# CMU-Quake/hercules

Hardware: AMD Instinct MI355X
Metric: element-updates/sec (whole node) + achieved HBM GB/s, 64M-elem box (higher is better)
Workload: dtype f64

## Files before the change

### hercules_amd/build.py

```python
import os
import subprocess
import sys

HERE = os.path.dirname(os.path.abspath(__file__))
ROOT = os.path.dirname(HERE)
CSRC = os.path.join(HERE, "csrc")
HIPCC = os.environ.get("HIPCC", "/opt/rocm/bin/hipcc")

SOLVER_LIB = os.path.join(CSRC, "libhq_solver.so")
HOST_LIB = os.path.join(CSRC, "libhq_host.so")


def _newer(target, sources):
    if not os.path.exists(target):
        return True
    t = os.path.getmtime(target)
    return any(os.path.getmtime(s) > t for s in sources)


def _build_solver(lib, defines, force):
    srcs = [os.path.join(CSRC, f) for f in ("hq_engine.hip", "hq_devmem.h", "hq_kernels.h", "hq_opts.h", "hq_patch.h",
                                           "hq_brick.h", "hq_prepare.h", "hq_plan_check.h", "hq_cadence.h", "hq_peak.h", "hq_cumul.h", "hq_sample.h", "hq_sdof.h",
                                           "hq_outputs.h")]
    srcs.append(os.path.join(ROOT, "include", "hq_solver.h"))
    if force or _newer(lib, srcs):
        cmd = [HIPCC, "-O3", "-std=c++17", "--offload-arch=gfx950", "-fPIC", "-shared"] + defines + \
              ["-fvisibility=hidden", "-fopenmp", "-Wno-unused-value"] + \
              os.environ.get("HQ_EXTRA_FLAGS", "").split() + \
              ["-o", lib, srcs[0], "-Wl,-rpath,/opt/rocm/lib", "-Wl,-Bsymbolic", "-ldl"]
        subprocess.check_call(cmd, cwd=CSRC)
    return lib


def build_solver(force=False):
    return _build_solver(SOLVER_LIB, [], force)


SOLVER_LIB_F32 = os.path.join(CSRC, "libhq_solver_f32.so")


def build_solver_f32(force=False):
    return _build_solver(SOLVER_LIB_F32, ["-DHQ_SINGLE_PRECISION_SOLVER"], force)


def build_host(force=False):
    src = os.path.join(CSRC, "hq_host.c")
    if not os.path.exists(src):
        return None
    deps = [src, os.path.join(CSRC, "hq_mesher.h"), os.path.join(CSRC, "hq_cadence.h"), os.path.join(CSRC, "hq_peak.h"), os.path.join(CSRC, "hq_cumul.h"),
            os.path.join(CSRC, "hq_sample.h"), os.path.join(CSRC, "hq_sdof.h"), os.path.join(ROOT, "include", "hq_host.h"),
            os.path.join(ROOT, "include", "hq_solver.h")]
    if force or _newer(HOST_LIB, deps):
        cmd = ["gcc", "-O2", "-std=gnu99", "-fPIC", "-shared", "-fvisibility=hidden", "-fopenmp",
               "-I", os.path.join(ROOT, "include"), "-o", HOST_LIB, src,
               "-L", CSRC, "-lhq_solver", "-Wl,-rpath,$ORIGIN", "-lm"]
        subprocess.check_call(cmd, cwd=CSRC)
    return HOST_LIB


EXAMPLE_BIN = os.path.join(ROOT, "examples", "hq_psolve_mini")


def build_example(force=False):
    src = os.path.join(ROOT, "examples", "hq_psolve_mini.c")
    if not os.path.exists(src):
        return None
    if force or _newer(EXAMPLE_BIN, [src, SOLVER_LIB, HOST_LIB]):
        cmd = ["gcc", "-O2", "-std=gnu99", "-I", os.path.join(ROOT, "include"), "-o", EXAMPLE_BIN, src,
               "-L", CSRC, "-lhq_host", "-lhq_solver", "-Wl,-rpath,$ORIGIN/../hercules_amd/csrc",
               "-Wl,-rpath,/opt/rocm/lib", "-lm"]
        subprocess.check_call(cmd)
    return EXAMPLE_BIN


def build(force=False):
    out = build_solver(force), build_host(force)
    build_solver_f32(force)
    build_example(force)
    return out


if __name__ == "__main__":
    print(build(force="--force" in sys.argv))
```

### hercules_amd/capi.py

```python
import ctypes
import os

import numpy as np

_HERE = os.path.dirname(os.path.abspath(__file__))
_LIBPATH = os.environ.get("HQ_SOLVER_LIB") or os.path.join(_HERE, "csrc", "libhq_solver.so")

HQ_VARIANT_AUTO, HQ_VARIANT_SCATTER, HQ_VARIANT_PATCH = 0, 1, 2
IPC_BLOB_BYTES = 4096

EXPORTS = ["hq_device_count", "hq_last_error", "hq_create", "hq_destroy", "hq_get_info", "hq_get_info_sized", "hq_abi_version", "hq_comm_init_ipc_n",
           "hq_options_init", "hq_create_opts", "hq_get_options", "hq_real_bytes",
           "hq_comm_unique_id", "hq_comm_init", "hq_comm_selftest", "hq_group_link", "hq_group_run", "hq_set_source", "hq_run", "hq_sync", "hq_gather", "hq_gather3",
           "hq_download", "hq_upload", "hq_phase_force", "hq_phase_update", "hq_download_force",
           "hq_run_timed", "hq_dominant_kernel", "hq_plan_check", "hq_stencil_plan_check", "hq_check_finite",
           "hq_stencil_coefficients", "hq_brick_plan_check", "hq_brick_plan_check_n", "hq_comm_init_host",
           "hq_comm_ipc_export", "hq_comm_init_ipc", "hq_comm_init_loopback",
           "hq_record_add", "hq_record_pending", "hq_record_fetch", "hq_record_clear",
           "hq_snapshot_add", "hq_snapshot_pending", "hq_snapshot_fetch", "hq_snapshot_clear",
           "hq_peak_add", "hq_peak_fetch", "hq_peak_load", "hq_peak_reset", "hq_peak_clear",
           "hq_spec_add", "hq_spec_coefficients", "hq_spec_fetch", "hq_spec_load", "hq_spec_reset", "hq_spec_clear",
           "hq_cum_add", "hq_cum_fetch", "hq_cum_load", "hq_cum_reset", "hq_cum_clear"]
HQ_SNAP_TM1, HQ_SNAP_TM2, HQ_SNAP_VEL = 1, 2, 4
HQ_PEAK_DISP, HQ_PEAK_VEL, HQ_PEAK_ACC = 1, 2, 4
HQ_SPEC_MAX_PERIODS, HQ_SPEC_NVAL = 32, 4


class HqError(RuntimeError):
    pass


HOST_EXCHANGE_FN = ctypes.CFUNCTYPE(ctypes.c_int, ctypes.c_void_p, ctypes.c_int32, ctypes.POINTER(ctypes.c_int32),
                                    ctypes.POINTER(ctypes.c_int64), ctypes.POINTER(ctypes.c_void_p), ctypes.c_int32,
                                    ctypes.POINTER(ctypes.c_int32), ctypes.POINTER(ctypes.c_int64),
                                    ctypes.POINTER(ctypes.c_void_p), ctypes.c_int32)


class _Messenger(ctypes.Structure):
    _fields_ = [("procid", ctypes.c_int32), ("nodecount", ctypes.c_int32),
                ("mapping", ctypes.c_void_p)]


class _Schedule(ctypes.Structure):
    _fields_ = [("c_count", ctypes.c_int32), ("first_c", ctypes.POINTER(_Messenger)),
                ("s_count", ctypes.c_int32), ("first_s", ctypes.POINTER(_Messenger))]


class _Desc(ctypes.Structure):
    _fields_ = [("lenum", ctypes.c_int32), ("nharbored", ctypes.c_int32), ("ldnnum", ctypes.c_int32),
                ("lnid", ctypes.c_void_p), ("node_xyz", ctypes.c_void_p),
                ("dn_ldnid", ctypes.c_void_p), ("dn_ptr", ctypes.c_void_p), ("dn_lanid", ctypes.c_void_p),
                ("eTable", ctypes.c_void_p), ("nTable", ctypes.c_void_p),
                ("tm1", ctypes.c_void_p), ("tm2", ctypes.c_void_p),
                ("an_sched", _Schedule), ("dn_sched", _Schedule),
                ("deltaT", ctypes.c_double), ("rank", ctypes.c_int32), ("nranks", ctypes.c_int32),
                ("variant", ctypes.c_int32), ("reserved", ctypes.c_int32), ("node_gnid", ctypes.c_void_p),
                ("edata", ctypes.c_void_p), ("mat_bbase", ctypes.c_double), ("mat_threshold_damping", ctypes.c_double),
                ("mat_threshold_vpvs", ctypes.c_double)]


class _RecorderDesc(ctypes.Structure):
    _fields_ = [("npoints", ctypes.c_int32), ("ids", ctypes.c_void_p), ("phi", ctypes.c_void_p),
                ("rate", ctypes.c_int32), ("derivs", ctypes.c_int32), ("capacity", ctypes.c_int32)]


class _SnapshotDesc(ctypes.Structure):
    _fields_ = [("first", ctypes.c_int32), ("count", ctypes.c_int32), ("rate", ctypes.c_int32),
                ("first_step", ctypes.c_int32), ("fields", ctypes.c_int32), ("slots", ctypes.c_int32)]


class _PeakDesc(ctypes.Structure):
    _fields_ = [("npoints", ctypes.c_int32), ("nodes_per_point", ctypes.c_int32), ("ids", ctypes.c_void_p),
                ("phi", ctypes.c_void_p), ("rate", ctypes.c_int32), ("first_step", ctypes.c_int32),
                ("quantities", ctypes.c_int32), ("reserved", ctypes.c_int32)]


class _SpecDesc(ctypes.Structure):
    _fields_ = [("npoints", ctypes.c_int32), ("nodes_per_point", ctypes.c_int32), ("ids", ctypes.c_void_p),
                ("phi", ctypes.c_void_p), ("rate", ctypes.c_int32), ("first_step", ctypes.c_int32),
                ("nperiods", ctypes.c_int32), ("reserved", ctypes.c_int32), ("periods", ctypes.c_void_p),
                ("damping", ctypes.c_double)]


class _CumDesc(ctypes.Structure):
    _fields_ = [("npoints", ctypes.c_int32), ("nodes_per_point", ctypes.c_int32), ("ids", ctypes.c_void_p),
                ("phi", ctypes.c_void_p), ("rate", ctypes.c_int32), ("first_step", ctypes.c_int32),
                ("quantities", ctypes.c_int32), ("husid_every", ctypes.c_int32), ("husid_slots", ctypes.c_int32),
                ("reserved", ctypes.c_int32), ("threshold", ctypes.c_double * 3)]


class _Info(ctypes.Structure):
    _fields_ = [("variant", ctypes.c_int32), ("npatches", ctypes.c_int32),
                ("patch_pairs", ctypes.c_int64), ("device_bytes", ctypes.c_int64),
                ("step", ctypes.c_int32), ("nranks", ctypes.c_int32),
                ("lattice_patches", ctypes.c_int32), ("stencil_patches", ctypes.c_int32),
                ("ragged_patches", ctypes.c_int32), ("brick_units", ctypes.c_int32),
                ("brick_nodes", ctypes.c_int64), ("brick_units_pernode", ctypes.c_int32),
                ("brick_units_het", ctypes.c_int32), ("pcie_h2d_bytes", ctypes.c_int64),
                ("pcie_d2h_bytes", ctypes.c_int64), ("transport", ctypes.c_int32), ("ipc_arena_coarse", ctypes.c_int32),
                ("ipc_arena_kind", ctypes.c_int32), ("debug_halo", ctypes.c_int32),
                ("brick_units_packed", ctypes.c_int32), ("brick_units_ragged", ctypes.c_int32),
                ("brick_stream", ctypes.c_int32), ("brick_units_ragged_het", ctypes.c_int32), ("timed_steps", ctypes.c_int64),
                ("t_step_us", ctypes.c_double), ("t_shell_us", ctypes.c_double), ("t_interior_us", ctypes.c_double),
                ("t_chain_us", ctypes.c_double), ("t_chain_exposed_us", ctypes.c_double)]


OPTION_FIELDS = ["no_bricks", "brick_cz", "brick_minz", "brick_minnodes", "brick_no_het", "brick_no_ntsame", "brick_by_component",
                 "brick_stream", "brick_no_faces", "brick_half_tiles", "brick_no_pack", "patch_pipe", "patch_threads", "patch_pmax", "patch_pmerge", "patch_psplit", "patch_nlmax",
                 "patch_vmax", "patch_ragged", "patch_no_lattice", "patch_no_stencil", "patch_no_uniform", "patch_no_iso",
                 "patch_no_ntsame", "patch_no_dedup", "patch_wform", "patch_merge_rounds", "overlap", "no_overlap", "reserve_cus",
                 "cu_mask", "no_fused_share", "group_copies", "debug_halo", "ipc_arena"]


class Options(ctypes.Structure):
    _fields_ = ([("size", ctypes.c_uint64)] + [(n, ctypes.c_int32) for n in OPTION_FIELDS] +
                [("ipc_timeout_ms", ctypes.c_double), ("loopback_delay_us", ctypes.c_double),
                 ("verbose", ctypes.c_int32), ("quiet", ctypes.c_int32),
                 ("brick_ragged", ctypes.c_int32), ("brick_ragged_minfill", ctypes.c_int32),
                 ("allow_env", ctypes.c_int32), ("brick_ragged_het", ctypes.c_int32), ("reserved0", ctypes.c_int32),
                 ("phase_timing", ctypes.c_int32)])

    def __init__(self, **kw):
        super().__init__()
        load_library().hq_options_init(ctypes.byref(self), ctypes.c_uint64(ctypes.sizeof(self)))
        for k, v in kw.items():
            if k not in dict(self._fields_):
                raise TypeError("hq_options has no field %r" % k)
            setattr(self, k, v)

    def as_dict(self):
        return {k: getattr(self, k) for k, _ in self._fields_ if k != "size"}


_lib = None
_lib_f32 = None
_LIBPATH_F32 = os.environ.get("HQ_SOLVER_LIB_F32") or os.path.join(_HERE, "csrc", "libhq_solver_f32.so")


def load_library(path=None, precision="f64"):
    global _lib, _lib_f32
    if precision == "f32" and path is None:
        if _lib_f32 is None:
            _lib_f32 = load_library(_LIBPATH_F32)
            if _lib_f32.hq_real_bytes() != 4:
                raise HqError("%s was not built with -DHQ_SINGLE_PRECISION_SOLVER" % _LIBPATH_F32)
        return _lib_f32
    if _lib is not None and path is None:
        return _lib
    p = path or _LIBPATH
    if not os.path.exists(p):
        raise HqError("native library %s is missing: run `python -m hercules_amd.build` "
                      "(there is no Python/CPU fallback)" % p)
    probe = ctypes.CDLL(p, mode=ctypes.RTLD_LOCAL)
    lib = probe if probe.hq_real_bytes() == 4 else ctypes.CDLL(p, mode=ctypes.RTLD_GLOBAL)
    lib.hq_last_error.restype = ctypes.c_char_p
    lib.hq_dominant_kernel.restype = ctypes.c_char_p
    lib.hq_dominant_kernel.argtypes = [ctypes.c_void_p]
    for name in EXPORTS:
        getattr(lib, name)
    if path is None:
        _lib = lib
    return lib


def device_count():
    return int(load_library().hq_device_count())


def _check(rc, lib=None):
    if rc != 0:
        raise HqError("hq error %d: %s" % (rc, (lib or load_library()).hq_last_error().decode()))


def _ptr(a):
    return None if a is None else a.ctypes.data_as(ctypes.c_void_p)


def _schedule(sched, keep):
    out = _Schedule()
    if not sched:
        return out
    for key, cnt, first in (("c", "c_count", "first_c"), ("s", "s_count", "first_s")):
        items = sched.get(key, [])
        arr = (_Messenger * max(len(items), 1))()
        for i, (procid, mapping) in enumerate(items):
            m = np.ascontiguousarray(mapping, np.int32)
            keep.append(m)
            arr[i].procid = int(procid)
            arr[i].nodecount = len(m)
            arr[i].mapping = m.ctypes.data
        keep.append(arr)
        setattr(out, cnt, len(items))
        setattr(out, first, ctypes.cast(arr, ctypes.POINTER(_Messenger)))
    return out


class Solver:

    def __init__(self, lnid, etable, ntable, dt, tm1=None, tm2=None, node_xyz=None,
                 dangling=None, an_sched=None, dn_sched=None, rank=0, nranks=1,
                 variant=HQ_VARIANT_AUTO, device=0, options=None, edata=None, material=None, precision="f64"):
        lib = load_library(precision=precision)
# ... 44 lines not shown
    def close(self):
        if getattr(self, "_h", None) and self._h.value:
            self._lib.hq_destroy(self._h)
            self._h = ctypes.c_void_p()

    __del__ = close

    def info(self):
        i = _Info()
        _check(self._lib.hq_get_info_sized(self._h, ctypes.byref(i), ctypes.c_uint64(ctypes.sizeof(i))), self._lib)
        return {k: getattr(i, k) for k, _ in _Info._fields_}

    def options(self):
        o = Options()
        _check(self._lib.hq_get_options(self._h, ctypes.byref(o), ctypes.c_uint64(ctypes.sizeof(o))), self._lib)
        return o.as_dict()

    def set_source(self, loaded_lnid, forces, step0=0):
        ids = np.ascontiguousarray(loaded_lnid, np.int32)
        F = np.ascontiguousarray(forces, np.float64)
        nsteps = F.shape[0] if len(ids) else 0
        _check(self._lib.hq_set_source(self._h, ctypes.c_int32(len(ids)), _ptr(ids),
                                       ctypes.c_int32(step0), ctypes.c_int32(nsteps), _ptr(F)))

    def comm_init(self, id128):
        buf = (ctypes.c_char * 128).from_buffer_copy(bytes(id128))
        _check(self._lib.hq_comm_init(self._h, buf), self._lib)

    def comm_init_host(self, exchange):
        import numpy as np

        def view(ptr, n):
            return np.ctypeslib.as_array(ctypes.cast(ctypes.c_void_p(ptr), ctypes.POINTER(ctypes.c_double)), shape=(int(n),))

        def trampoline(user, nrecv, rpeer, rcount, rbuf, nsend, speer, scount, sbuf, tag):
            try:
                exchange([(rpeer[i], view(rbuf[i], rcount[i])) for i in range(nrecv)],
                         [(speer[i], view(sbuf[i], scount[i])) for i in range(nsend)], tag)
                return 0
            except Exception:
                import traceback
                traceback.print_exc()
                return 1
        self._host_exchange = HOST_EXCHANGE_FN(trampoline)
        _check(self._lib.hq_comm_init_host(self._h, self._host_exchange, None), self._lib)

    def comm_ipc_export(self):
        buf = (ctypes.c_char * IPC_BLOB_BYTES)()
        _check(self._lib.hq_comm_ipc_export(self._h, buf), self._lib)
        return bytes(buf)

    def comm_init_ipc(self, blobs):
        raw = blobs if isinstance(blobs, (bytes, bytearray)) else b"".join(blobs)
        if len(raw) % IPC_BLOB_BYTES:
            raise HqError("comm_init_ipc: %d bytes is not a whole number of %d-byte blobs" % (len(raw), IPC_BLOB_BYTES))
        buf = (ctypes.c_char * len(raw)).from_buffer_copy(bytes(raw))
        _check(self._lib.hq_comm_init_ipc_n(self._h, buf, ctypes.c_int32(len(raw) // IPC_BLOB_BYTES)), self._lib)

    def comm_init_loopback(self):
        _check(self._lib.hq_comm_init_loopback(self._h), self._lib)

    def comm_selftest(self, count=1024):
        _check(self._lib.hq_comm_selftest(self._h, ctypes.c_int32(count)), self._lib)

    def run(self, nsteps):
        _check(self._lib.hq_run(self._h, ctypes.c_int32(nsteps)), self._lib)

    def sync(self):
        _check(self._lib.hq_sync(self._h), self._lib)

    def check_finite(self):
        n = ctypes.c_int64()
        _check(self._lib.hq_check_finite(self._h, ctypes.byref(n)), self._lib)
        return int(n.value)

    def run_timed(self, nsteps):
        tot, ker = ctypes.c_double(), ctypes.c_double()
        _check(self._lib.hq_run_timed(self._h, ctypes.c_int32(nsteps), ctypes.byref(tot), ctypes.byref(ker)), self._lib)
        return tot.value, ker.value

    def dominant_kernel(self):
        return self._lib.hq_dominant_kernel(self._h).decode()

    def download(self, want_tm2=True):
        tm1 = np.empty((self.N, 3), self.real)
        tm2 = np.empty((self.N, 3), self.real) if want_tm2 else None
        _check(self._lib.hq_download(self._h, _ptr(tm1), _ptr(tm2)), self._lib)
        return tm1, tm2

    def upload(self, tm1, tm2, step):
        a = np.ascontiguousarray(tm1, self.real)
        b = np.ascontiguousarray(tm2, self.real)
        _check(self._lib.hq_upload(self._h, _ptr(a), _ptr(b), ctypes.c_int32(step)), self._lib)

    def gather(self, lnid):
        ids = np.ascontiguousarray(np.asarray(lnid).reshape(-1), np.int32)
        o1 = np.empty((len(ids), 3), self.real)
        o2 = np.empty((len(ids), 3), self.real)
        _check(self._lib.hq_gather(self._h, ctypes.c_int32(len(ids)), _ptr(ids), _ptr(o1), _ptr(o2)), self._lib)
        return o1, o2

    def gather3(self, lnid):
        ids = np.ascontiguousarray(np.asarray(lnid).reshape(-1), np.int32)
        o = [np.empty((len(ids), 3), self.real) for _ in range(3)]
        _check(self._lib.hq_gather3(self._h, ctypes.c_int32(len(ids)), _ptr(ids), _ptr(o[0]), _ptr(o[1]), _ptr(o[2])), self._lib)
        return tuple(o)

    def record_add(self, ids, phi, rate, derivs=0, capacity=1024):
        ids = np.ascontiguousarray(np.asarray(ids).reshape(-1, 8), np.int32)
        phi = np.ascontiguousarray(np.asarray(phi).reshape(-1, 8), np.float64)
        if len(ids) != len(phi):
            raise HqError("record_add: %d rows of ids, %d of phi" % (len(ids), len(phi)))
        d = _RecorderDesc(len(ids), ids.ctypes.data, phi.ctypes.data, int(rate), int(derivs), int(capacity))
        h = ctypes.c_int32(-1)
        _check(self._lib.hq_record_add(self._h, ctypes.byref(d), ctypes.byref(h)), self._lib)
        if not hasattr(self, "_recorders"):
            self._recorders = {}
        self._recorders[h.value] = (len(ids), 3 * (1 + int(derivs)))
        return h.value

    def record_pending(self, handle):
        n, first = ctypes.c_int32(), ctypes.c_int32()
        _check(self._lib.hq_record_pending(self._h, ctypes.c_int32(handle), ctypes.byref(n), ctypes.byref(first)), self._lib)
        return n.value, first.value

    def record_fetch(self, handle, max_samples=None):
        pending, _ = self.record_pending(handle)
        npoints, ncomp = self._recorders[handle]
        want = pending if max_samples is None else min(int(max_samples), pending)
        steps = np.zeros(max(want, 1), np.int32)
        vals = np.zeros((max(want, 1), npoints, ncomp))
        got = ctypes.c_int32()
        _check(self._lib.hq_record_fetch(self._h, ctypes.c_int32(handle), ctypes.c_int32(want), _ptr(vals), _ptr(steps),
                                         ctypes.byref(got)), self._lib)
        return steps[:got.value].copy(), vals[:got.value].copy()

    def record_clear(self):
        _check(self._lib.hq_record_clear(self._h), self._lib)
        self._recorders = {}

    def snapshot_add(self, first=0, count=None, rate=1, first_step=0, fields=HQ_SNAP_TM1, slots=1):
        count = self.N - int(first) if count is None else int(count)
        d = _SnapshotDesc(int(first), count, int(rate), int(first_step), int(fields), int(slots))
        h = ctypes.c_int32(-1)
        _check(self._lib.hq_snapshot_add(self._h, ctypes.byref(d), ctypes.byref(h)), self._lib)
        if not hasattr(self, "_snapshots"):
            self._snapshots = {}
        self._snapshots[h.value] = (count, int(fields))
        return h.value

    def snapshot_pending(self, handle):
        n, ready, first = ctypes.c_int32(), ctypes.c_int32(), ctypes.c_int32()
        _check(self._lib.hq_snapshot_pending(self._h, ctypes.c_int32(handle), ctypes.byref(n), ctypes.byref(ready),
                                             ctypes.byref(first)), self._lib)
        return n.value, ready.value, first.value

    def snapshot_fetch(self, handle):
        self.snapshot_pending(handle)
        count, fields = self._snapshots[handle]
        tm1 = np.empty((count, 3), self.real) if fields & HQ_SNAP_TM1 else None
        tm2 = np.empty((count, 3), self.real) if fields & HQ_SNAP_TM2 else None
        vel = np.empty((count, 3), np.float64) if fields & HQ_SNAP_VEL else None
        step = ctypes.c_int32(-1)
        _check(self._lib.hq_snapshot_fetch(self._h, ctypes.c_int32(handle), _ptr(tm1), _ptr(tm2), _ptr(vel),
                                           ctypes.byref(step)), self._lib)
        if step.value < 0:
# ... 246 lines not shown
```

### hercules_amd/csrc/hq_brick.h

```cpp
#ifndef HQ_BRICK_H
#define HQ_BRICK_H

#include <chrono>
#include <map>

#include "hq_patch.h"

#define HQ_BK_TX 64
#ifndef HQ_BK_TY
#define HQ_BK_TY 8
#endif
#define HQ_BK_THREADS (HQ_BK_TX * HQ_BK_TY)
#define HQ_BK_PY (HQ_BK_TX + 2)
#define HQ_BK_PLANE ((HQ_BK_TX + 2) * (HQ_BK_TY + 2))
#ifndef HQ_BK_ATTR
#define HQ_BK_ATTR
#endif
#define HQ_BK_NTSAME 1
#define HQ_BK_HET 2
#define HQ_BK_TOPFACE 8
#define HQ_BK_BOTFACE 16
#define HQ_BK_RAGGED 32
#define HQ_BK_PACKED 4
#ifndef HQ_BH_WAVES
// ... 670 lines not shown
                            if (cx >= 0 && cy >= 0 && cz >= 0 && cx < L.D[0] && cy < L.D[1] && cz < L.D[2])
                                e = L.Eg[(size_t)((cz * L.D[1] + cy) * L.D[0] + cx)];
                            float* o = cq + (int64_t)l * (3 * HQ_BH_THREADS) + (j * 64 + i);
                            o[0] = o[HQ_BH_CS] = o[2 * HQ_BH_CS] = 0.0f;
                            if (e < 0) continue;
                            const float* ed = MS->edata + 4 * (int64_t)e;
                            if (ed[0] != hf || !(ed[3] > 0.0f)) { ok = false; break; }
                            bool hit = false;
                            for (int fixed = 0; fixed < 2 && !hit; fixed++) {
                                double k1, k2, kb;
                                hq_material_coef(fixed ? -ed[3] : ed[3], ed[2], ed[1], K, &k1, &k2, &kb);
                                if (k1 == c1[e] && k2 == c2[e] && kb == beta[e]) { o[0] = fixed ? -ed[3] : ed[3]; o[HQ_BH_CS] = ed[2]; o[2 * HQ_BH_CS] = ed[1]; hit = true; }
                            }
                            if (!hit) { ok = false; break; }
                        }
                const int32_t* own_ids = c.rag ? t + (int64_t)(np + 2) * nr + (int64_t)nx * ny : nullptr;
                for (int32_t z = 0; z < np && ok; z++)
                    for (int32_t y = 0; y < ny && ok; y++)
                        for (int32_t x = 0; x < nx; x++) {
                            if (own_ids && own_ids[((int64_t)z * ny + y) * nx + x] < 0) continue;
                            const int32_t n = L.Ng[(size_t)((((int64_t)za + z) * NY + (c.y0 + y)) * NX + (c.x0 + x))];
                            const double* q = ntab + 7 * (int64_t)n;
                            const double sdiff = q[0] - q[4];
                            if (q[0] - sdiff != q[4] || fabs((2.0 * q[0] - sdiff) - q[1]) > 1e-15 * fabs(q[1])) { ok = false; break; }
                            double* o2 = B->nt2.data() + 2 * (own_ids ? (int64_t)own_ids[((int64_t)z * ny + y) * nx + x] : U.base + ((int64_t)z * ny + y) * nx + x);
                            o2[0] = q[0]; o2[1] = sdiff;
                        }
                if (ok) { U.flags |= HQ_BK_PACKED; same[(size_t)u] = c.rag ? 6 : 3; U.c1 = K.A; U.c2 = K.h; }
            }
        }
    }
    lap("unit tables");
    if (fault) { g_patch_err = "brick plan: a neighbour of a simple node is missing"; return -1; }
    {
        std::vector<hq_brick_unit> a, r, b, h, hp, rh, rhp;
        for (size_t u = 0; u < us.size(); u++)
            (same[u] == 1 ? a : (same[u] == 4 ? r : (same[u] == 2 ? h : (same[u] == 3 ? hp : (same[u] == 5 ? rh : (same[u] == 6 ? rhp : b)))))).push_back(B->units[u]);
        B->nsame = (int32_t)(a.size() + r.size());
        B->nrag = (int32_t)r.size();
        B->nhet = (int32_t)(h.size() + hp.size());
        B->npacked = (int32_t)hp.size();
        B->nrhet = (int32_t)(rh.size() + rhp.size());
        B->nrpacked = (int32_t)rhp.size();
        a.insert(a.end(), r.begin(), r.end());
        a.insert(a.end(), b.begin(), b.end());
        a.insert(a.end(), h.begin(), h.end());
        a.insert(a.end(), hp.begin(), hp.end());
        a.insert(a.end(), rh.begin(), rh.end());
        a.insert(a.end(), rhp.begin(), rhp.end());
        B->units.swap(a);
        if (B->npacked + B->nrpacked == 0) { std::vector<float>().swap(B->coef32); std::vector<double>().swap(B->nt2); }
        if (verbose) fprintf(stderr, "  brick plan: %d units: %d with one n_t row of which %d ragged, %d per-element coefficients of which %d packed, %d ragged per-element of which %d packed\n",
                             (int)B->units.size(), B->nsame, B->nrag, B->nhet, B->npacked, B->nrhet, B->nrpacked);
        if (verbose && B->nrag) {
            int64_t pos = 0, own = 0, other = 0;
            for (const hq_brick_unit& U : B->units) {
                if (!(U.flags & HQ_BK_RAGGED)) continue;
                const int32_t* pl = B->tab.data() + U.tab + (int64_t)(U.np + 2) * (2 * (U.nx + 2) + 2 * U.ny);
                for (int64_t i = 0; i < (int64_t)U.nx * U.ny * (U.np + 2); i++) { pos++; own += pl[i] >= 0; other += pl[i] <= -2; }
            }
            fprintf(stderr, "  brick plan: ragged units: %lld positions, %lld owned, %lld loaded for their neighbours' sake\n", (long long)pos, (long long)own, (long long)other);
        }
    }
    return 0;
}


static __device__ __forceinline__ double hq_uniform(double v)
{
    const int lo = __builtin_amdgcn_readfirstlane(__double2loint(v)), hi = __builtin_amdgcn_readfirstlane(__double2hiint(v));
    return __hiloint2double(hi, lo);
}

template <bool PERNODE, bool BYCOMP, bool RAGGED = false>
__global__ void HQ_BK_ATTR __launch_bounds__(HQ_BK_THREADS, 4)
hq_k_brick(int32_t count, int32_t per_xcd, const hq_brick_unit* __restrict__ units, const int32_t* __restrict__ tab,
           const hq_real* __restrict__ u1g, const hq_real* __restrict__ u2g, hq_real* __restrict__ ung,
           const double* __restrict__ nt3, const int32_t* __restrict__ src_ptr, const int32_t* __restrict__ src_ent,
           const double* __restrict__ F, double dt2, hq_stencil_coef sc)
{
    __shared__ __align__(16) double s_w[2 * 3 * HQ_BK_PLANE];
    const int slot = (int)(blockIdx.x & 7) * per_xcd + (int)(blockIdx.x >> 3);
    if (slot >= count) return;
    const hq_brick_unit U = units[slot];
    const int nx = U.nx, ny = U.ny, np = U.np, nxy = nx * ny, nr = 2 * (nx + 2) + 2 * ny;
    const int t = threadIdx.x, lx = t & (HQ_BK_TX - 1), ly = t >> 6;
    const bool active = lx < nx && ly < ny;
    const int sidx = active ? ly * nx + lx : 0;
    const int myrow = (ly + 1) * HQ_BK_PY + lx + 1;
    const bool ring = t < nr;
    int rrow;
    {
        int rx, ry;
        if (t < nx + 2) { rx = t - 1; ry = -1; }
        else if (t < 2 * (nx + 2)) { rx = t - (nx + 2) - 1; ry = ny; }
        else if (t < 2 * (nx + 2) + ny) { rx = -1; ry = t - 2 * (nx + 2); }
        else { rx = nx; ry = t - 2 * (nx + 2) - ny; }
        rrow = (ry + 1) * HQ_BK_PY + rx + 1;
    }
    const int32_t* __restrict__ utab = tab + U.tab;
    const int rofs = ring ? t : 0;
    const int32_t* __restrict__ cap = utab + (int64_t)(np + 2) * nr;
    int32_t vOut = -1, vMid = RAGGED ? cap[sidx] : 0, vCur = RAGGED ? cap[nxy + sidx] : 0, vNext = 0;
    const int32_t id_lo = RAGGED ? (vMid >= 0 ? vMid : -vMid - 2) : cap[sidx];
    const double beta = U.beta;
    double P[6], Q[2];
#pragma unroll
    for (int i = 0; i < 6; i++) P[i] = hq_uniform(U.c1 * sc.p1[i] + U.c2 * sc.p2[i]);
#pragma unroll
    for (int i = 0; i < 2; i++) Q[i] = hq_uniform(U.c1 * sc.q1[i] + U.c2 * sc.q2[i]);
    const bool has_src = F && src_ptr[slot + 1] > src_ptr[slot];

    hq_real x1[3] = { 0, 0, 0 }, x2[3] = { 0, 0, 0 }, y1[3] = { 0, 0, 0 }, y2[3] = { 0, 0, 0 };
    double mn[3] = { U.m0, U.m2, U.m1 };
    double m0A = hq_uniform(1.0 / U.m0), m0B = m0A;
    double fA[3] = { 0.0, 0.0, 0.0 }, fB[3] = { 0.0, 0.0, 0.0 };
    int32_t rid = utab[rofs];

#define HQ_BK_LOAD(node_)                                                                             \
    {                                                                                                 \
        const int64_t a_ = (node_);                                                                   \
        if (active && (!RAGGED || a_ >= 0)) {                                                         \
            _Pragma("unroll") for (int d = 0; d < 3; d++) { x1[d] = u1g[3 * a_ + d]; x2[d] = u2g[3 * a_ + d]; } \
            if (PERNODE) { _Pragma("unroll") for (int d = 0; d < 3; d++) mn[d] = nt3[3 * a_ + d]; }    \
        }                                                                                             \
        if (ring && (!RAGGED || rid >= 0)) {                                                          \
            const int64_t b_ = (int64_t)rid;                                                          \
            _Pragma("unroll") for (int d = 0; d < 3; d++) { y1[d] = u1g[3 * b_ + d]; y2[d] = u2g[3 * b_ + d]; } \
        }                                                                                             \
    }
#define HQ_BK_PUT(s_, acc_, M2_, M1_)                                                                 \
    {                                                                                                 \
        hq_lds_double* img_ = (hq_lds_double*)s_w + 3 * HQ_BK_PLANE * (s_);                            \
        if (active) {                                                                                 \
            _Pragma("unroll") for (int d = 0; d < 3; d++) {                                           \
                const double a1_ = x1[d], a2_ = x2[d];                                                \
                img_[3 * myrow + d] = a1_ + beta * (a1_ - a2_);                                       \
                acc_[d] += (M2_) * a1_ - (M1_) * a2_;                                                 \
            }                                                                                         \
        }                                                                                             \
        if (ring) { _Pragma("unroll") for (int d = 0; d < 3; d++) { const double b1_ = y1[d], b2_ = y2[d]; img_[3 * rrow + d] = b1_ + beta * (b1_ - b2_); } } \
    }

    const bool topf = !PERNODE && !RAGGED && (U.flags & HQ_BK_TOPFACE) != 0, botf = !PERNODE && !RAGGED && (U.flags & HQ_BK_BOTFACE) != 0;
    const double rho = hq_uniform((U.c1 - U.c2) / (U.c1 + U.c2));

    HQ_BK_LOAD((int64_t)id_lo)
    rid = utab[nr + rofs];
    if (topf) HQ_BK_PUT(0, fB, U.ft[1 + d], U.ft[4 + d])
    else { double dummy[3] = { 0.0, 0.0, 0.0 }; HQ_BK_PUT(0, dummy, mn[1], mn[2]) }
    for (int k = 0; k <= np + 1; k++) {
        if (k <= np) {
            if (RAGGED) {
                HQ_BK_LOAD((int64_t)(vCur >= 0 ? vCur : -vCur - 2))
                if (k < np) vNext = cap[(k + 2) * nxy + sidx];
            } else HQ_BK_LOAD(k == np ? (int64_t)cap[nxy + sidx] : U.base + (int64_t)k * nxy + sidx)
            if (k < np) rid = utab[(k + 2) * nr + rofs];
        }
        __syncthreads();
        const hq_lds_double* __restrict__ q = (const hq_lds_double*)s_w + 3 * (HQ_BK_PLANE * (k & 1) + myrow);
        double m[3], g[3], Uo[3];
        if (BYCOMP) {
            double A_x, A_y;
            {
                const double C = q[2], XM = q[2 - 3], XP = q[2 + 3], YM = q[2 - 3 * HQ_BK_PY], YP = q[2 + 3 * HQ_BK_PY];
                const double MM = q[2 - 3 * HQ_BK_PY - 3], PM = q[2 - 3 * HQ_BK_PY + 3], MP = q[2 + 3 * HQ_BK_PY - 3], PP = q[2 + 3 * HQ_BK_PY + 3];
                const double sxy = (XM + XP) + (YM + YP), dg = (MM + PP) + (PM + MP);
                m[2] = fma(P[0], C, fma(P[2], sxy, P[4] * dg));
                g[2] = fma(P[1], C, fma(P[3], sxy, P[5] * dg));
                Uo[0] = fma(Q[0], XP - XM, Q[1] * ((PP - MP) + (PM - MM)));
                Uo[1] = fma(Q[0], YP - YM, Q[1] * ((PP - PM) + (MP - MM)));
            }
            __builtin_amdgcn_sched_barrier(0);
            {
                const double C = q[0], XM = q[0 - 3], XP = q[0 + 3], YM = q[0 - 3 * HQ_BK_PY], YP = q[0 + 3 * HQ_BK_PY];
                const double MM = q[0 - 3 * HQ_BK_PY - 3], PM = q[0 - 3 * HQ_BK_PY + 3], MP = q[0 + 3 * HQ_BK_PY - 3], PP = q[0 + 3 * HQ_BK_PY + 3];
                const double sx = XM + XP, sy = YM + YP, dg = (MM + PP) + (PM + MP);
                A_x = (PP + MM) - (PM + MP);
                m[0] = fma(P[0], C, fma(P[1], sx, fma(P[2], sy, P[3] * dg)));
                g[0] = fma(P[2], C, fma(P[3], sx, fma(P[4], sy, P[5] * dg)));
                Uo[2] = fma(Q[0], XP - XM, Q[1] * ((PP - MP) + (PM - MM)));
            }
            __builtin_amdgcn_sched_barrier(0);
            {
                const double C = q[1], XM = q[1 - 3], XP = q[1 + 3], YM = q[1 - 3 * HQ_BK_PY], YP = q[1 + 3 * HQ_BK_PY];
                const double MM = q[1 - 3 * HQ_BK_PY - 3], PM = q[1 - 3 * HQ_BK_PY + 3], MP = q[1 + 3 * HQ_BK_PY - 3], PP = q[1 + 3 * HQ_BK_PY + 3];
                const double sx = XM + XP, sy = YM + YP, dg = (MM + PP) + (PM + MP);
                A_y = (PP + MM) - (PM + MP);
                m[1] = fma(P[0], C, fma(P[1], sy, fma(P[2], sx, fma(P[3], dg, Q[0] * A_x))));
                g[1] = fma(P[2], C, fma(P[3], sy, fma(P[4], sx, fma(P[5], dg, Q[1] * A_x))));
                Uo[2] += fma(Q[0], YP - YM, Q[1] * ((PP - PM) + (MP - MM)));
            }
            m[0] = fma(Q[0], A_y, m[0]);
            g[0] = fma(Q[1], A_y, g[0]);
        } else {
            double C[3], XM[3], XP[3], YM[3], YP[3], MM[3], PM[3], MP[3], PP[3];
#pragma unroll
            for (int d = 0; d < 3; d++) {
                C[d] = q[d]; XM[d] = q[d - 3]; XP[d] = q[d + 3]; YM[d] = q[d - 3 * HQ_BK_PY]; YP[d] = q[d + 3 * HQ_BK_PY];
                MM[d] = q[d - 3 * HQ_BK_PY - 3]; PM[d] = q[d - 3 * HQ_BK_PY + 3];
                MP[d] = q[d + 3 * HQ_BK_PY - 3]; PP[d] = q[d + 3 * HQ_BK_PY + 3];
            }
            double sx[3], sy[3], dg[3];
#pragma unroll
            for (int d = 0; d < 3; d++) { sx[d] = XM[d] + XP[d]; sy[d] = YM[d] + YP[d]; dg[d] = (MM[d] + PP[d]) + (PM[d] + MP[d]); }
            const double A_x = (PP[0] + MM[0]) - (PM[0] + MP[0]), A_y = (PP[1] + MM[1]) - (PM[1] + MP[1]);
            const double Bx0_z = XP[2] - XM[2], Bx0_x = XP[0] - XM[0], By0_z = YP[2] - YM[2], By0_y = YP[1] - YM[1];
            const double Bx1_z = (PP[2] - MP[2]) + (PM[2] - MM[2]), Bx1_x = (PP[0] - MP[0]) + (PM[0] - MM[0]);
            const double By1_z = (PP[2] - PM[2]) + (MP[2] - MM[2]), By1_y = (PP[1] - PM[1]) + (MP[1] - MM[1]);
            const double sxy_z = sx[2] + sy[2];
            m[0] = fma(P[0], C[0], fma(P[1], sx[0], fma(P[2], sy[0], fma(P[3], dg[0], Q[0] * A_y))));
            m[1] = fma(P[0], C[1], fma(P[1], sy[1], fma(P[2], sx[1], fma(P[3], dg[1], Q[0] * A_x))));
            m[2] = fma(P[0], C[2], fma(P[2], sxy_z, P[4] * dg[2]));
            g[0] = fma(P[2], C[0], fma(P[3], sx[0], fma(P[4], sy[0], fma(P[5], dg[0], Q[1] * A_y))));
            g[1] = fma(P[2], C[1], fma(P[3], sy[1], fma(P[4], sx[1], fma(P[5], dg[1], Q[1] * A_x))));
            g[2] = fma(P[1], C[2], fma(P[3], sxy_z, P[5] * dg[2]));
            Uo[0] = fma(Q[0], Bx0_z, Q[1] * Bx1_z);
            Uo[1] = fma(Q[0], By0_z, Q[1] * By1_z);
            Uo[2] = fma(Q[0], Bx0_x, fma(Q[1], Bx1_x, fma(Q[0], By0_y, Q[1] * By1_y)));
        }
        if (k == 0 && topf) {
            m[0] = fma(rho, Uo[0], 0.5 * m[0]); m[1] = fma(rho, Uo[1], 0.5 * m[1]); m[2] = fma(-rho, Uo[2], 0.5 * m[2]);
        }
        if (k == np + 1 && botf && active) {
            double f[3];
            f[0] = fB[0] + fma(-rho, Uo[0], 0.5 * m[0]); f[1] = fB[1] + fma(-rho, Uo[1], 0.5 * m[1]); f[2] = fB[2] + fma(rho, Uo[2], 0.5 * m[2]);
            const int local = np * nxy + sidx;
            if (has_src) {
                for (int i = src_ptr[slot]; i < src_ptr[slot + 1]; i++)
                    if (src_ent[2 * i] == local) {
                        const int li = src_ent[2 * i + 1];
                        for (int d = 0; d < 3; d++) f[d] += F[3 * li + d] * dt2;
                    }
            }
            hq_real* out = ung + 3 * (int64_t)cap[nxy + sidx];
            const double rm = 1.0 / U.fb[0];
#pragma unroll
            for (int d = 0; d < 3; d++) out[d] = f[d] * rm;
        }
        const bool outface = k == 1 && topf;
        if ((k >= 2 || outface) && active && (!RAGGED || vOut >= 0)) {
            double f[3];
#pragma unroll
            for (int d = 0; d < 3; d++) f[d] = fA[d] + (g[d] + Uo[d]);
            const int local = RAGGED ? (int)(vOut - U.base) : (k - 2) * nxy + sidx;
            if (has_src) {
                for (int i = src_ptr[slot]; i < src_ptr[slot + 1]; i++)
                    if (src_ent[2 * i] == local) {
                        const int li = src_ent[2 * i + 1];
                        for (int d = 0; d < 3; d++) f[d] += F[3 * li + d] * dt2;
                    }
            }
            hq_real* out = ung + 3 * (RAGGED ? (int64_t)vOut : (outface ? (int64_t)cap[sidx] : U.base + (int64_t)local));
            const double rm = outface ? 1.0 / U.ft[0] : m0A;
#pragma unroll
            for (int d = 0; d < 3; d++) out[d] = f[d] * rm;
        }
#pragma unroll
        for (int d = 0; d < 3; d++) { fA[d] = fB[d] + m[d]; fB[d] = g[d] - Uo[d]; }
        if (RAGGED) { vOut = vMid; vMid = vCur; vCur = vNext; }
        if (PERNODE) { m0A = m0B; m0B = 1.0 / mn[0]; }
        if (k < np || (k == np && !botf)) HQ_BK_PUT((k + 1) & 1, fB, mn[1], mn[2])
        else if (k == np) HQ_BK_PUT((k + 1) & 1, fB, U.fb[1 + d], U.fb[4 + d])
    }
#undef HQ_BK_LOAD
#undef HQ_BK_PUT
}


#define HQ_BH_LDS (8 * (2 * 2 * 3 * HQ_BH_ROWS + 6 * HQ_BH_THREADS))
#ifndef HQ_BH_ABL
#define HQ_BH_ABL 0
#endif

static __device__ __forceinline__ double hq_dpp_from_next_lane(double v)
{
    int lo = __double2loint(v), hi = __double2hiint(v);
    lo = __builtin_amdgcn_update_dpp(0, lo, 0x130, 0xf, 0xf, true);
    hi = __builtin_amdgcn_update_dpp(0, hi, 0x130, 0xf, 0xf, true);
    return __hiloint2double(hi, lo);
}

static __device__ __forceinline__ int64_t hq_rag_node(int32_t v) { return v >= 0 ? (int64_t)v : (v <= -2 ? (int64_t)(-v - 2) : (int64_t)0); }

template <bool PACKED, bool RAGGED = false>
__global__ void __launch_bounds__(HQ_BH_THREADS, HQ_BH_WAVES == 12 ? 3 : 4)
hq_k_brick_het(int32_t count, int32_t per_xcd, const hq_brick_unit* __restrict__ units, const int32_t* __restrict__ tab,
               const void* __restrict__ coef_any, const hq_real* __restrict__ u1g, const hq_real* __restrict__ u2g,
               hq_real* __restrict__ ung, const double* __restrict__ nt3, const int32_t* __restrict__ src_ptr,
               const int32_t* __restrict__ src_ent, const double* __restrict__ F, double dt2, hq_mat_const mat)
{
    extern __shared__ __align__(16) double s_het[];
    hq_lds_double* const img = (hq_lds_double*)s_het;
    hq_lds_double* const xch = img + 2 * 2 * 3 * HQ_BH_ROWS;
    const int slot = (int)(blockIdx.x & 7) * per_xcd + (int)(blockIdx.x >> 3);
    if (slot >= count) return;
    const hq_brick_unit U = units[slot];
    const int nx = U.nx, ny = U.ny, np = U.np, nxy = nx * ny, nr = 2 * (nx + 2) + 2 * ny;
    const int t = threadIdx.x, lx = t & 63, ly = t >> 6;
    const bool owner = lx < nx && ly < ny;
    const int sidx = owner ? ly * nx + lx : 0;
    const int myrow = (ly + 1) * HQ_BH_PY + lx + 1;
    const int row0 = ly * HQ_BH_PY + lx;
    const int rq = ly == HQ_BH_WAVES - 1 ? lx : (lx >= 62 ? 64 + 2 * ly + (lx - 62) : -1);
    const bool ringA = rq >= 0 && rq < nr, ringB = rq >= 0 && rq + HQ_BH_NRT < nr;
    auto ring_row = [&](int r) {
        int rx, ry;
        if (r < nx + 2) { rx = r - 1; ry = -1; }
        else if (r < 2 * (nx + 2)) { rx = r - (nx + 2) - 1; ry = ny; }
        else if (r < 2 * (nx + 2) + ny) { rx = -1; ry = r - 2 * (nx + 2); }
        else { rx = nx; ry = r - 2 * (nx + 2) - ny; }
        return (ry + 1) * HQ_BH_PY + rx + 1;
    };
    const int rrowA = ringA ? ring_row(rq) : 0, rrowB = ringB ? ring_row(rq + HQ_BH_NRT) : 0;
    const int32_t* __restrict__ rtabA = tab + U.tab + (ringA ? rq : 0);
    const int32_t* __restrict__ rtabB = tab + U.tab + (ringB ? rq + HQ_BH_NRT : 0);
    const int32_t* __restrict__ cap = tab + U.tab + (int64_t)(np + 2) * nr;
    const int64_t id_lo = RAGGED ? 0 : cap[sidx], id_hi = RAGGED ? 0 : cap[nxy + sidx];
    int32_t vload = RAGGED ? cap[sidx] : 0, vnext = RAGGED ? cap[nxy + sidx] : 0, idA = -1, idB = -1;
    const double* __restrict__ cf = (const double*)coef_any + (PACKED ? 0 : U.coef + t);
    const float* __restrict__ cf32 = (const float*)coef_any + (PACKED ? U.coef + t : 0);
    hq_mat_const K = mat;
    if (PACKED) { K.A = hq_uniform(U.c1); K.h = hq_uniform(U.c2); }
    const int third = (PACKED && owner) ? 1 : 2;
    const bool has_src = F && src_ptr[slot + 1] > src_ptr[slot];

    hq_real x1[3] = { 0, 0, 0 }, x2[3] = { 0, 0, 0 }, rb1[3] = { 0, 0, 0 }, rb2[3] = { 0, 0, 0 };
    constexpr bool SAME = sizeof(hq_real) == sizeof(double);
    double mn[3] = { 1.0, 0.0, 0.0 };
    double accA[3] = { 0.0, 0.0, 0.0 }, accB[3] = { 0.0, 0.0, 0.0 }, m0A = 1.0, m0B = 1.0;
    int32_t ridA = rtabA[0], ridB = rtabB[0];
    if (RAGGED) { ridA = ridA < 0 ? 0 : ridA; ridB = ridB < 0 ? 0 : ridB; }

#define HQ_BH_LOAD(node_)                                                                             \
    {                                                                                                 \
        const int64_t a_ = owner ? (int64_t)(node_) : (int64_t)ridA;                                  \
        const double* __restrict__ pb_ = (owner || sizeof(hq_real) != sizeof(double)) ? nt3 + (PACKED ? 2 : 3) * a_ : (const double*)(const void*)(u1g + 3 * (int64_t)ridB); \
        _Pragma("unroll") for (int d = 0; d < 3; d++) { x1[d] = u1g[3 * a_ + d]; x2[d] = u2g[3 * a_ + d]; } \
        if (SAME || owner) {                                                                          \
            if (HQ_BH_ABL != 4) { mn[0] = pb_[0]; mn[1] = pb_[1]; mn[2] = pb_[third]; }                \
        } else {                      \
            const hq_real* __restrict__ pu_ = u1g + 3 * (int64_t)ridB;                                \
            rb1[0] = pu_[0]; rb1[1] = pu_[1]; rb1[2] = pu_[2];                                         \
        }                                                                                             \
    }
#define HQ_BH_LOAD_B()                                                                                \
    {                                                                                                 \
        if (ringB && HQ_BH_ABL != 1) {                                                                \
            const int64_t b_ = (int64_t)ridB;                                                         \
// ... 99 lines not shown
        __syncthreads();
    }
#undef HQ_BH_REQUEST
#undef HQ_BH_LOAD
#undef HQ_BH_LOAD_B
#undef HQ_BH_PUT
}


static void hq_brick_free(hq_brick_plan* P)
{
    *P = hq_brick_plan();
}

static int hq_brick_upload(hq_brick_plan* P, const hq_brick_host& B, int64_t* ledger, hipStream_t st)
{
    P->nb = B.nb;
    P->nunits = (int32_t)B.units.size();
    P->nsame = B.nsame;
    P->nrag = B.nrag;
    P->nhet = B.nhet;
    P->npacked = B.npacked;
    P->nrhet = B.nrhet;
    P->nrpacked = B.nrpacked;
    if (P->nunits == 0) return HQ_OK;
    if (P->nhet + P->nrhet > 0) {
        if (P->nhet > P->npacked || P->nrhet > P->nrpacked) HQ_TRY(P->d_coef.put(ledger, B.coef, st));
        if (P->npacked + P->nrpacked > 0) {
            HQ_TRY(P->d_coef32.put(ledger, B.coef32, st));
            HQ_TRY(P->d_nt2.put(ledger, B.nt2, st));
        }
        static bool attr_set = false;
        if (!attr_set) {
            if (hipFuncSetAttribute((const void*)hq_k_brick_het<false>, hipFuncAttributeMaxDynamicSharedMemorySize, HQ_BH_LDS) != hipSuccess ||
                hipFuncSetAttribute((const void*)hq_k_brick_het<true>, hipFuncAttributeMaxDynamicSharedMemorySize, HQ_BH_LDS) != hipSuccess ||
                hipFuncSetAttribute((const void*)hq_k_brick_het<false, true>, hipFuncAttributeMaxDynamicSharedMemorySize, HQ_BH_LDS) != hipSuccess ||
                hipFuncSetAttribute((const void*)hq_k_brick_het<true, true>, hipFuncAttributeMaxDynamicSharedMemorySize, HQ_BH_LDS) != hipSuccess) return hq_fail(HQ_ERR_DEVICE, "hq_k_brick_het: LDS attribute%s", "");
            attr_set = true;
        }
    }
    HQ_TRY(P->d_units.put(ledger, B.units, st));
    HQ_TRY(P->d_tab.put(ledger, B.tab, st));
    std::vector<std::pair<int64_t, int32_t>> by_base;
    for (int32_t u = 0; u < P->nunits; u++) by_base.push_back({ B.units[(size_t)u].base, u });
    std::sort(by_base.begin(), by_base.end());
    for (auto& pr : by_base) {
        const hq_brick_unit& U = B.units[(size_t)pr.second];
        const int64_t nxy = (int64_t)U.nx * U.ny;
        const int top = (U.flags & HQ_BK_TOPFACE) != 0, bot = (U.flags & HQ_BK_BOTFACE) != 0;
        int64_t size = nxy * (U.np + top + bot);
        if (U.flags & HQ_BK_RAGGED) {
            const int32_t* pl = B.tab.data() + U.tab + (int64_t)(U.np + 2) * (2 * (U.nx + 2) + 2 * U.ny);
            size = 0;
            for (int64_t i = nxy; i < nxy * (U.np + 1); i++) size += pl[i] >= 0;
        }
        P->h_base.push_back(pr.first - top * nxy); P->h_slot.push_back(pr.second); P->h_size.push_back(size);
        P->h_first.push_back(pr.first);
    }
    return HQ_OK;
}

static int hq_brick_set_source(hq_brick_plan* P, int32_t nloaded, const int32_t* loaded, int64_t* ledger, hipStream_t st)
{
    P->d_src_ptr.reset();
    P->d_src_ent.reset();
    if (nloaded <= 0 || P->nunits == 0) return HQ_OK;
    std::vector<std::array<int32_t, 3>> rec;
    for (int32_t i = 0; i < nloaded; i++) {
        if (loaded[i] >= P->nb) continue;
        const size_t k = (size_t)(std::upper_bound(P->h_base.begin(), P->h_base.end(), (int64_t)loaded[i]) - P->h_base.begin()) - 1;
        rec.push_back({ P->h_slot[k], (int32_t)(loaded[i] - P->h_first[k]), i });
    }
    if (rec.empty()) return HQ_OK;
    std::sort(rec.begin(), rec.end());
    std::vector<int32_t> ptr((size_t)P->nunits + 1, 0), ent(rec.size() * 2);
    for (auto& r : rec) ptr[(size_t)r[0] + 1]++;
    for (int32_t u = 0; u < P->nunits; u++) ptr[(size_t)u + 1] += ptr[(size_t)u];
    for (size_t k = 0; k < rec.size(); k++) { ent[2 * k] = rec[k][1]; ent[2 * k + 1] = rec[k][2]; }
    HQ_TRY(P->d_src_ptr.put(ledger, ptr, st));
    return P->d_src_ent.put(ledger, ent, st);
}

static void hq_brick_launch(const hq_brick_plan* P, const hq_real* u1, const hq_real* u2, hq_real* un, const double* nt3,
                            const double* F, double dt2, hipStream_t stream, bool light = false)
{
    const int32_t cnt[7] = { P->nsame - P->nrag, P->nunits - P->nsame - P->nhet - P->nrhet, P->nhet - P->npacked, P->npacked, P->nrag,
                             P->nrhet - P->nrpacked, P->nrpacked };
    int32_t first = 0;
    for (int k4 = 0; k4 < 7; k4++) {
        const int k = k4 == 0 ? 0 : (k4 == 1 ? 4 : (k4 < 5 ? k4 - 1 : k4));
        const int32_t count = cnt[k];
        if (count <= 0) continue;
        const int per_xcd = (count + 7) / 8;
        const int32_t* sp = P->d_src_ptr ? P->d_src_ptr + first : nullptr;
#define HQ_BK_ARGS count, per_xcd, P->d_units + first, P->d_tab, u1, u2, un, nt3, sp, P->d_src_ent, (sp ? F : nullptr), dt2, hq_stencil().c
#ifdef HQ_EXPERIMENT
        const unsigned xpad = getenv("HQ_X_BRICK_LDS_PAD") ? (unsigned)atoi(getenv("HQ_X_BRICK_LDS_PAD")) : 0u;
        if (xpad && k == 0) {
            static bool once = false;
            if (!once) {
                once = true;
                hipFuncSetAttribute((const void*)hq_k_brick<false, true>, hipFuncAttributeMaxDynamicSharedMemorySize, (int)xpad);
                hipFuncSetAttribute((const void*)hq_k_brick<false, false>, hipFuncAttributeMaxDynamicSharedMemorySize, (int)xpad);
            }
            if (light) hq_k_brick<false, true><<<per_xcd * 8, HQ_BK_THREADS, xpad, stream>>>(HQ_BK_ARGS);
            else hq_k_brick<false, false><<<per_xcd * 8, HQ_BK_THREADS, xpad, stream>>>(HQ_BK_ARGS);
        } else
#endif
        if (k == 0 && light) hq_k_brick<false, true><<<per_xcd * 8, HQ_BK_THREADS, 0, stream>>>(HQ_BK_ARGS);
        else if (k == 0) hq_k_brick<false, false><<<per_xcd * 8, HQ_BK_THREADS, 0, stream>>>(HQ_BK_ARGS);
        else if (k == 1 && light) hq_k_brick<true, true><<<per_xcd * 8, HQ_BK_THREADS, 0, stream>>>(HQ_BK_ARGS);
        else if (k == 1) hq_k_brick<true, false><<<per_xcd * 8, HQ_BK_THREADS, 0, stream>>>(HQ_BK_ARGS);
        else if (k == 4 && light) hq_k_brick<false, true, true><<<per_xcd * 8, HQ_BK_THREADS, 0, stream>>>(HQ_BK_ARGS);
        else if (k == 4) hq_k_brick<false, false, true><<<per_xcd * 8, HQ_BK_THREADS, 0, stream>>>(HQ_BK_ARGS);
        else if (k == 2) hq_k_brick_het<false><<<per_xcd * 8, HQ_BH_THREADS, HQ_BH_LDS, stream>>>(count, per_xcd, P->d_units + first, P->d_tab, P->d_coef, u1, u2, un, nt3, sp,
                                                                                               P->d_src_ent, (sp ? F : nullptr), dt2, P->mat);
        else if (k == 3) hq_k_brick_het<true><<<per_xcd * 8, HQ_BH_THREADS, HQ_BH_LDS, stream>>>(count, per_xcd, P->d_units + first, P->d_tab, P->d_coef32, u1, u2, un, P->d_nt2, sp,
                                                                                   P->d_src_ent, (sp ? F : nullptr), dt2, P->mat);
        else if (k == 5) hq_k_brick_het<false, true><<<per_xcd * 8, HQ_BH_THREADS, HQ_BH_LDS, stream>>>(count, per_xcd, P->d_units + first, P->d_tab, P->d_coef, u1, u2, un, nt3, sp,
                                                                                                     P->d_src_ent, (sp ? F : nullptr), dt2, P->mat);
        else hq_k_brick_het<true, true><<<per_xcd * 8, HQ_BH_THREADS, HQ_BH_LDS, stream>>>(count, per_xcd, P->d_units + first, P->d_tab, P->d_coef32, u1, u2, un, P->d_nt2, sp,
                                                                                          P->d_src_ent, (sp ? F : nullptr), dt2, P->mat);
#undef HQ_BK_ARGS
        first += count;
    }
}

#endif
```

### hercules_amd/csrc/hq_engine.hip

```cpp
#include <hip/hip_runtime.h>
#include <dlfcn.h>
#include <stdint.h>
#include <stdio.h>
#include <stdlib.h>
#include <string.h>
#include <unistd.h>

#include <algorithm>
#include <chrono>
#include <vector>

#define HQ_SOLVER_IMPLEMENTATION 1
#include "../../include/hq_solver.h"
#include "hq_devmem.h"
#include "hq_kernels.h"
#include "hq_opts.h"
#include "hq_cadence.h"
#include "hq_peak.h"
#include "hq_cumul.h"
#include "hq_sdof.h"
#define HQ_SAMPLE_REAL hq_real
#include "hq_sample.h"
#include "hq_patch.h"
#include "hq_brick.h"
// ... 44 lines not shown

#define HQ_NCCL(call)                                                                     \
    do {                                                                                  \
        ncclResult_t r_ = (call);                                                         \
        if (r_ != ncclSuccess) return hq_fail(HQ_ERR_COMM, "%s: %s", #call, g_rccl.GetErrorString(r_)); \
    } while (0)


struct hq_dev_messenger {
    int32_t procid, nodecount;
    int32_t offset;
};

struct hq_dev_schedule {
    std::vector<hq_dev_messenger> c, s;
    hq_dbuf<int32_t> d_cmap;
    hq_dbuf<int32_t> d_smap;
    int32_t* d_cmap_f = nullptr;
    int32_t* d_smap_f = nullptr;
    hq_dbuf<int32_t> d_cslot, d_sslot;
    hq_dbuf<double> d_c_out;
    hq_dbuf<double> d_s_out;
    double*  d_c_in = nullptr;
    double*  d_s_in = nullptr;
    hq_dbuf<double> c_in_mem, s_in_mem;
    int32_t  ctotal = 0, stotal = 0;
    hq_dbuf<int64_t> d_c_out_id, d_c_in_id, d_s_out_id, d_s_in_id;
    hq_dbuf<double*> d_c_dst, d_s_dst;
    double*  h_c_out = nullptr;
    double*  h_c_in = nullptr;
    double*  h_s_out = nullptr;
    double*  h_s_in = nullptr;
    int64_t* h_c_out_id = nullptr;
    int64_t* h_c_in_id = nullptr;
    int64_t* h_s_out_id = nullptr;
    int64_t* h_s_in_id = nullptr;
};

struct hq_ctx {
    hq_options opts;
    int device = 0;
    hipStream_t stream = nullptr;
    int32_t E = 0, N = 0, ldnnum = 0;
    int32_t variant = HQ_VARIANT_SCATTER;
    int32_t step = 0;
    int32_t rank = 0, nranks = 1;
    double dt = 0, dt2 = 0;
    int64_t bytes = 0;
    int64_t h2d_bytes = 0, d2h_bytes = 0;
    hq_dbuf<int32_t> d_gather_ids;
    hq_dbuf<hq_real> d_gather_out;
    int32_t gather_cap = 0;

    int32_t Epad = 0;
    hq_dbuf<int32_t> d_lnid;
    hq_dbuf<double> d_c1, d_c2, d_beta;
    double* d_nt = nullptr;
    hq_dbuf<double> d_nt_rows;
    hq_dbuf<hq_real> d_u[3];
    int now = 0, prev = 1, spare = 2;
    hq_dbuf<double> d_force;
    int32_t nloaded = 0, src_step0 = 0, src_nsteps = 0;
    hq_dbuf<int32_t> d_loaded;
    hq_dbuf<double> d_F;
    std::vector<int32_t> h_loaded;
    size_t F_capacity = 0;
    hq_dbuf<int32_t> d_dn_id, d_dn_ptr, d_dn_anchor;
    hq_dev_schedule an, dn;
    hq_nccl_comm comm = nullptr;
    hq_host_exchange_fn host_xchg = nullptr;
    void* host_user = nullptr;
    std::vector<hq_ctx*>* group = nullptr;
    bool group_owner = false;
    bool share_packed = false;
    struct hq_ipc_state* ipc = nullptr;
    hipEvent_t ev_sent = nullptr;
    hipStream_t cstream = nullptr;
    hipEvent_t ev_bnd = nullptr, ev_shared = nullptr, ev_an_shared = nullptr, ev_assigned = nullptr;
    hipStream_t bstream = nullptr;
    hipEvent_t ev_patches = nullptr, ev_bricks = nullptr;
    bool overlap = false;
    bool stream_masked = false;
    bool can_overlap = false;
    int reserve_cus = 8;
    int32_t nI = 0, nOI = 0;
    hq_dbuf<double> d_iforce;
    hq_dbuf<int32_t> d_oi_node;
    hq_dbuf<int32_t> d_oi_slot;
    hq_dbuf<int32_t> d_oi_ptr;
    hq_dbuf<int32_t> d_oi_pos;
    hq_dbuf<int32_t> d_oi_fc;
    int32_t  nSD = 0;
    hq_dbuf<int32_t> d_sd_dst;
    hq_dbuf<int32_t> d_sd_ptr;
    hq_dbuf<int32_t> d_sd_src;
    hq_dbuf<int32_t> d_sd_deps;
    hq_patch_plan plan;
    hq_brick_plan bricks;
    std::vector<int32_t> perm;
    bool debug_halo = false;
    unsigned long long dbg_send_epoch[4] = { 0, 0, 0, 0 }, dbg_recv_epoch[4] = { 0, 0, 0, 0 };
    hq_dbuf<int64_t> d_gkey;
    hq_dbuf<int32_t> d_halo_err;
    enum { HQ_CLK_STEP0 = 0, HQ_CLK_SHELL1, HQ_CLK_INT0, HQ_CLK_INT1, HQ_CLK_CHAIN0, HQ_CLK_CHAIN1, HQ_CLK_N, HQ_CLK_SLOTS = 64 };
    struct hq_clock_slot { hipEvent_t e[HQ_CLK_N] = {}; bool used[HQ_CLK_N] = {}; bool pending = false; };
    bool clock_skip = false;
    std::vector<hq_clock_slot> clock;
    size_t clock_at = 0;
    double clk_us[5] = { 0, 0, 0, 0, 0 };
    int64_t clk_steps = 0;
    struct hq_output; struct hq_recorder; struct hq_peak_tracker; struct hq_spec_tracker; struct hq_cum_tracker; struct hq_snapshot;
    std::vector<hq_recorder> recs;
    int32_t rec_next_id = 0;
    std::vector<hq_peak_tracker> peaks;
    int32_t peak_next_id = 0;
    std::vector<hq_spec_tracker> specs;
    int32_t spec_next_id = 0;
    std::vector<hq_cum_tracker> cums;
    int32_t cum_next_id = 0;
    std::vector<hq_snapshot> snaps;
    int32_t snap_next_id = 0;
    hipStream_t sstream = nullptr;
    hipEvent_t ev_output = nullptr;
    std::vector<hipEvent_t> ev;
    hipEvent_t ev_span[2] = { nullptr, nullptr };
    bool timing = false;
    size_t ev_used = 0;
};

enum { HQ_IPC_MAXNB = 64, HQ_IPC_MAGIC = 0x48514950  };
struct hq_ipc_blob {
    uint32_t magic, version;
    int32_t rank, nranks, device, pid;
    int32_t coarse, reserved;
    char busid[32];
    uint64_t arena_bytes, arena_addr;
    hipIpcMemHandle_t mem;
    uint64_t buf_off[4];
    uint64_t flag_off;
    uint64_t id_off[4];
    int32_t nrecv[4];
    struct { int32_t procid, offset, count; } recv[4][HQ_IPC_MAXNB];
};
static_assert(sizeof(hq_ipc_blob) <= HQ_IPC_BLOB_BYTES, "hq_ipc_blob must fit HQ_IPC_BLOB_BYTES");

struct hq_ipc_state {
    void* arena = nullptr;
    size_t arena_bytes = 0;
    bool coarse = false, ready = false, loopback = false;
    int arena_kind = 0;
    hq_ipc_blob mine;
    std::vector<void*> opened;
    unsigned long long* d_flags = nullptr;
    hq_dbuf<double*> d_dst[4];
    hq_dbuf<unsigned long long*> d_sig[4];
    hq_dbuf<int64_t*> d_dst_id[4];
    int64_t* d_in_id[4] = { nullptr, nullptr, nullptr, nullptr };
    int32_t nsig[4] = { 0, 0, 0, 0 };
    unsigned long long wait_mask[4] = { 0, 0, 0, 0 };
    unsigned long long send_epoch[4] = { 0, 0, 0, 0 }, recv_epoch[4] = { 0, 0, 0, 0 };
    hq_dbuf<uint32_t> d_done;
    unsigned long long timeout_ticks = 2000000000ull;
    unsigned long long delay_ticks = 0;
};


// ... 598 lines not shown
}

struct hq_ipc_args {
    const unsigned long long* wait_flags;
    unsigned long long wait_mask, wait_epoch, timeout_ticks;
    int32_t* err;
    uint32_t* done;
    int32_t nsig;
    unsigned long long* const* sig;
    unsigned long long sig_epoch;
    unsigned long long delay_ticks;
};

template <int IPC>
__global__ void __launch_bounds__(256)
hq_k_interface_update(int32_t n, const int32_t* __restrict__ node, const int32_t* __restrict__ slot,
                      const int32_t* __restrict__ ptr, const int32_t* __restrict__ pos, const int32_t* __restrict__ fcv,
                      const double* __restrict__ iforce, const double* rec,
                      const double* __restrict__ nt, const hq_real* __restrict__ u1,
                      const hq_real* __restrict__ u2, hq_real* __restrict__ un, double* __restrict__ s_out,
                      double* const* __restrict__ s_dst, hq_ipc_args ia)
{
    int t = blockIdx.x * blockDim.x + threadIdx.x;
    if (IPC) {
        const int j = threadIdx.x;
        if (j < 64 && ((ia.wait_mask >> j) & 1ull)) {
            const unsigned long long t0 = wall_clock64();
            while (__hip_atomic_load(&ia.wait_flags[j], __ATOMIC_RELAXED, __HIP_MEMORY_SCOPE_SYSTEM) < ia.wait_epoch) {
                __builtin_amdgcn_s_sleep(16);
                if (wall_clock64() - t0 > ia.timeout_ticks) { atomicAdd(ia.err, 1); break; }
            }
        }
        __syncthreads();
    }
    if (t < n * 3) {
        int i = t / 3, d = t - 3 * i;
        int64_t g = node[i];
        const int32_t fc = fcv[i];
        const int32_t first = fc & 0xffffff, cnt = (int32_t)((uint32_t)fc >> 24);
        const double* np = nt + 7 * g;
        double f = iforce[3 * (int64_t)slot[i] + d];
        double* p0 = (s_dst && cnt) ? s_dst[first] : nullptr;
        if (cnt)
            f += IPC ? __hip_atomic_load(rec + 3 * (int64_t)first + d, __ATOMIC_RELAXED, __HIP_MEMORY_SCOPE_SYSTEM)
                     : rec[3 * (int64_t)first + d];
        const int32_t k0 = cnt > 1 ? ptr[i] : 0;
        for (int32_t k = 1; k < cnt; k++)
            f += IPC ? __hip_atomic_load(rec + 3 * (int64_t)pos[k0 + k] + d, __ATOMIC_RELAXED, __HIP_MEMORY_SCOPE_SYSTEM)
                     : rec[3 * (int64_t)pos[k0 + k] + d];
        f += (np[1 + d] * (double)u1[3 * g + d] - np[4 + d] * (double)u2[3 * g + d]);
        const double v = (double)(hq_real)(f / np[0]);
        un[3 * g + d] = (hq_real)v;
        if (s_dst) {
            if (cnt) {
                if (IPC) __hip_atomic_store(p0 + d, v, __ATOMIC_RELAXED, __HIP_MEMORY_SCOPE_SYSTEM);
                else p0[d] = v;
            }
            for (int32_t k = 1; k < cnt; k++) {
                if (IPC) __hip_atomic_store(s_dst[pos[k0 + k]] + d, v, __ATOMIC_RELAXED, __HIP_MEMORY_SCOPE_SYSTEM);
                else s_dst[pos[k0 + k]][d] = v;
            }
        } else if (s_out) {
            if (cnt) s_out[3 * (int64_t)first + d] = v;
            for (int32_t k = 1; k < cnt; k++) s_out[3 * (int64_t)pos[k0 + k] + d] = v;
        }
    }
    if (IPC) {
        asm volatile("s_waitcnt vmcnt(0)" ::: "memory");
        __syncthreads();
        __shared__ int s_last;
        if (threadIdx.x == 0) s_last = __hip_atomic_fetch_add(ia.done, 1u, __ATOMIC_RELAXED, __HIP_MEMORY_SCOPE_AGENT) == gridDim.x - 1;
        __syncthreads();
        if (!s_last) return;
        if (threadIdx.x == 0) __hip_atomic_store(ia.done, 0u, __ATOMIC_RELAXED, __HIP_MEMORY_SCOPE_AGENT);
        if ((int)threadIdx.x < ia.nsig) {
            hq_ipc_delay(ia.delay_ticks);
            __hip_atomic_store(ia.sig[threadIdx.x], ia.sig_epoch, __ATOMIC_RELAXED, __HIP_MEMORY_SCOPE_SYSTEM);
        }
    }
}

enum { HQ_NPHASE = 9 };

static bool hq_use_brick_stream(hq_ctx* c)
{
    const bool solo = !hq_has_transport(c) && c->nranks == 1 && c->plan.npatches > 16 * c->plan.grid_cus;
    const bool want = hq_given(c->opts.brick_stream) ? c->opts.brick_stream != 0 : solo;
    if (!want || !(c->overlap || (!hq_has_transport(c) && c->nranks == 1)) || c->stream_masked || c->bricks.nunits <= 0 || c->plan.npatches <= 0) return false;
    if (!c->bstream) {
        int prio_lo = 0, prio_hi = 0;
        if (hipDeviceGetStreamPriorityRange(&prio_lo, &prio_hi) != hipSuccess) return false;
        int prio = prio_lo;
#ifdef HQ_EXPERIMENT
        if (getenv("HQ_X_BRICK_PRIO")) prio = !strcmp(getenv("HQ_X_BRICK_PRIO"), "high") ? prio_hi : (prio_lo + prio_hi) / 2;
#endif
        if (hipStreamCreateWithPriority(&c->bstream, hipStreamNonBlocking, prio) != hipSuccess) { c->bstream = nullptr; return false; }
        if (hipEventCreateWithFlags(&c->ev_patches, hipEventDisableTiming) != hipSuccess ||
            hipEventCreateWithFlags(&c->ev_bricks, hipEventDisableTiming) != hipSuccess) return false;
        hipEventRecord(c->ev_patches, c->stream);
        hipEventRecord(c->ev_bricks, c->stream);
    }
    return true;
}

#include "hq_outputs.h"

static int hq_phase(hq_ctx* c, int ph)
{
    const bool patch = (c->variant == HQ_VARIANT_PATCH);
    double* ftab = patch ? c->d_iforce : c->d_force;
    hq_real* unew = patch ? c->d_u[c->spare] : c->d_u[c->prev];
    switch (ph) {
    case 0:
        if (patch) {
            int32_t k = c->step - c->src_step0;
            const double* F = (c->nloaded > 0 && k >= 0 && k < c->src_nsteps)
                                  ? c->d_F + (int64_t)k * c->nloaded * 3 : nullptr;
            int32_t nb = c->plan.nb, ne = c->plan.ne;
            if (c->overlap && !hq_patch_uses_pers(&c->plan) && nb > 0 && nb + ne <= 2 * hq_value_or(c->opts.patch_merge_rounds, 2) * c->plan.grid_cus) { nb += ne; ne = 0; }
            const bool bs = hq_use_brick_stream(c);
            if (c->overlap) HQ_HIP(hipStreamWaitEvent(c->stream, c->ev_shared, 0));
            if (bs) {
                HQ_HIP(hipStreamWaitEvent(c->stream, c->ev_bricks, 0));
                if (c->ev_shared) HQ_HIP(hipStreamWaitEvent(c->bstream, c->ev_shared, 0));
                HQ_HIP(hipStreamWaitEvent(c->bstream, c->ev_patches, 0));
            }
            HQ_TRY(hq_outputs_enqueue(c, bs));
            auto launch_bricks = [&]() {
                if (c->bricks.nunits > 0)
                    hq_brick_launch(&c->bricks, c->d_u[c->now], c->d_u[c->prev], c->d_u[c->spare], c->plan.d_nt3, F, c->dt2,
                                    bs ? c->bstream : c->stream, hq_given(c->opts.brick_by_component) ? c->opts.brick_by_component != 0 : c->overlap);
                if (bs) hipEventRecord(c->ev_bricks, c->bstream);
            };
            hq_mark(c);
            hq_clock_begin(c);
            hq_clock(c, hq_ctx::HQ_CLK_STEP0, c->stream);
            if (bs) hq_clock(c, hq_ctx::HQ_CLK_INT0, c->bstream);
            bool chain_marked = false;
            auto chain_released = [&]() {
                if (!chain_marked && c->overlap) hq_clock(c, hq_ctx::HQ_CLK_CHAIN0, c->cstream);
                chain_marked = true;
            };
            if (c->plan.ns > 0 || c->plan.nr > 0) {
                const int32_t head = c->overlap ? nb : nb + ne;
                hq_patch_launch(&c->plan, 0, head, c->d_u[c->now], c->d_u[c->prev], c->d_u[c->spare], c->d_nt, F, c->dt2,
                                c->d_iforce, c->stream);
                hq_patch_launch_stencil(&c->plan, 0, c->d_u[c->now], c->d_u[c->prev], c->d_u[c->spare], c->d_nt, F, c->dt2,
                                        c->d_iforce, c->stream);
                if (c->overlap) {
                    HQ_HIP(hipEventRecord(c->ev_bnd, c->stream));
                    HQ_HIP(hipStreamWaitEvent(c->cstream, c->ev_bnd, 0));
                    chain_released();
                    hq_patch_launch(&c->plan, nb, ne, c->d_u[c->now], c->d_u[c->prev], c->d_u[c->spare], c->d_nt, F, c->dt2,
                                    c->d_iforce, c->stream, c->reserve_cus);
                }
                hq_patch_launch_stencil(&c->plan, 1, c->d_u[c->now], c->d_u[c->prev], c->d_u[c->spare], c->d_nt, F, c->dt2,
                                        c->d_iforce, c->stream);
            } else {
                if (c->overlap) {
                    hq_patch_launch(&c->plan, 0, nb, c->d_u[c->now], c->d_u[c->prev], c->d_u[c->spare], c->d_nt, F, c->dt2,
                                    c->d_iforce, c->stream);
                    HQ_HIP(hipEventRecord(c->ev_bnd, c->stream));
                    HQ_HIP(hipStreamWaitEvent(c->cstream, c->ev_bnd, 0));
                    chain_released();
                    hq_patch_launch(&c->plan, nb, ne, c->d_u[c->now], c->d_u[c->prev], c->d_u[c->spare], c->d_nt, F,
                                    c->dt2, c->d_iforce, c->stream, c->reserve_cus);
                } else {
                    hq_patch_launch(&c->plan, 0, nb + ne, c->d_u[c->now], c->d_u[c->prev], c->d_u[c->spare], c->d_nt, F,
                                    c->dt2, c->d_iforce, c->stream);
                }
            }
            if (bs) HQ_HIP(hipEventRecord(c->ev_patches, c->stream));
            hq_clock(c, hq_ctx::HQ_CLK_SHELL1, c->stream);
            if (!bs) hq_clock(c, hq_ctx::HQ_CLK_INT0, c->stream);
            launch_bricks();
            hq_clock(c, hq_ctx::HQ_CLK_INT1, bs ? c->bstream : c->stream);
            if (!c->overlap && hq_has_transport(c)) hq_clock(c, hq_ctx::HQ_CLK_CHAIN0, c->stream);
            hq_mark(c);
        } else {
            HQ_TRY(hq_outputs_enqueue(c, false));
            HQ_TRY(hq_launch_source(c));
            HQ_TRY(hq_launch_element_scatter(c));
        }
        return HQ_OK;
    case 1: return hq_xchg_send(c, &c->dn, ftab, true, true);
    case 2:
        HQ_TRY(hq_xchg_recv(c, &c->dn, ftab, true, true));
        if (patch) {
            if (c->nSD)
                hq_k_distribute<<<hq_blocks(c->nSD * 3, 256), 256, 0, c->overlap ? c->cstream : c->stream>>>(
                    c->nSD, c->d_sd_dst, c->d_sd_ptr, c->d_sd_src, c->d_sd_deps, c->d_iforce);
        } else if (c->nSD) {
            hq_k_distribute<<<hq_blocks(c->nSD * 3, 256), 256, 0, c->stream>>>(
                c->nSD, c->d_sd_dst, c->d_sd_ptr, c->d_sd_src, c->d_sd_deps, c->d_force);
        }
        return HQ_OK;
    case 3: return hq_xchg_send(c, &c->an, ftab, true, true);
    case 4:
        if (patch) {
            hipStream_t xs = c->overlap ? c->cstream : c->stream;
            if (c->group)
                for (auto& m : c->an.s)
                    if (m.nodecount) HQ_HIP(hipStreamWaitEvent(xs, (*c->group)[m.procid]->ev_sent, 0));
            const bool ipc_dbg = hq_ipc_ready(c) && c->debug_halo;
            if (ipc_dbg) hq_ipc_wait(c, &c->an, true, xs);
            hq_xchg_check(c, &c->an, true, xs);
            c->share_packed = false;
            if (c->nOI) {
                hq_ipc_args ia = {};
                const bool fuse = !hq_set(c->opts.no_fused_share) && !(c->debug_halo && (hq_ipc_ready(c) || c->host_xchg));
                double* s_out = fuse ? c->an.d_s_out : nullptr;
                double* const* s_dst = nullptr;
                if (fuse && c->group && c->an.d_s_dst && !c->debug_halo) s_dst = c->an.d_s_dst;
                if (hq_ipc_ready(c)) {
                    hq_ipc_state* I = c->ipc;
                    if (fuse) {
                        s_dst = I->d_dst[1];
                        ia.wait_flags = I->d_flags;
                        ia.wait_mask = I->wait_mask[0];
                        if (ia.wait_mask) ia.wait_epoch = ++I->recv_epoch[0];
                        ia.timeout_ticks = I->timeout_ticks;
                        ia.err = c->d_halo_err + 2;
                        ia.done = I->d_done + 1;
                        ia.nsig = I->nsig[1];
                        ia.sig = I->d_sig[1];
                        ia.sig_epoch = c->an.stotal ? ++I->send_epoch[1] : 0;
                        ia.delay_ticks = I->delay_ticks;
                        hq_k_interface_update<1><<<hq_blocks(c->nOI * 3, 256), 256, 0, xs>>>(
                            c->nOI, c->d_oi_node, c->d_oi_slot, c->d_oi_ptr, c->d_oi_pos, c->d_oi_fc, c->d_iforce, c->an.d_s_in,
                            c->d_nt, c->d_u[c->now], c->d_u[c->prev], unew, nullptr, s_dst, ia);
                        c->share_packed = true;
                        return HQ_OK;
                    }
                    if (!ipc_dbg) hq_ipc_wait(c, &c->an, true, xs);
                }
                hq_k_interface_update<0><<<hq_blocks(c->nOI * 3, 256), 256, 0, xs>>>(
                    c->nOI, c->d_oi_node, c->d_oi_slot, c->d_oi_ptr, c->d_oi_pos, c->d_oi_fc, c->d_iforce, c->an.d_s_in,
                    c->d_nt, c->d_u[c->now], c->d_u[c->prev], unew, s_dst ? nullptr : s_out, s_dst, ia);
                c->share_packed = fuse;
            } else if (hq_ipc_ready(c) && !ipc_dbg) {
                hq_ipc_wait(c, &c->an, true, xs);
            }
        } else {
            HQ_TRY(hq_xchg_recv(c, &c->an, ftab, true, true));
            HQ_TRY(hq_launch_update(c));
        }
        return HQ_OK;
    case 5: return hq_xchg_send(c, &c->an, unew, false, false);
    case 6:
        HQ_TRY(hq_xchg_recv(c, &c->an, unew, false, false));
        if (c->ldnnum) {
            if (c->overlap) {
                HQ_HIP(hipEventRecord(c->ev_an_shared, c->cstream));
                HQ_HIP(hipStreamWaitEvent(c->stream, c->ev_an_shared, 0));
            }
            hq_k_adjust_assign<<<hq_blocks(c->ldnnum * 3, 256), 256, 0, c->stream>>>(
                c->ldnnum, c->d_dn_id, c->d_dn_ptr, c->d_dn_anchor, unew);
// ... 140 lines not shown
        HQ_HIP(hipEventRecord(c->ev_shared, c->cstream));
        c->can_overlap = true;
        c->reserve_cus = hq_value_or(c->opts.reserve_cus, 8);
    }
    return HQ_OK;
}

extern "C" int hq_device_count(void)
{
    int n = 0;
    if (hipGetDeviceCount(&n) != hipSuccess) return 0;
    int ok = 0;
    for (int i = 0; i < n; i++) {
        hipDeviceProp_t p;
        if (hipGetDeviceProperties(&p, i) == hipSuccess && strncmp(p.gcnArchName, "gfx950", 6) == 0) ok++;
    }
    return ok;
}

static int hq_field_to_device(hq_ctx* c, const hq_real* host, hq_real* dev)
{
    const size_t bytes = sizeof(hq_real) * 3 * (size_t)c->N;
    c->h2d_bytes += (int64_t)bytes;
    if (c->perm.empty()) return hq_copy_wait(dev, host, bytes, hipMemcpyHostToDevice, c->stream);
    std::vector<hq_real> tmp;
    try { tmp.resize(3 * (size_t)c->N); } catch (...) { return hq_fail(HQ_ERR_NOMEM, "out of host memory%s", ""); }
    const int32_t* pm = c->perm.data();
#pragma omp parallel for schedule(static) if (c->N > 262144)
    for (int64_t n = 0; n < (int64_t)c->N; n++) {
        const int64_t q = pm[n];
        tmp[(size_t)(3 * q)] = host[3 * n]; tmp[(size_t)(3 * q + 1)] = host[3 * n + 1]; tmp[(size_t)(3 * q + 2)] = host[3 * n + 2];
    }
    return hq_copy_wait(dev, tmp.data(), bytes, hipMemcpyHostToDevice, c->stream);
}

static int hq_field_to_host(hq_ctx* c, const hq_real* dev, hq_real* host)
{
    const size_t bytes = sizeof(hq_real) * 3 * (size_t)c->N;
    c->d2h_bytes += (int64_t)bytes;
    if (c->perm.empty()) return hq_copy_wait(host, dev, bytes, hipMemcpyDeviceToHost, c->stream);
    std::vector<hq_real> tmp;
    try { tmp.resize(3 * (size_t)c->N); } catch (...) { return hq_fail(HQ_ERR_NOMEM, "out of host memory%s", ""); }
    HQ_TRY(hq_copy_wait(tmp.data(), dev, bytes, hipMemcpyDeviceToHost, c->stream));
    const int32_t* pm = c->perm.data();
#pragma omp parallel for schedule(static) if (c->N > 262144)
    for (int64_t n = 0; n < (int64_t)c->N; n++) {
        const int64_t q = pm[n];
        host[3 * n] = tmp[(size_t)(3 * q)]; host[3 * n + 1] = tmp[(size_t)(3 * q + 1)]; host[3 * n + 2] = tmp[(size_t)(3 * q + 2)];
    }
    return HQ_OK;
}

static int hq_create_impl(const hq_desc* d, int device, const hq_options& opts, hq_ctx** out);

#include "hq_prepare.h"

extern "C" void hq_options_init(hq_options* o, uint64_t size)
{
    if (!o || size < sizeof(uint64_t)) return;
    hq_options full;
    hq_options_defaults(&full);
    memcpy(o, &full, (size_t)std::min<uint64_t>(size, sizeof(full)));
    o->size = std::min<uint64_t>(size, sizeof(full));
}

extern "C" int hq_create_opts(const hq_desc* d, int device, const hq_options* opts, hq_ctx** out)
{
    if (opts && opts->size < sizeof(uint64_t)) return hq_fail(HQ_ERR_ARG, "hq_options.size is not set (hq_options_init)%s", "");
    hq_options full;
    hq_options_resolve(&full, opts);
    return hq_create_impl(d, device, full, out);
}

extern "C" int hq_create(const hq_desc* d, int device, hq_ctx** out) { return hq_create_opts(d, device, nullptr, out); }

extern "C" int hq_get_options(hq_ctx* c, hq_options* out, uint64_t size)
{
    if (!c || !out || size < sizeof(uint64_t)) return hq_fail(HQ_ERR_ARG, "null argument%s", "");
    memcpy(out, &c->opts, (size_t)std::min<uint64_t>(size, sizeof(c->opts)));
    out->size = std::min<uint64_t>(size, sizeof(c->opts));
    return HQ_OK;
}

static int hq_create_impl(const hq_desc* d, int device, const hq_options& opts, hq_ctx** out)
{
    if (!d || !out) return hq_fail(HQ_ERR_ARG, "null argument%s", "");
    *out = nullptr;
    int ndev = 0;
    if (hipGetDeviceCount(&ndev) != hipSuccess || ndev <= 0)
        return hq_fail(HQ_ERR_NODEVICE, "no HIP device: this engine has no CPU path%s", "");
    if (device < 0 || device >= ndev) return hq_fail(HQ_ERR_ARG, "device index out of range%s", "");
    hipDeviceProp_t prop;
    HQ_HIP(hipGetDeviceProperties(&prop, device));
    if (strncmp(prop.gcnArchName, "gfx950", 6) != 0)
        return hq_fail(HQ_ERR_NODEVICE, "device is %s, kernels are built for gfx950 only", prop.gcnArchName);
    HQ_HIP(hipSetDevice(device));
    const int variant = d->variant == HQ_VARIANT_AUTO ? HQ_VARIANT_PATCH : d->variant;
    if (variant != HQ_VARIANT_SCATTER && variant != HQ_VARIANT_PATCH) return hq_fail(HQ_ERR_ARG, "unknown variant%s", "");
    if (variant == HQ_VARIANT_PATCH && !d->node_xyz) {
        static bool warned = false;
        if (!warned && !hq_set(opts.quiet)) {
            warned = true;
            fprintf(stderr, "hq_create: hq_desc.node_xyz is NULL -- no bricks, no lattice / stencil patches (fixed runs of the node "
                            "order, element-form kernels only): expect about a third of the throughput; pass node_t.x/y/z\n");
        }
    }

    const hq_real *h_tm1 = d->tm1, *h_tm2 = d->tm2;
    hq_prep prep;
    HQ_TRY(hq_prepare(d, opts, HQ_PREP_COEF | HQ_PREP_NT | (variant == HQ_VARIANT_PATCH ? HQ_PREP_BRICKS : 0), &prep));
    d = &prep.desc;
    std::vector<char>().swap(prep.excl);
    const hq_brick_host& BH = prep.bricks;
    const double* ntab = prep.ntab;

    hq_ctx* c = new (std::nothrow) hq_ctx();
    if (!c) return hq_fail(HQ_ERR_NOMEM, "out of host memory%s", "");
    c->device = device;
    c->opts = opts;
    c->E = d->lenum; c->N = d->nharbored; c->ldnnum = d->ldnnum;
    c->dt = d->deltaT; c->dt2 = d->deltaT * d->deltaT;
    c->rank = d->rank; c->nranks = d->nranks > 0 ? d->nranks : 1;
    c->variant = variant;
    c->perm = std::move(prep.perm);
    int rc = HQ_OK;
    auto bail = [&](int r) { hq_destroy(c); return r; };
    if (hipStreamCreateWithFlags(&c->stream, hipStreamNonBlocking) != hipSuccess)
        return bail(hq_fail(HQ_ERR_DEVICE, "hipStreamCreate failed%s", ""));
    if (hipEventCreateWithFlags(&c->ev_sent, hipEventDisableTiming) != hipSuccess ||
        hipEventCreateWithFlags(&c->ev_output, hipEventDisableTiming) != hipSuccess)
        return bail(hq_fail(HQ_ERR_DEVICE, "hipEventCreate failed%s", ""));

    const bool verbose = hq_set(opts.verbose);
    auto t_last = std::chrono::steady_clock::now();
    auto lap = [&](const char* what, double s = -1.0) {
        const auto now = std::chrono::steady_clock::now();
        if (verbose) fprintf(stderr, "hq_create: %-34s %7.2f s\n", what, s >= 0.0 ? s : std::chrono::duration<double>(now - t_last).count());
        t_last = now;
    };
    if (prep.brick_plan_s > 0.0) lap("brick plan", prep.brick_plan_s);
    if (BH.nb > 0) lap("renumbering", prep.renumber_s);

    size_t n3 = (size_t)c->N * 3;
    int nbuf = (variant == HQ_VARIANT_PATCH) ? 3 : 2;
    for (int b = 0; b < nbuf; b++) {
        if ((rc = c->d_u[b].alloc(&c->bytes, n3)) != HQ_OK || (rc = c->d_u[b].fill(0, c->stream)) != HQ_OK) return bail(rc);
    }
    {
        const int64_t nt_first = (variant == HQ_VARIANT_PATCH) ? BH.nb : 0;
        const size_t rows = (size_t)std::max<int64_t>(c->N - nt_first, 1);
        if ((rc = c->d_nt_rows.alloc(&c->bytes, rows * 7)) != HQ_OK) return bail(rc);
        if (c->N > nt_first && (rc = c->d_nt_rows.upload(ntab + 7 * nt_first, 7 * (size_t)(c->N - nt_first), c->stream)) != HQ_OK) return bail(rc);
        c->d_nt = c->d_nt_rows - 7 * nt_first;
    }
    lap("state buffers, n_t rows");
    if (h_tm1 && (rc = hq_field_to_device(c, h_tm1, c->d_u[c->now])) != HQ_OK) return bail(rc);
    if (h_tm2 && (rc = hq_field_to_device(c, h_tm2, c->d_u[c->prev])) != HQ_OK) return bail(rc);
    lap("start fields");

    if (c->ldnnum) {
        int32_t na = d->dn_ptr[c->ldnnum];
        if ((rc = c->d_dn_id.put(&c->bytes, d->dn_ldnid, (size_t)c->ldnnum, c->stream)) != HQ_OK ||
            (rc = c->d_dn_ptr.put(&c->bytes, d->dn_ptr, (size_t)c->ldnnum + 1, c->stream)) != HQ_OK ||
            (rc = c->d_dn_anchor.put(&c->bytes, d->dn_lanid, (size_t)na, c->stream)) != HQ_OK)
            return bail(rc);
    }

    if ((rc = c->d_halo_err.alloc(&c->bytes, 4)) != HQ_OK || (rc = c->d_halo_err.fill(0, c->stream)) != HQ_OK) return bail(rc);
    if (hq_set(opts.debug_halo) && c->nranks > 1) {
        if (!d->node_gnid && !d->node_xyz)
            return bail(hq_fail(HQ_ERR_ARG, "HQ_DEBUG_HALO needs hq_desc.node_gnid or node_xyz%s", ""));
        std::vector<int64_t> key((size_t)c->N);
        for (int64_t n = 0; n < c->N; n++) {
            if (d->node_gnid) { key[(size_t)n] = d->node_gnid[n]; continue; }
            uint64_t h = 0x9E3779B97F4A7C15ull;
            for (int k = 0; k < 3; k++) {
                h ^= (uint64_t)(uint32_t)d->node_xyz[3 * n + k];
                h *= 0xBF58476D1CE4E5B9ull; h ^= h >> 29;
            }
            key[(size_t)n] = (int64_t)h;
        }
        if ((rc = c->d_gkey.put(&c->bytes, key, c->stream)) != HQ_OK) return bail(rc);
        c->debug_halo = true;
    }

    if (variant == HQ_VARIANT_SCATTER) {
        if ((rc = c->d_force.alloc(&c->bytes, n3)) != HQ_OK || (rc = c->d_force.fill(0, c->stream)) != HQ_OK) return bail(rc);
        c->Epad = (c->E + 63) & ~63;
        std::vector<int32_t> soa((size_t)8 * c->Epad, 0);
        for (int64_t e = 0; e < c->E; e++)
            for (int n = 0; n < 8; n++) soa[(size_t)n * c->Epad + e] = d->lnid[8 * e + n];
        if ((rc = c->d_lnid.put(&c->bytes, soa, c->stream)) != HQ_OK ||
            (rc = c->d_c1.put(&c->bytes, prep.c1.data(), (size_t)c->E, c->stream)) != HQ_OK ||
            (rc = c->d_c2.put(&c->bytes, prep.c2.data(), (size_t)c->E, c->stream)) != HQ_OK ||
            (rc = c->d_beta.put(&c->bytes, prep.beta.data(), (size_t)c->E, c->stream)) != HQ_OK)
            return bail(rc);
        if ((rc = hq_build_schedule(c, &d->an_sched, &c->an)) != HQ_OK) return bail(rc);
        if ((rc = hq_build_schedule(c, &d->dn_sched, &c->dn)) != HQ_OK) return bail(rc);
        if (c->ldnnum) {
            std::vector<int32_t> sd;
            for (int32_t k = 0; k < c->ldnnum; k++)
                for (int32_t a = d->dn_ptr[k]; a < d->dn_ptr[k + 1]; a++) {
// ... 591 lines not shown
            return hq_fail(HQ_ERR_COMM, "IPC transport: %s waits for a neighbour's halo records timed out (HQ_IPC_TIMEOUT_MS)", n);
        }
    }
    if (c->debug_halo) {
        int32_t bad = 0;
        HQ_TRY(hq_copy_wait(&bad, c->d_halo_err, sizeof bad, hipMemcpyDeviceToHost, c->stream));
        if (bad) {
            char n[32];
            snprintf(n, sizeof n, "%d", bad);
            HQ_HIP(hipMemsetAsync(c->d_halo_err, 0, sizeof(int32_t), c->stream));
            HQ_HIP(hipStreamSynchronize(c->stream));
            return hq_fail(HQ_ERR_COMM, "HQ_DEBUG_HALO: %s halo records arrived for another node than the schedule names "
                                        "(global node ids do not match, psolve.c:5058-5069)", n);
        }
    }
    return HQ_OK;
}

extern "C" int hq_check_finite(hq_ctx* c, int64_t* nonfinite)
{
    if (!c || !nonfinite) return hq_fail(HQ_ERR_ARG, "null argument%s", "");
    HQ_HIP(hipSetDevice(c->device));
    HQ_HIP(hq_quiesce(c));
    HQ_HIP(hipMemsetAsync(c->d_halo_err + 1, 0, sizeof(int32_t), c->stream));
    const int64_t n3 = 3 * (int64_t)c->N;
    const hq_real* arr[2] = { c->d_u[c->now], c->d_u[c->prev] };
    for (const hq_real* a : arr)
        if (a) hq_k_count_nonfinite<<<2048, 256, 0, c->stream>>>(n3, a, c->d_halo_err + 1);
    if (c->d_force) hq_k_count_nonfinite<<<2048, 256, 0, c->stream>>>(n3, (const double*)c->d_force, c->d_halo_err + 1);
    int32_t bad = 0;
    HQ_HIP(hipMemcpyAsync(&bad, c->d_halo_err + 1, sizeof bad, hipMemcpyDeviceToHost, c->stream));
    HQ_HIP(hipStreamSynchronize(c->stream));
    *nonfinite = bad;
    return HQ_OK;
}

extern "C" int hq_run_timed(hq_ctx* c, int32_t nsteps, double* total_ms, double* kernel_ms_avg)
{
    if (!c || nsteps <= 0) return hq_fail(HQ_ERR_ARG, "bad argument%s", "");
    HQ_TRY(hq_output_check_room(c, nsteps));
    HQ_HIP(hipSetDevice(c->device));
    size_t need = 2 * (size_t)nsteps;
    while (c->ev.size() < need) {
        hipEvent_t e;
        HQ_HIP(hipEventCreate(&e));
        c->ev.push_back(e);
    }
    for (int k = 0; k < 2; k++)
        if (!c->ev_span[k]) HQ_HIP(hipEventCreate(&c->ev_span[k]));
    HQ_HIP(hq_quiesce(c));
    hq_clock_harvest_all(c, true);
    const double clk_us0 = c->clk_us[0];
    const int64_t clk_n0 = c->clk_steps;
    c->ev_used = 0;
    HQ_HIP(hipEventRecord(c->ev_span[0], c->stream));
    c->timing = true;
    int rc = HQ_OK;
    for (int32_t s = 0; s < nsteps && rc == HQ_OK; s++) rc = hq_step(c);
    c->timing = false;
    if (c->overlap) hipStreamWaitEvent(c->stream, c->ev_shared, 0);
    if (c->bstream) hipStreamWaitEvent(c->stream, c->ev_bricks, 0);
    hipEventRecord(c->ev_span[1], c->stream);
    hipError_t he = hq_quiesce(c);
    if (he == hipSuccess) hq_clock_harvest_all(c, true);
    double tot = 0, ker = 0;
    if (rc == HQ_OK && he == hipSuccess) {
        float ms = 0;
        hipEventElapsedTime(&ms, c->ev_span[0], c->ev_span[1]);
        tot = ms;
        for (size_t i = 0; i + 1 < c->ev_used; i += 2) {
            hipEventElapsedTime(&ms, c->ev[i], c->ev[i + 1]);
            ker += ms;
        }
        if (c->ev_used >= 2) ker /= (double)(c->ev_used / 2);
        if (c->bstream && c->clk_steps > clk_n0) ker = (c->clk_us[0] - clk_us0) / (double)(c->clk_steps - clk_n0) * 1e-3;
    }
    if (rc != HQ_OK) return rc;
    if (he != hipSuccess) return hq_fail(HQ_ERR_DEVICE, "timed run failed: %s", hipGetErrorString(he));
    if (total_ms) *total_ms = tot;
    if (kernel_ms_avg) *kernel_ms_avg = ker;
    return HQ_OK;
}

extern "C" const char* hq_dominant_kernel(hq_ctx* c)
{
    if (!c || c->variant != HQ_VARIANT_PATCH) return "hq_k_element_scatter";
    if (2 * c->bricks.nb > (int64_t)c->N) return "hq_k_brick";
    if (2 * c->plan.nstencil > c->plan.npatches) return "hq_k_patch_stencil";
    if (!hq_patch_uses_pers(&c->plan)) return "hq_k_patch_step";
    return c->plan.seeded ? "hq_k_patch_seed" : "hq_k_patch_pers";
}

static int hq_gather_impl(hq_ctx* c, int32_t n, const int32_t* lnid, hq_real* o1, hq_real* o2, hq_real* o3);

extern "C" int hq_gather(hq_ctx* c, int32_t n, const int32_t* lnid, hq_real* o1, hq_real* o2)
{
    return hq_gather_impl(c, n, lnid, o1, o2, nullptr);
}

extern "C" int hq_gather3(hq_ctx* c, int32_t n, const int32_t* lnid, hq_real* o1, hq_real* o2, hq_real* o3)
{
    if (c && o3 && c->variant != HQ_VARIANT_PATCH)
        return hq_fail(HQ_ERR_STATE, "u(t - 2 dt) is kept by the patch variant only%s", "");
    return hq_gather_impl(c, n, lnid, o1, o2, o3);
}

static int hq_gather_impl(hq_ctx* c, int32_t n, const int32_t* lnid, hq_real* o1, hq_real* o2, hq_real* o3)
{
    if (!c || n < 0 || (n && !lnid)) return hq_fail(HQ_ERR_ARG, "bad argument%s", "");
    if (n == 0) return HQ_OK;
    HQ_HIP(hipSetDevice(c->device));
    HQ_HIP(hq_quiesce(c));
    for (int32_t i = 0; i < n; i++)
        if (lnid[i] < 0 || lnid[i] >= c->N) return hq_fail(HQ_ERR_ARG, "node id out of range%s", "");
    if (n > c->gather_cap) {
        c->gather_cap = 0;
        const int32_t cap = std::max(n, 1024);
        HQ_TRY(c->d_gather_ids.alloc(nullptr, (size_t)cap));
        HQ_TRY(c->d_gather_out.alloc(nullptr, 9 * (size_t)cap));
        c->gather_cap = cap;
    }
    int32_t* d_ids = c->d_gather_ids;
    hq_real* d_o = c->d_gather_out;
    hipError_t e;
    c->h2d_bytes += 4 * (int64_t)n;
    c->d2h_bytes += 3 * (int64_t)sizeof(hq_real) * (int64_t)n * ((o1 ? 1 : 0) + (o2 ? 1 : 0) + (o3 ? 1 : 0));
    std::vector<int32_t> dev_ids;
    if (!c->perm.empty()) {
        dev_ids.resize((size_t)n);
        for (int32_t i = 0; i < n; i++) dev_ids[(size_t)i] = c->perm[(size_t)lnid[i]];
        lnid = dev_ids.data();
    }
    hipMemcpyAsync(d_ids, lnid, sizeof(int32_t) * n, hipMemcpyHostToDevice, c->stream);
    hq_k_gather<<<hq_blocks((int64_t)n * 3, 256), 256, 0, c->stream>>>(n, d_ids, c->d_u[c->now], c->d_u[c->prev],
                                                                         d_o, d_o + 3 * (size_t)n);
    if (o1) hipMemcpyAsync(o1, d_o, sizeof(hq_real) * 3 * n, hipMemcpyDeviceToHost, c->stream);
    if (o2) hipMemcpyAsync(o2, d_o + 3 * (size_t)n, sizeof(hq_real) * 3 * n, hipMemcpyDeviceToHost, c->stream);
    if (o3) {
        hq_k_gather<<<hq_blocks((int64_t)n * 3, 256), 256, 0, c->stream>>>(n, d_ids, c->d_u[c->spare], c->d_u[c->spare],
                                                                             d_o + 6 * (size_t)n, d_o + 6 * (size_t)n);
        hipMemcpyAsync(o3, d_o + 6 * (size_t)n, sizeof(hq_real) * 3 * n, hipMemcpyDeviceToHost, c->stream);
    }
    e = hq_quiesce(c);
    if (e != hipSuccess) return hq_fail(HQ_ERR_DEVICE, "gather failed: %s", hipGetErrorString(e));
    return HQ_OK;
}

extern "C" int hq_download(hq_ctx* c, hq_real* tm1, hq_real* tm2)
{
    if (!c) return hq_fail(HQ_ERR_ARG, "null argument%s", "");
    HQ_HIP(hipSetDevice(c->device));
    HQ_HIP(hq_quiesce(c));
    if (tm1) HQ_TRY(hq_field_to_host(c, c->d_u[c->now], tm1));
    if (tm2) HQ_TRY(hq_field_to_host(c, c->d_u[c->prev], tm2));
    return HQ_OK;
}

extern "C" int hq_upload(hq_ctx* c, const hq_real* tm1, const hq_real* tm2, int32_t step)
{
    if (!c || !tm1 || !tm2) return hq_fail(HQ_ERR_ARG, "null argument%s", "");
    HQ_HIP(hipSetDevice(c->device));
    HQ_HIP(hq_quiesce(c));
    size_t bytes = sizeof(hq_real) * 3 * (size_t)c->N;
    HQ_TRY(hq_field_to_device(c, tm1, c->d_u[c->now]));
    HQ_TRY(hq_field_to_device(c, tm2, c->d_u[c->prev]));
    if (c->d_u[2]) {
// ... 39 lines not shown
```

### hercules_amd/csrc/hq_opts.h

```cpp
#ifndef HQ_OPTS_H
#define HQ_OPTS_H

#include <cstddef>
#include <cstdlib>
#include <cstring>

struct hq_opt_entry { const char* env; size_t off; int kind; };

#define HQ_OPT_I(env_, field_) { env_, offsetof(hq_options, field_), 0 }
#define HQ_OPT_D(env_, field_) { env_, offsetof(hq_options, field_), 1 }
static const hq_opt_entry g_opt_table[] = {
    HQ_OPT_I("HQ_NO_BRICKS", no_bricks), HQ_OPT_I("HQ_BRICK_CZ", brick_cz), HQ_OPT_I("HQ_BRICK_MINZ", brick_minz),
    HQ_OPT_I("HQ_BRICK_MINNODES", brick_minnodes), HQ_OPT_I("HQ_BRICK_NO_HET", brick_no_het),
    HQ_OPT_I("HQ_BRICK_NO_NTSAME", brick_no_ntsame), HQ_OPT_I("HQ_BRICK_BY_COMPONENT", brick_by_component),
    HQ_OPT_I("HQ_BRICK_STREAM", brick_stream), HQ_OPT_I("HQ_BRICK_NO_FACES", brick_no_faces), HQ_OPT_I("HQ_BRICK_HALF_TILES", brick_half_tiles), HQ_OPT_I("HQ_BRICK_NO_PACK", brick_no_pack), HQ_OPT_I("HQ_PATCH_PIPE", patch_pipe), HQ_OPT_I("HQ_PATCH_THREADS", patch_threads),
    HQ_OPT_I("HQ_PATCH_PMAX", patch_pmax), HQ_OPT_I("HQ_PATCH_PMERGE", patch_pmerge), HQ_OPT_I("HQ_PATCH_PSPLIT", patch_psplit),
    HQ_OPT_I("HQ_PATCH_NLMAX", patch_nlmax), HQ_OPT_I("HQ_PATCH_VMAX", patch_vmax), HQ_OPT_I("HQ_PATCH_RAGGED", patch_ragged),
    HQ_OPT_I("HQ_PATCH_NO_LATTICE", patch_no_lattice), HQ_OPT_I("HQ_PATCH_NO_STENCIL", patch_no_stencil),
    HQ_OPT_I("HQ_PATCH_NO_UNIFORM", patch_no_uniform), HQ_OPT_I("HQ_PATCH_NO_ISO", patch_no_iso),
    HQ_OPT_I("HQ_PATCH_NO_NTSAME", patch_no_ntsame), HQ_OPT_I("HQ_PATCH_NO_DEDUP", patch_no_dedup),
    HQ_OPT_I("HQ_PATCH_WFORM", patch_wform), HQ_OPT_I("HQ_PATCH_MERGE_ROUNDS", patch_merge_rounds),
    HQ_OPT_I("HQ_OVERLAP", overlap), HQ_OPT_I("HQ_NO_OVERLAP", no_overlap), HQ_OPT_I("HQ_RESERVE_CUS", reserve_cus),
    HQ_OPT_I("HQ_CU_MASK", cu_mask), HQ_OPT_I("HQ_NO_FUSED_SHARE", no_fused_share), HQ_OPT_I("HQ_GROUP_COPIES", group_copies),
    HQ_OPT_I("HQ_DEBUG_HALO", debug_halo), HQ_OPT_I("HQ_IPC_ARENA", ipc_arena), HQ_OPT_D("HQ_IPC_TIMEOUT_MS", ipc_timeout_ms),
    HQ_OPT_D("HQ_LOOPBACK_DELAY_US", loopback_delay_us), HQ_OPT_I("HQ_PATCH_VERBOSE", verbose), HQ_OPT_I("HQ_QUIET", quiet),
    HQ_OPT_I("HQ_BRICK_RAGGED", brick_ragged), HQ_OPT_I("HQ_BRICK_RAGGED_MINFILL", brick_ragged_minfill),
    HQ_OPT_I("HQ_PHASE_TIMING", phase_timing), HQ_OPT_I("HQ_BRICK_RAGGED_HET", brick_ragged_het),
};
#undef HQ_OPT_I
#undef HQ_OPT_D

static void hq_options_defaults(hq_options* o)
{
    o->size = sizeof(hq_options);
    for (const hq_opt_entry& e : g_opt_table) {
        if (e.kind == 0) *(int32_t*)((char*)o + e.off) = -1;
        else *(double*)((char*)o + e.off) = -1.0;
    }
    o->allow_env = -1;
    o->reserved0 = -1;
}

static void hq_options_adopt(hq_options* dst, const hq_options* src)
{
    hq_options_defaults(dst);
    if (!src) return;
    const size_t n = (size_t)(src->size < sizeof(hq_options) ? src->size : sizeof(hq_options));
    if (n > sizeof(uint64_t)) memcpy((char*)dst + sizeof(uint64_t), (const char*)src + sizeof(uint64_t), n - sizeof(uint64_t));
    dst->size = sizeof(hq_options);
}

static int hq_opt_env_int(const char* env, const char* v)
{
    if (!strcmp(env, "HQ_IPC_ARENA")) return !strcmp(v, "fine") ? 0 : (!strcmp(v, "uncached") ? 1 : (!strcmp(v, "coarse") ? 2 : atoi(v)));
    if (!*v) return 1;
    return atoi(v);
}

static void hq_options_resolve(hq_options* out, const hq_options* caller)
{
    hq_options_adopt(out, caller);
    const char* master = getenv("HQ_ALLOW_ENV");
    const bool allow = out->allow_env >= 0 ? out->allow_env != 0 : (master && *master && strcmp(master, "0") != 0);
    out->allow_env = allow ? 1 : 0;
    if (!allow) return;
    for (const hq_opt_entry& e : g_opt_table) {
        const char* v = getenv(e.env);
        if (!v) continue;
        if (e.kind == 0) *(int32_t*)((char*)out + e.off) = hq_opt_env_int(e.env, v);
        else if (*v) *(double*)((char*)out + e.off) = atof(v);
    }
}

template <typename T> static inline bool hq_given(T f) { return f >= 0; }
template <typename T> static inline T hq_value_or(T f, T def) { return f >= 0 ? f : def; }
template <typename T> static inline bool hq_set(T f) { return f > 0; }

static inline const char* hq_opt_env_only(const hq_options& o, const char* env)
{
    return o.allow_env == 1 ? getenv(env) : nullptr;
}

#endif
```

### hercules_amd/csrc/hq_patch.h

```cpp
#ifndef HQ_PATCH_H
#define HQ_PATCH_H

#ifdef _OPENMP
#include <omp.h>
#else
static inline int omp_get_num_threads(void) { return 1; }
static inline int omp_get_thread_num(void) { return 0; }
#endif
#include <hip/hip_runtime.h>
#include <stdint.h>

#include <algorithm>
#include <chrono>
#include <array>
#include <string>
#include <unordered_map>
#include <vector>
#include <cstring>

#include "hq_kernels.h"
#include "hq_opts.h"

#define HQ_PATCH_MAX_THREADS 512

// ... 739 lines not shown
                    ent[p].push_back(dn.anchor[a] - D.base);
                    ent[p].push_back(deps);
                }
            }
            H->ds_ptr.assign((size_t)P + 1, 0);
            for (int32_t p = 0; p < P; p++) {
                H->ds_ptr[p + 1] = H->ds_ptr[p] + (int32_t)(ent[p].size() / 3);
                H->ds_ent.insert(H->ds_ent.end(), ent[p].begin(), ent[p].end());
            }
        }
        return 0;
    }
    g_patch_err = "patch refinement did not converge";
    return -1;
}


#define HQ_PIDX_UNPACK(l, raw)                                                                  \
    l[0] = (raw).x & HQ_PIDX_ROW; l[1] = ((raw).x >> 16) & HQ_PIDX_ROW;                          \
    l[2] = (raw).y & HQ_PIDX_ROW; l[3] = ((raw).y >> 16) & HQ_PIDX_ROW;                          \
    l[4] = (raw).z & HQ_PIDX_ROW; l[5] = ((raw).z >> 16) & HQ_PIDX_ROW;                          \
    l[6] = (raw).w & HQ_PIDX_ROW; l[7] = ((raw).w >> 16) & HQ_PIDX_ROW;
#define HQ_PIDX_WORD(raw, n) ((n) < 2 ? (raw).x : (n) < 4 ? (raw).y : (n) < 6 ? (raw).z : (raw).w)
#define HQ_PIDX_HAS_ACC(raw, n) ((HQ_PIDX_WORD(raw, n) & (((n) & 1) ? (HQ_PIDX_ACC << 16) : HQ_PIDX_ACC)) != 0)

struct hq_pair_data {
    uint4 raw;
    double beta, c1, c2;
};

#ifdef HQ_PATCH_PROFILING
__device__ unsigned long long* g_hq_stamps = nullptr;
__device__ unsigned long long* g_hq_wg = nullptr;
#define HQ_WG_STAMP(k) do { if (threadIdx.x == 0 && g_hq_wg) g_hq_wg[2 * blockIdx.x + (k)] = __builtin_amdgcn_s_memrealtime(); } while (0)
static void hq_patch_report_stamps(const struct hq_patch_plan* P);
#define HQ_STAMP(k) do { if (DIAG == 6 && threadIdx.x == 0 && g_hq_stamps) g_hq_stamps[8 * (size_t)p + (k)] = __builtin_amdgcn_s_memtime(); } while (0)
#ifndef HQ_STAMP_TID
#define HQ_STAMP_TID 0
#endif
#define HQ_STAMPD(k) do { if (tid0 == HQ_STAMP_TID && p0 >= 0 && g_hq_stamps) g_hq_stamps[8 * (size_t)p0 + (k)] = __builtin_amdgcn_s_memtime(); } while (0)
#else
#define HQ_STAMP(k) do { } while (0)
#define HQ_STAMPD(k) do { } while (0)
#define HQ_WG_STAMP(k) do { } while (0)
#endif

typedef unsigned int hq_u32x4 __attribute__((ext_vector_type(4)));

__device__ __forceinline__ hq_pair_data hq_pair_load(const uint4* __restrict__ pidx, const double* __restrict__ pc1,
                                                     const double* __restrict__ pc2,
                                                     const double* __restrict__ pbeta, int64_t gi, int64_t gc)
{
    hq_pair_data d;
    hq_u32x4 r = reinterpret_cast<const hq_u32x4*>(pidx)[gi];
    d.raw.x = r.x; d.raw.y = r.y; d.raw.z = r.z; d.raw.w = r.w;
    d.beta = pbeta[gc];
    d.c1 = pc1[gc];
    d.c2 = pc2[gc];
    return d;
}

template <int DIAG>
__global__ void __launch_bounds__(HQ_PATCH_MAX_THREADS, 4)
hq_k_patch_step(int32_t npatches, int32_t per_xcd, const int32_t* __restrict__ order, int32_t nlmax,
                const hq_patch_desc* __restrict__ desc,
                const uint4* __restrict__ pidx, const double* __restrict__ pc1,
                const double* __restrict__ pc2, const double* __restrict__ pbeta,
                const int32_t* __restrict__ halo, const hq_real* __restrict__ u1g,
                const hq_real* __restrict__ u2g, hq_real* __restrict__ ung,
                const double* __restrict__ nt, const double* __restrict__ nt3,
                const int32_t* __restrict__ src_ptr,
                const int32_t* __restrict__ src_ent, const double* __restrict__ F, double dt2,
                const int32_t* __restrict__ if_ptr, const int32_t* __restrict__ if_ent,
                double* __restrict__ iforce, const int32_t* __restrict__ ds_ptr,
                const int32_t* __restrict__ ds_ent, int32_t hstride)
{
    extern __shared__ __align__(16) double s_mem[];
    double* __restrict__ s_u1 = s_mem;
    double* __restrict__ s_u2 = s_mem + 3 * nlmax;
    double* __restrict__ s_f = s_mem + 6 * nlmax;

    const int slot = (int)(blockIdx.x & 7) * per_xcd + (int)(blockIdx.x >> 3);
    if (slot >= npatches) return;
    const int p = order ? order[slot] : slot;
    const int tid = threadIdx.x, T = blockDim.x;
    HQ_STAMP(0);
    const int32_t* __restrict__ hl = halo + (int64_t)p * hstride;
    int32_t hid[4];
#pragma unroll
    for (int k = 0; k < 4; k++) hid[k] = hl[(k * T + tid) / 3];
    const hq_patch_desc D = desc[p];
    const int own3 = D.nown * 3, halo3 = D.nhalo * 3;
    for (int i = own3 + tid; i < 3 * D.nacc; i += T) s_f[i] = 0.0;
    if (DIAG == 6 && D.nown > 0) HQ_STAMP(1);

    const bool wf = (D.flags & HQ_PATCH_WFORM) != 0;
    const double wbeta = wf ? pbeta[D.pair_off] : 0.0;
    const int o2off = 3 * (nlmax / 2);
    hq_pair_data cur;
    const int cstep = (D.flags & HQ_PATCH_UNIFORM) ? 0 : 1;
    if (tid < D.npairs) cur = hq_pair_load(pidx, pc1, pc2, pbeta, D.pidx_off + tid, D.pair_off + cstep * tid);

    {
        const hq_real* g1 = u1g + 3 * (int64_t)D.base;
        const hq_real* g2 = u2g + 3 * (int64_t)D.base;
        for (int i0 = 0; i0 < own3 || i0 < halo3; i0 += 4 * T) {
            double a1[4], a2[4], b1[4], b2[4];
#pragma unroll
            for (int k = 0; k < 4; k++) {
                int i = i0 + k * T + tid;
                if (DIAG == 2) { a1[k] = a2[k] = b1[k] = b2[k] = 1e-3 * i; continue; }
                if (i < own3) { a1[k] = g1[i]; a2[k] = g2[i]; }
                if (i < halo3) {
                    int h = i / 3, d = i - 3 * h;
                    int32_t id = hid[k];
                    if (i0 > 0) id = hl[h];
                    int64_t g = 3 * (int64_t)id + d;
                    b1[k] = u1g[g]; b2[k] = u2g[g];
                }
            }
#pragma unroll
            for (int k = 0; k < 4; k++) {
                int i = i0 + k * T + tid;
                if (wf) {
                    if (i < own3) { s_u1[i] = a1[k] + wbeta * (a1[k] - a2[k]); s_u2[i] = a1[k]; s_u2[o2off + i] = a2[k]; s_f[i] = 0.0; }
                    if (i < halo3) s_u1[own3 + i] = b1[k] + wbeta * (b1[k] - b2[k]);
                } else {
                    if (i < own3) { s_u1[i] = a1[k]; s_u2[i] = a2[k]; s_f[i] = 0.0; }
                    if (i < halo3) { s_u1[own3 + i] = b1[k]; s_u2[own3 + i] = b2[k]; }
                }
            }
        }
    }
    HQ_STAMP(2);
    __syncthreads();
    HQ_STAMP(3);

    const bool iso = (D.flags & HQ_PATCH_ISO) != 0;
    double np[7];
    if (tid < D.nown) {
        if (iso) {
            const double* q = nt3 + 3 * ((int64_t)D.base + ((D.flags & HQ_PATCH_NTSAME) ? 0 : tid));
            np[0] = q[0];
            np[1] = q[1];
            np[4] = q[2];
        } else {
            const double* q = nt + 7 * ((int64_t)D.base + tid);
#pragma unroll
            for (int k = 0; k < 7; k++) np[k] = q[k];
        }
    }

    for (int q = tid; q < (DIAG == 1 ? 0 : D.npairs); q += T) {
        hq_pair_data nxt;
        if (q + T < D.npairs)
            nxt = hq_pair_load(pidx, pc1, pc2, pbeta, D.pidx_off + q + T, D.pair_off + cstep * (q + T));
        const uint4 raw = cur.raw;
        const double beta = cur.beta;
        int l[8];
        HQ_PIDX_UNPACK(l, raw)
        double X[8], Y[8], Z[8];
        if (wf) {
#pragma unroll
            for (int n = 0; n < 8; n++) {
                const double* a = &s_u1[3 * (DIAG == 5 ? (tid & 7) : l[n])];
                X[n] = a[0]; Y[n] = a[1]; Z[n] = a[2];
            }
        } else {
#pragma unroll
            for (int n = 0; n < 8; n++) {
                const double* a = &s_u1[3 * (DIAG == 5 ? (tid & 7) : l[n])];
                const double* b = &s_u2[3 * (DIAG == 5 ? (tid & 7) : l[n])];
                double a0 = a[0], a1 = a[1], a2 = a[2];
                X[n] = a0 + beta * (a0 - b[0]);
                Y[n] = a1 + beta * (a1 - b[1]);
                Z[n] = a2 + beta * (a2 - b[2]);
            }
        }
        hq_element_force(X, Y, Z, cur.c1, cur.c2);
#pragma unroll
        for (int n = 0; n < 8; n++) {
            if (DIAG == 4) { if (X[n] + Y[n] + Z[n] == 1.2345e-300) s_f[n] = 1.0; continue; }
            if (HQ_PIDX_HAS_ACC(raw, n)) {
                atomicAdd(&s_f[3 * l[n] + 0], X[n]);
                atomicAdd(&s_f[3 * l[n] + 1], Y[n]);
                atomicAdd(&s_f[3 * l[n] + 2], Z[n]);
            }
        }
        cur = nxt;
    }
    HQ_STAMP(4);
    if (F) {
        for (int k = src_ptr[p] + tid; k < src_ptr[p + 1]; k += T) {
            int ln = src_ent[2 * k], li = src_ent[2 * k + 1];
            for (int d = 0; d < 3; d++) atomicAdd(&s_f[3 * ln + d], F[3 * li + d] * dt2);
        }
    }
    if (ds_ptr && ds_ptr[p + 1] > ds_ptr[p]) {
        __syncthreads();
        for (int k = ds_ptr[p] + tid; k < ds_ptr[p + 1]; k += T) {
            const int src = ds_ent[3 * k], dst = ds_ent[3 * k + 1];
            const double deps = (double)(unsigned)ds_ent[3 * k + 2];
            for (int d = 0; d < 3; d++) atomicAdd(&s_f[3 * dst + d], s_f[3 * src + d] / deps);
        }
    }
    __syncthreads();
    HQ_STAMP(5);

    for (int n = tid; n < (DIAG == 3 ? (tid == 0 ? 1 : 0) : D.nown); n += T) {
        if (n != tid) {
            if (iso) {
                const double* q = nt3 + 3 * ((int64_t)D.base + ((D.flags & HQ_PATCH_NTSAME) ? 0 : n));
                np[0] = q[0]; np[1] = q[1]; np[4] = q[2];
            } else {
                const double* q = nt + 7 * ((int64_t)D.base + n);
#pragma unroll
                for (int k = 0; k < 7; k++) np[k] = q[k];
            }
        }
        hq_real* out = ung + 3 * ((int64_t)D.base + n);
#pragma unroll
        for (int d = 0; d < 3; d++) {
            const double m2 = iso ? np[1] : np[1 + d], m1 = iso ? np[4] : np[4 + d];
            const double x1 = wf ? s_u2[3 * n + d] : s_u1[3 * n + d], x2 = wf ? s_u2[o2off + 3 * n + d] : s_u2[3 * n + d];
            double f = s_f[3 * n + d] + (m2 * x1 - m1 * x2);
            out[d] = f / np[0];
        }
    }
    if (if_ptr) {
        for (int k = if_ptr[p] + tid; k < if_ptr[p + 1]; k += T) {
            int ln = if_ent[2 * k];
            double* o = iforce + 3 * (int64_t)if_ent[2 * k + 1];
            o[0] = s_f[3 * ln]; o[1] = s_f[3 * ln + 1]; o[2] = s_f[3 * ln + 2];
        }
    }
    HQ_STAMP(6);
}

__device__ __forceinline__ hq_patch_desc hq_patch_desc_or_empty(const hq_patch_desc* __restrict__ desc, int p)
{
    hq_patch_desc D = desc[p < 0 ? 0 : p];
    if (p < 0) { D.nown = 0; D.nhalo = 0; D.npairs = 0; D.nacc = 0; D.flags = 0; }
    return D;
}

#define HQ_PERS_THREADS 1024
#ifndef HQ_TICKET_STRIDE
#define HQ_TICKET_STRIDE 64
#endif
typedef __attribute__((address_space(3))) double hq_lds_double;
#define HQ_LDS_ADD(p, v) __hip_atomic_fetch_add((p), (v), __ATOMIC_RELAXED, __HIP_MEMORY_SCOPE_WORKGROUP)
static __device__ __forceinline__ hq_lds_double* hq_lds_row3(hq_lds_double* base, int i) {
    unsigned b = (unsigned)(__SIZE_TYPE__)base, o;
    asm("v_mad_u32_u24 %0, %1, 24, %2" : "=v"(o) : "v"(i), "v"(b));
    return (hq_lds_double*)(__SIZE_TYPE__)o;
}

__global__ void __launch_bounds__(HQ_PERS_THREADS)
hq_k_patch_pers(int32_t count, int32_t per_xcd, const int32_t* __restrict__ order, int32_t nrows,
                int32_t nfacc, const hq_patch_desc* __restrict__ desc,
                const uint4* __restrict__ pidx, const double* __restrict__ pc1,
                const double* __restrict__ pc2, const double* __restrict__ pbeta,
                const int32_t* __restrict__ halo, const hq_real* __restrict__ u1g,
                const hq_real* __restrict__ u2g, hq_real* __restrict__ ung,
                const double* __restrict__ nt, const double* __restrict__ nt3,
                const int32_t* __restrict__ src_ptr, const int32_t* __restrict__ src_ent,
                const double* __restrict__ F, double dt2, const int32_t* __restrict__ if_ptr,
                const int32_t* __restrict__ if_ent, double* __restrict__ iforce,
                const int32_t* __restrict__ ds_ptr, const int32_t* __restrict__ ds_ent, int32_t hstride,
                int32_t* __restrict__ tickets, const uint16_t* __restrict__ lat_row)
{
    extern __shared__ __align__(16) double s_mem[];
    double* __restrict__ s_fg = s_mem + 12 * nrows;
    int32_t* __restrict__ s_tick = reinterpret_cast<int32_t*>(s_fg + nfacc);
    const int tid0 = threadIdx.x, T = HQ_PERS_THREADS;
    const int W = (int)(gridDim.x >> 3), xcd = (int)(blockIdx.x & 7);
    const int end = min((xcd + 1) * per_xcd, count);
    HQ_WG_STAMP(0);
#define HQ_SLOT_PATCH(s) ((s) < end ? (order ? order[(s)] : (s)) : -1)
#define HQ_DRAW() (xcd * per_xcd + atomicAdd(&tickets[HQ_TICKET_STRIDE * xcd], 1))
#define HQ_PERS_ID(P_, DD) \
    ((tid >= (DD).nown && tid < (DD).nown + (DD).nhalo) ? halo[(int64_t)(P_) * hstride + (tid - (DD).nown)] : 0)

    if (tid0 == 0) { for (int i = 0; i < 5; i++) s_tick[i] = HQ_DRAW(); }
    int lrow0 = lat_row ? (int)lat_row[tid0] : tid0;
    __syncthreads();
    const int sl0 = __builtin_amdgcn_readfirstlane(s_tick[0]), sl1 = __builtin_amdgcn_readfirstlane(s_tick[1]),
              sl2 = __builtin_amdgcn_readfirstlane(s_tick[2]);
    int p0 = HQ_SLOT_PATCH(sl0), p1 = HQ_SLOT_PATCH(sl1), p2 = HQ_SLOT_PATCH(sl2);
#define HQ_PERS_EXIT()                                                                          \
    {                                                                                           \
        if (tid0 == 0 && atomicAdd(&tickets[HQ_TICKET_STRIDE * xcd + 1], 1) == W - 1) {    \
            tickets[HQ_TICKET_STRIDE * xcd] = 0;                                                \
            tickets[HQ_TICKET_STRIDE * xcd + 1] = 0;                                            \
        }                                                                                       \
        HQ_WG_STAMP(1);                                                                         \
    }
    if (p0 < 0) {
        HQ_PERS_EXIT()
        return;
    }
    hq_patch_desc D0 = hq_patch_desc_or_empty(desc, p0);
    hq_patch_desc D1 = hq_patch_desc_or_empty(desc, p1);
    hq_patch_desc D2 = hq_patch_desc_or_empty(desc, p2);
    hq_u32x4 c_raw = { 0, 0, 0, 0 };
    double c_beta = 0.0, c_c1 = 0.0, c_c2 = 0.0;
    int32_t idn;
#define HQ_PERS_ROW(DD)                                                                         \
    {                                                                                           \
        const int q_ = tid < (DD).npairs ? tid : 0;                                             \
        const int64_t gc_ = (DD).pair_off + (((DD).flags & HQ_PATCH_UNIFORM) ? 0 : q_);         \
        c_raw = *(reinterpret_cast<const hq_u32x4*>(pidx) + ((DD).pidx_off + q_));              \
        c_beta = pbeta[gc_]; c_c1 = pc1[gc_]; c_c2 = pc2[gc_];                                  \
    }
    {
        const int tid = tid0;
        for (int i = tid; i < nfacc; i += T) s_fg[i] = 0.0;
        HQ_PERS_ROW(D0)
        const int32_t id0 = HQ_PERS_ID(p0, D0);
// ... 973 lines not shown
static int hq_patch_set_interface(const hq_options& o, hq_patch_plan* P, const int32_t* slot, int64_t nnodes, int64_t* ledger, hipStream_t st)
{
    std::vector<int32_t> ptr((size_t)P->npatches + 1, 0), ent;
    for (int32_t p = 0; p < P->npatches; p++) {
        for (int32_t n = 0; n < P->patch_nown[p]; n++) {
            int32_t sl = slot[P->patch_base[p] + n];
            if (sl >= 0) { ent.push_back(P->patch_lat[p] ? (int32_t)hq_lattice().row_of_local[n] : n); ent.push_back(sl); }
        }
        ptr[p + 1] = (int32_t)(ent.size() / 2);
    }
    if (ent.empty()) return HQ_OK;
    bool any_st_if = false;
    for (int32_t p = 0; p < P->npatches; p++)
        if (ptr[p + 1] > ptr[p] && (P->h_flags[p] & HQ_PATCH_STENCIL)) {
            if (o.patch_ragged == 2) { P->h_flags[p] &= ~(HQ_PATCH_STENCIL | HQ_PATCH_RAGGED); continue; }
            P->h_flags[p] |= HQ_PATCH_RAGGED;
            any_st_if = true;
        }
    P->d_if_slot.reset();
    if (any_st_if) HQ_TRY(P->d_if_slot.put(ledger, slot, (size_t)nnodes, st));
    HQ_TRY(hq_patch_build_order(P, ptr.data(), ledger, st));
    HQ_TRY(P->d_if_ptr.put(ledger, ptr, st));
    return P->d_if_ent.put(ledger, ent, st);
}

#ifdef HQ_PATCH_PROFILING
static unsigned long long* g_hq_stamp_buf = nullptr;
static unsigned long long* g_hq_wg_buf = nullptr;
static int32_t g_hq_stamp_n = 0;
static void hq_patch_report_stamps(const hq_patch_plan* P)
{
    if (!g_hq_stamp_buf) return;
    std::vector<unsigned long long> h((size_t)g_hq_stamp_n * 8);
    hipDeviceSynchronize();
    hipMemcpy(h.data(), g_hq_stamp_buf, 64 * (size_t)g_hq_stamp_n, hipMemcpyDeviceToHost);
    const int pipe_ = P->pipe == 0 ? 0 : (P->pipe == 6 ? 6 : 4);
    const char* name0[6] = { "descriptor", "issue+wait staging, LDS write", "barrier 1", "element loop", "src/ds + barrier 2", "update + stores issued" };
    const char* name4[6] = { "row wait + node loads issued", "element section", "row/n_t loads, src/ds, barrier", "wait node data, LDS write", "update + stores issued", "barrier" };
    const char* name6[6] = { "node requests issued, descriptor", "gather + arithmetic", "row/n_t requests, atomics, image + seeds", "barrier", "update + stores issued", "-" };
    const char** name = pipe_ == 4 ? name4 : (pipe_ == 6 ? name6 : name0);
    double sum[6] = { 0, 0, 0, 0, 0, 0 };
    long cnt = 0;
    for (int32_t p = 0; p < g_hq_stamp_n; p++) {
        const unsigned long long* s = &h[8 * (size_t)p];
        if (!s[6] || !s[0]) continue;
        for (int k = 0; k < 6; k++) sum[k] += (double)(s[k + 1] - s[k]);
        cnt++;
    }
    if ((pipe_ == 4 || pipe_ == 6) && g_hq_wg_buf) {
        unsigned long long w[512];
        hipMemcpy(w, g_hq_wg_buf, sizeof w, hipMemcpyDeviceToHost);
        unsigned long long t0 = ~0ull, t1 = 0; double me = 0; int c = 0;
        for (int i = 0; i < 256; i++) if (w[2 * i] && w[2 * i + 1]) { if (w[2 * i] < t0) t0 = w[2 * i]; if (w[2 * i + 1] > t1) t1 = w[2 * i + 1]; c++; }
        for (int i = 0; i < 256; i++) if (w[2 * i] && w[2 * i + 1]) me += (double)(w[2 * i + 1] - t0);
        if (c) fprintf(stderr, "  workgroups of the last launch: %d; first start -> last exit %.1f us, mean exit at %.1f us "
                       "(the mean workgroup idles %.1f %% at the end)\n", c, (double)(t1 - t0) / 100.0, me / c / 100.0,
                       100.0 * ((double)(t1 - t0) - me / c) / (double)(t1 - t0));
    }
    if (pipe_ == 4 || pipe_ == 6) {
        double pre = 0; long c7 = 0;
        for (int32_t p = 0; p < g_hq_stamp_n; p++) {
            const unsigned long long* s = &h[8 * (size_t)p];
            if (!s[6] || !s[0] || !s[7]) continue;
            pre += (double)(s[7] - s[0]); c7++;
        }
        fprintf(stderr, "  (of the first phase, up to and including the issue of the node loads: %.0f)\n", pre / (c7 ? c7 : 1));
    }
    fprintf(stderr, "hq patch stamps (mean shader cycles per workgroup over %ld patches, last step):\n", cnt);
    double tot = 0;
    for (int k = 0; k < 6; k++) tot += sum[k] / (cnt ? cnt : 1);
    for (int k = 0; k < 6; k++) fprintf(stderr, "  %-34s %9.0f  (%4.1f %%)\n", name[k], sum[k] / (cnt ? cnt : 1), 100.0 * sum[k] / (cnt ? cnt : 1) / tot);
    fprintf(stderr, "  %-34s %9.0f\n", "total", tot);
}
#endif


static bool hq_patch_uses_pers(const hq_patch_plan* P)
{
    if (P->pipe != 4 && P->pipe != 6) return false;
    if (P->cfg.nlmax > HQ_PERS_THREADS || P->max_npairs > HQ_PERS_THREADS) return false;
    return (12 * (size_t)P->nrows + 3 * (size_t)(P->cfg.pmax + P->cfg.vmax) + 36) * sizeof(double) <= 160 * 1024;
}

static void hq_patch_launch(const hq_patch_plan* P, int32_t first, int32_t count, const hq_real* u1,
                            const hq_real* u2, hq_real* un, const double* nt, const double* F, double dt2,
                            double* iforce, hipStream_t stream, int reserve_cus = 0)
{
    if (count <= 0) return;
#ifdef HQ_EXPERIMENT
    if (getenv("HQ_X_NO_SHELL")) return;
#endif
    int per_xcd = (count + 7) / 8;
    const int32_t step_nl = P->step_nl > 0 ? P->step_nl : P->cfg.nlmax;
    const int32_t step_na = P->step_nl > 0 && P->max_nacc > 0 ? P->max_nacc : P->cfg.pmax + P->cfg.vmax;
    size_t lds = (6 * (size_t)step_nl + 3 * (size_t)step_na) * sizeof(double);
#ifdef HQ_PATCH_PROFILING
    const int diag = getenv("HQ_PATCH_DIAG") ? atoi(getenv("HQ_PATCH_DIAG")) : 0;
    if (diag == 6) {
        static unsigned long long* d_st = nullptr;
        if (!d_st) {
            hipMalloc((void**)&d_st, 64 * (size_t)P->npatches);
            hipMemset(d_st, 0, 64 * (size_t)P->npatches);
            hipMemcpyToSymbol(HIP_SYMBOL(g_hq_stamps), &d_st, sizeof d_st);
            g_hq_stamp_buf = d_st; g_hq_stamp_n = P->npatches;
            hipMalloc((void**)&g_hq_wg_buf, 16 * 256);
            hipMemset(g_hq_wg_buf, 0, 16 * 256);
            hipMemcpyToSymbol(HIP_SYMBOL(g_hq_wg), &g_hq_wg_buf, sizeof g_hq_wg_buf);
        }
    }
#endif
    if (hq_patch_uses_pers(P)) {
        const int32_t nfacc = 3 * (P->cfg.pmax + P->cfg.vmax);
        size_t lds4 = (12 * (size_t)P->nrows + (size_t)nfacc + 4) * sizeof(double);
        {
            int grid = std::max(8, P->grid_cus - (reserve_cus & ~7));
            while (grid > 8 && (grid >> 3) > per_xcd) grid -= 8;
            if (P->seeded) {
                const int32_t nfa = 3 * P->max_nacc;
                const size_t ldss = (12 * (size_t)P->nrows + 3 * (size_t)nfa + 4) * sizeof(double);
                hq_k_patch_seed<<<grid, HQ_PERS_THREADS, ldss, stream>>>(
                    count, per_xcd, P->d_order ? P->d_order + first : nullptr, P->nrows, nfa, P->d_desc, P->d_pidx,
                    P->d_pc1, P->d_pc2, P->d_pbeta, P->d_halo, u1, u2, un, nt, P->d_nt3, P->d_src_ptr, P->d_src_ent,
                    (P->d_src_ptr ? F : nullptr), dt2, P->d_if_ptr, P->d_if_ent, iforce, P->d_ds_ptr, P->d_ds_ent,
                    P->hstride, P->d_tickets, P->d_lat_row);
                return;
            }
            hq_k_patch_pers<<<grid, HQ_PERS_THREADS, lds4, stream>>>(
                count, per_xcd, P->d_order ? P->d_order + first : nullptr, P->nrows, nfacc, P->d_desc, P->d_pidx,
                P->d_pc1, P->d_pc2, P->d_pbeta, P->d_halo, u1, u2, un, nt, P->d_nt3, P->d_src_ptr, P->d_src_ent,
                (P->d_src_ptr ? F : nullptr), dt2, P->d_if_ptr, P->d_if_ent, iforce, P->d_ds_ptr, P->d_ds_ent,
                P->hstride, P->d_tickets, P->d_lat_row);
            return;
        }
    }
    auto kern = hq_k_patch_step<0>;
#ifdef HQ_PATCH_PROFILING
    if (diag == 1) kern = hq_k_patch_step<1>;
    if (diag == 2) kern = hq_k_patch_step<2>;
    if (diag == 3) kern = hq_k_patch_step<3>;
    if (diag == 4) kern = hq_k_patch_step<4>;
    if (diag == 5) kern = hq_k_patch_step<5>;
    if (diag == 6) kern = hq_k_patch_step<6>;
#endif
    kern<<<per_xcd * 8, P->cfg.threads, lds, stream>>>(
        count, per_xcd, P->d_order ? P->d_order + first : nullptr, step_nl, P->d_desc, P->d_pidx, P->d_pc1,
        P->d_pc2, P->d_pbeta, P->d_halo, u1, u2, un, nt, P->d_nt3, P->d_src_ptr, P->d_src_ent,
        (P->d_src_ptr ? F : nullptr), dt2, P->d_if_ptr, P->d_if_ent, iforce, P->d_ds_ptr, P->d_ds_ent,
        P->hstride);
}

static void hq_patch_launch_stencil(const hq_patch_plan* P, int part, const hq_real* u1, const hq_real* u2, hq_real* un,
                                    const double* nt, const double* F, double dt2, double* iforce, hipStream_t stream)
{
    const int32_t total = part == 0 ? P->nr : P->ns, nbig = part == 0 ? P->nr_big : P->ns_big;
    const int32_t nrg = part == 0 ? total - nbig : P->ns_rg;
    const int64_t first = part == 0 ? 0 : P->nr;
    const int32_t cnt[3] = { total - nbig - nrg, nrg, nbig };
    int64_t e0 = first;
    for (int k = 0; k < 3; k++) {
        const int32_t count = cnt[k];
        if (count <= 0) continue;
        const int per_xcd = (count + 7) / 8;
        const size_t lds = k == 0 ? 0 : HQ_ST_LDS_RAGGED;
#define HQ_ST_ARGS count, per_xcd, P->d_st_desc + e0, P->d_st_halo + e0 * HQ_ST_HSTRIDE, u1, u2, un, nt, P->d_nt3, P->d_src_ptr,  \
        P->d_src_ent, (P->d_src_ptr ? F : nullptr), dt2, P->d_rg_tab, P->d_E1, P->d_E2,                                             \
        part == 0 ? P->d_if_slot : nullptr, iforce, P->d_lat_row, hq_stencil().c
        if (k < 2) hq_k_patch_stencil<HQ_ST_THREADS><<<per_xcd * 8, HQ_ST_THREADS, lds, stream>>>(HQ_ST_ARGS);
        else hq_k_patch_stencil<768><<<per_xcd * 8, 768, lds, stream>>>(HQ_ST_ARGS);
#undef HQ_ST_ARGS
        e0 += count;
    }
}

#endif
```

### include/hq_solver.h

```cpp
#ifndef HQ_SOLVER_H
#define HQ_SOLVER_H

#include <stdint.h>

#ifdef __cplusplus
extern "C" {
#endif

#define HQ_API __attribute__((visibility("default")))

typedef struct hq_ctx hq_ctx;

typedef enum {
    HQ_OK            =  0,
    HQ_ERR_ARG       = -1,
    HQ_ERR_NOMEM     = -2,
    HQ_ERR_DEVICE    = -3,
    HQ_ERR_NODEVICE  = -4,
    HQ_ERR_COMM      = -5,
    HQ_ERR_STATE     = -6
} hq_status;

enum {
    HQ_VARIANT_AUTO    = 0,
// ... 49 lines not shown
typedef struct {
    int32_t variant;
    int32_t npatches;
    int64_t patch_pairs;
    int64_t device_bytes;
    int32_t step;
    int32_t nranks;
    int32_t lattice_patches;
    int32_t stencil_patches;
    int32_t ragged_patches;
    int32_t brick_units;
    int64_t brick_nodes;
    int32_t brick_units_pernode;
    int32_t brick_units_het;
    int64_t pcie_h2d_bytes;
    int64_t pcie_d2h_bytes;
    int32_t transport;
    int32_t ipc_arena_coarse;
    int32_t ipc_arena_kind;
    int32_t debug_halo;
    int32_t brick_units_packed;
    int32_t brick_units_ragged;
    int32_t brick_stream;
    int32_t brick_units_ragged_het;
    int64_t timed_steps;
    double  t_step_us;
    double  t_shell_us;
    double  t_interior_us;
    double  t_chain_us;
    double  t_chain_exposed_us;
} hq_info;

HQ_API int hq_device_count(void);

HQ_API const char* hq_last_error(void);

HQ_API int hq_create(const hq_desc* desc, int device, hq_ctx** out);

typedef struct {
    uint64_t size;
    int32_t no_bricks;
    int32_t brick_cz;
    int32_t brick_minz;
    int32_t brick_minnodes;
    int32_t brick_no_het;
    int32_t brick_no_ntsame;
    int32_t brick_by_component;
    int32_t brick_stream;
    int32_t brick_no_faces;
    int32_t brick_half_tiles;
    int32_t brick_no_pack;
    int32_t patch_pipe;
    int32_t patch_threads;
    int32_t patch_pmax;
    int32_t patch_pmerge;
    int32_t patch_psplit;
    int32_t patch_nlmax;
    int32_t patch_vmax;
    int32_t patch_ragged;
    int32_t patch_no_lattice;
    int32_t patch_no_stencil;
    int32_t patch_no_uniform;
    int32_t patch_no_iso;
    int32_t patch_no_ntsame;
    int32_t patch_no_dedup;
    int32_t patch_wform;
    int32_t patch_merge_rounds;
    int32_t overlap;
    int32_t no_overlap;
    int32_t reserve_cus;
    int32_t cu_mask;
    int32_t no_fused_share;
    int32_t group_copies;
    int32_t debug_halo;
    int32_t ipc_arena;
    double  ipc_timeout_ms;
    double  loopback_delay_us;
    int32_t verbose;
    int32_t quiet;
    int32_t brick_ragged;
    int32_t brick_ragged_minfill;
    int32_t allow_env;
    int32_t brick_ragged_het;
    int32_t reserved0;
    int32_t phase_timing;
} hq_options;

HQ_API void hq_options_init(hq_options* opts, uint64_t size);
HQ_API int  hq_create_opts(const hq_desc* desc, int device, const hq_options* opts, hq_ctx** out);
HQ_API int  hq_get_options(hq_ctx* ctx, hq_options* out, uint64_t size);

HQ_API int hq_destroy(hq_ctx* ctx);

#define HQ_ABI_VERSION 6
HQ_API int hq_abi_version(void);
HQ_API int hq_real_bytes(void);
HQ_API int hq_get_info_sized(hq_ctx* ctx, hq_info* info, uint64_t size);
HQ_API int hq_get_info(hq_ctx* ctx, hq_info* info);
#ifndef HQ_SOLVER_IMPLEMENTATION
#define hq_get_info(ctx, info) hq_get_info_sized((ctx), (info), (uint64_t)sizeof(hq_info))
#endif

HQ_API int hq_comm_unique_id(void* id128);
HQ_API int hq_comm_init(hq_ctx* ctx, const void* id128);
HQ_API int hq_comm_selftest(hq_ctx* ctx, int32_t count);

typedef int (*hq_host_exchange_fn)(void* user, int32_t nrecv, const int32_t* recv_peer, const int64_t* recv_count,
                                   double* const* recv_buf, int32_t nsend, const int32_t* send_peer,
                                   const int64_t* send_count, const double* const* send_buf, int32_t tag);
HQ_API int hq_comm_init_host(hq_ctx* ctx, hq_host_exchange_fn fn, void* user);

#define HQ_IPC_BLOB_BYTES 4096
HQ_API int hq_comm_ipc_export(hq_ctx* ctx, void* blob);
HQ_API int hq_comm_init_ipc(hq_ctx* ctx, const void* all_blobs);
HQ_API int hq_comm_init_ipc_n(hq_ctx* ctx, const void* all_blobs, int32_t nblobs);
HQ_API int hq_comm_init_loopback(hq_ctx* ctx);

HQ_API int hq_group_link(hq_ctx** ctxs, int32_t n);
HQ_API int hq_group_run(hq_ctx** ctxs, int32_t n, int32_t nsteps);

HQ_API int hq_set_source(hq_ctx* ctx, int32_t nloaded, const int32_t* loaded_lnid,
                         int32_t step0, int32_t nsteps, const double* F);

HQ_API int hq_run(hq_ctx* ctx, int32_t nsteps);

HQ_API int hq_sync(hq_ctx* ctx);

HQ_API int hq_check_finite(hq_ctx* ctx, int64_t* nonfinite);

HQ_API int hq_gather(hq_ctx* ctx, int32_t n, const int32_t* lnid, hq_real* tm1_out, hq_real* tm2_out);
HQ_API int hq_gather3(hq_ctx* ctx, int32_t n, const int32_t* lnid, hq_real* tm1_out, hq_real* tm2_out,
                      hq_real* tm3_out);
HQ_API int hq_download(hq_ctx* ctx, hq_real* tm1, hq_real* tm2);
HQ_API int hq_upload(hq_ctx* ctx, const hq_real* tm1, const hq_real* tm2, int32_t step);

typedef struct {
    int32_t        npoints;
    const int32_t* ids;
    const double*  phi;
    int32_t        rate;
    int32_t        derivs;
    int32_t        capacity;
} hq_recorder_desc;
HQ_API int hq_record_add(hq_ctx* ctx, const hq_recorder_desc* desc, int32_t* handle);
HQ_API int hq_record_pending(hq_ctx* ctx, int32_t handle, int32_t* nsamples, int32_t* first_step);
HQ_API int hq_record_fetch(hq_ctx* ctx, int32_t handle, int32_t max_samples, double* out, int32_t* steps,
                           int32_t* nfetched);
HQ_API int hq_record_clear(hq_ctx* ctx);

enum { HQ_SNAP_TM1 = 1, HQ_SNAP_TM2 = 2, HQ_SNAP_VEL = 4 };
typedef struct {
    int32_t first, count;
    int32_t rate;
    int32_t first_step;
    int32_t fields;
    int32_t slots;
} hq_snapshot_desc;
HQ_API int hq_snapshot_add(hq_ctx* ctx, const hq_snapshot_desc* desc, int32_t* handle);
HQ_API int hq_snapshot_pending(hq_ctx* ctx, int32_t handle, int32_t* npending, int32_t* nready, int32_t* first_step);
HQ_API int hq_snapshot_fetch(hq_ctx* ctx, int32_t handle, hq_real* tm1, hq_real* tm2, double* vel, int32_t* step);
HQ_API int hq_snapshot_clear(hq_ctx* ctx);

enum { HQ_PEAK_DISP = 1, HQ_PEAK_VEL = 2, HQ_PEAK_ACC = 4 };
typedef struct {
    int32_t        npoints;
    int32_t        nodes_per_point;
    const int32_t* ids;
    const double*  phi;
    int32_t        rate, first_step;
    int32_t        quantities;
    int32_t        reserved;
} hq_peak_desc;
HQ_API int hq_peak_add(hq_ctx* ctx, const hq_peak_desc* desc, int32_t* handle);
HQ_API int hq_peak_fetch(hq_ctx* ctx, int32_t handle, double* peaks, int32_t* when, int64_t* nsamples);
HQ_API int hq_peak_load(hq_ctx* ctx, int32_t handle, const double* peaks, const int32_t* when, int64_t nsamples);
HQ_API int hq_peak_reset(hq_ctx* ctx, int32_t handle);
HQ_API int hq_peak_clear(hq_ctx* ctx);

enum { HQ_SPEC_MAX_PERIODS = 32, HQ_SPEC_NVAL = 4 };
typedef struct {
    int32_t        npoints;
    int32_t        nodes_per_point;
    const int32_t* ids;
    const double*  phi;
    int32_t        rate, first_step;
    int32_t        nperiods;
    int32_t        reserved;
    const double*  periods;
    double         damping;
} hq_spec_desc;
HQ_API int hq_spec_add(hq_ctx* ctx, const hq_spec_desc* desc, int32_t* handle);
HQ_API int hq_spec_coefficients(hq_ctx* ctx, int32_t handle, double* coef);
HQ_API int hq_spec_fetch(hq_ctx* ctx, int32_t handle, double* sd, double* osc, double* aprev, int64_t* nsamples);
HQ_API int hq_spec_load(hq_ctx* ctx, int32_t handle, const double* sd, const double* osc, const double* aprev, int64_t nsamples);
HQ_API int hq_spec_reset(hq_ctx* ctx, int32_t handle);
HQ_API int hq_spec_clear(hq_ctx* ctx);

typedef struct {
    int32_t        npoints;
    int32_t        nodes_per_point;
    const int32_t* ids;
    const double*  phi;
    int32_t        rate, first_step;
    int32_t        quantities;
    int32_t        husid_every, husid_slots;
    int32_t        reserved;
    double         threshold[3];
} hq_cum_desc;
HQ_API int hq_cum_add(hq_ctx* ctx, const hq_cum_desc* desc, int32_t* handle);
HQ_API int hq_cum_fetch(hq_ctx* ctx, int32_t handle, double* sums, int32_t* span, double* curve, int32_t* curve_steps,
                        int32_t* nfilled, int64_t* nsamples);
HQ_API int hq_cum_load(hq_ctx* ctx, int32_t handle, const double* sums, const int32_t* span, const double* curve,
                       const int32_t* curve_steps, int32_t nfilled, int64_t nsamples);
HQ_API int hq_cum_reset(hq_ctx* ctx, int32_t handle);
HQ_API int hq_cum_clear(hq_ctx* ctx);

HQ_API int hq_phase_force(hq_ctx* ctx);
HQ_API int hq_phase_update(hq_ctx* ctx);
HQ_API int hq_download_force(hq_ctx* ctx, double* force);

HQ_API int hq_run_timed(hq_ctx* ctx, int32_t nsteps, double* total_ms, double* kernel_ms_avg);

HQ_API int hq_plan_check(const hq_desc* desc, int64_t report[8]);

HQ_API int hq_stencil_plan_check(const hq_desc* desc, int64_t report[6]);

HQ_API int hq_brick_plan_check(const hq_desc* desc, int64_t report[8]);
HQ_API int hq_brick_plan_check_n(const hq_desc* desc, int64_t* report, int32_t n);

HQ_API int hq_stencil_coefficients(double out[16]);

HQ_API const char* hq_dominant_kernel(hq_ctx* ctx);

#ifdef __cplusplus
}
#endif
#endif
```

Before: 68.50 billion.

## Fuse brick interior march and patch shell step into one kernel launch

Moves the brick march body and the patch step body into shared include files so one kernel, hq_k_brick_shell, can run either body per workgroup. Workgroups are assigned to brick units or shell patches according to a placement mode (first, last or spread). The aim is to remove a separate launch and let the shell and interior work run concurrently on the CUs. It adds a fused_step option and query, uses dynamic LDS sized for the larger of the two bodies, and may lower occupancy or unbalance the load across workgroups.

After: 66.53 billion. 0.971x the previous value.

```diff
diff --git a/hercules_amd/build.py b/hercules_amd/build.py
--- a/hercules_amd/build.py
+++ b/hercules_amd/build.py
@@ -20,7 +20,7 @@
 
 def _build_solver(lib, defines, force):
     srcs = [os.path.join(CSRC, f) for f in ("hq_engine.hip", "hq_devmem.h", "hq_kernels.h", "hq_opts.h", "hq_patch.h",
-                                           "hq_brick.h", "hq_prepare.h", "hq_plan_check.h", "hq_cadence.h", "hq_peak.h", "hq_cumul.h", "hq_sample.h", "hq_sdof.h",
+                                           "hq_patch_step.inc", "hq_brick.h", "hq_brick_march.inc", "hq_prepare.h", "hq_plan_check.h", "hq_cadence.h", "hq_peak.h", "hq_cumul.h", "hq_sample.h", "hq_sdof.h",
                                            "hq_outputs.h")]
     srcs.append(os.path.join(ROOT, "include", "hq_solver.h"))
     if force or _newer(lib, srcs):
diff --git a/hercules_amd/capi.py b/hercules_amd/capi.py
--- a/hercules_amd/capi.py
+++ b/hercules_amd/capi.py
@@ -13,7 +13,7 @@
            "hq_options_init", "hq_create_opts", "hq_get_options", "hq_real_bytes",
            "hq_comm_unique_id", "hq_comm_init", "hq_comm_selftest", "hq_group_link", "hq_group_run", "hq_set_source", "hq_run", "hq_sync", "hq_gather", "hq_gather3",
            "hq_download", "hq_upload", "hq_phase_force", "hq_phase_update", "hq_download_force",
-           "hq_run_timed", "hq_dominant_kernel", "hq_plan_check", "hq_stencil_plan_check", "hq_check_finite",
+           "hq_run_timed", "hq_dominant_kernel", "hq_fused_step", "hq_plan_check", "hq_stencil_plan_check", "hq_check_finite",
            "hq_stencil_coefficients", "hq_brick_plan_check", "hq_brick_plan_check_n", "hq_comm_init_host",
            "hq_comm_ipc_export", "hq_comm_init_ipc", "hq_comm_init_loopback",
            "hq_record_add", "hq_record_pending", "hq_record_fetch", "hq_record_clear",
@@ -117,7 +117,7 @@
                 [("ipc_timeout_ms", ctypes.c_double), ("loopback_delay_us", ctypes.c_double),
                  ("verbose", ctypes.c_int32), ("quiet", ctypes.c_int32),
                  ("brick_ragged", ctypes.c_int32), ("brick_ragged_minfill", ctypes.c_int32),
-                 ("allow_env", ctypes.c_int32), ("brick_ragged_het", ctypes.c_int32), ("reserved0", ctypes.c_int32),
+                 ("allow_env", ctypes.c_int32), ("brick_ragged_het", ctypes.c_int32), ("fused_step", ctypes.c_int32),
                  ("phase_timing", ctypes.c_int32)])
 
     def __init__(self, **kw):
@@ -328,6 +328,9 @@
     def dominant_kernel(self):
         return self._lib.hq_dominant_kernel(self._h).decode()
 
+    def fused_step(self):
+        return int(self._lib.hq_fused_step(self._h))
+
     def download(self, want_tm2=True):
         tm1 = np.empty((self.N, 3), self.real)
         tm2 = np.empty((self.N, 3), self.real) if want_tm2 else None
diff --git a/hercules_amd/csrc/hq_brick.h b/hercules_amd/csrc/hq_brick.h
--- a/hercules_amd/csrc/hq_brick.h
+++ b/hercules_amd/csrc/hq_brick.h
@@ -776,189 +776,70 @@
     __shared__ __align__(16) double s_w[2 * 3 * HQ_BK_PLANE];
     const int slot = (int)(blockIdx.x & 7) * per_xcd + (int)(blockIdx.x >> 3);
     if (slot >= count) return;
-    const hq_brick_unit U = units[slot];
-    const int nx = U.nx, ny = U.ny, np = U.np, nxy = nx * ny, nr = 2 * (nx + 2) + 2 * ny;
-    const int t = threadIdx.x, lx = t & (HQ_BK_TX - 1), ly = t >> 6;
-    const bool active = lx < nx && ly < ny;
-    const int sidx = active ? ly * nx + lx : 0;
-    const int myrow = (ly + 1) * HQ_BK_PY + lx + 1;
-    const bool ring = t < nr;
-    int rrow;
-    {
-        int rx, ry;
-        if (t < nx + 2) { rx = t - 1; ry = -1; }
-        else if (t < 2 * (nx + 2)) { rx = t - (nx + 2) - 1; ry = ny; }
-        else if (t < 2 * (nx + 2) + ny) { rx = -1; ry = t - 2 * (nx + 2); }
-        else { rx = nx; ry = t - 2 * (nx + 2) - ny; }
-        rrow = (ry + 1) * HQ_BK_PY + rx + 1;
-    }
-    const int32_t* __restrict__ utab = tab + U.tab;
-    const int rofs = ring ? t : 0;
-    const int32_t* __restrict__ cap = utab + (int64_t)(np + 2) * nr;
-    int32_t vOut = -1, vMid = RAGGED ? cap[sidx] : 0, vCur = RAGGED ? cap[nxy + sidx] : 0, vNext = 0;
-    const int32_t id_lo = RAGGED ? (vMid >= 0 ? vMid : -vMid - 2) : cap[sidx];
-    const double beta = U.beta;
-    double P[6], Q[2];
-#pragma unroll
-    for (int i = 0; i < 6; i++) P[i] = hq_uniform(U.c1 * sc.p1[i] + U.c2 * sc.p2[i]);
-#pragma unroll
-    for (int i = 0; i < 2; i++) Q[i] = hq_uniform(U.c1 * sc.q1[i] + U.c2 * sc.q2[i]);
-    const bool has_src = F && src_ptr[slot + 1] > src_ptr[slot];
-
-    hq_real x1[3] = { 0, 0, 0 }, x2[3] = { 0, 0, 0 }, y1[3] = { 0, 0, 0 }, y2[3] = { 0, 0, 0 };
-    double mn[3] = { U.m0, U.m2, U.m1 };
-    double m0A = hq_uniform(1.0 / U.m0), m0B = m0A;
-    double fA[3] = { 0.0, 0.0, 0.0 }, fB[3] = { 0.0, 0.0, 0.0 };
-    int32_t rid = utab[rofs];
-
-#define HQ_BK_LOAD(node_)                                                                             \
-    {                                                                                                 \
-        const int64_t a_ = (node_);                                                                   \
-        if (active && (!RAGGED || a_ >= 0)) {                                                         \
-            _Pragma("unroll") for (int d = 0; d < 3; d++) { x1[d] = u1g[3 * a_ + d]; x2[d] = u2g[3 * a_ + d]; } \
-            if (PERNODE) { _Pragma("unroll") for (int d = 0; d < 3; d++) mn[d] = nt3[3 * a_ + d]; }    \
-        }                                                                                             \
-        if (ring && (!RAGGED || rid >= 0)) {                                                          \
-            const int64_t b_ = (int64_t)rid;                                                          \
-            _Pragma("unroll") for (int d = 0; d < 3; d++) { y1[d] = u1g[3 * b_ + d]; y2[d] = u2g[3 * b_ + d]; } \
-        }                                                                                             \
-    }
-#define HQ_BK_PUT(s_, acc_, M2_, M1_)                                                                 \
-    {                                                                                                 \
-        hq_lds_double* img_ = (hq_lds_double*)s_w + 3 * HQ_BK_PLANE * (s_);                            \
-        if (active) {                                                                                 \
-            _Pragma("unroll") for (int d = 0; d < 3; d++) {                                           \
-                const double a1_ = x1[d], a2_ = x2[d];                                                \
-                img_[3 * myrow + d] = a1_ + beta * (a1_ - a2_);                                       \
-                acc_[d] += (M2_) * a1_ - (M1_) * a2_;                                                 \
-            }                                                                                         \
-        }                                                                                             \
-        if (ring) { _Pragma("unroll") for (int d = 0; d < 3; d++) { const double b1_ = y1[d], b2_ = y2[d]; img_[3 * rrow + d] = b1_ + beta * (b1_ - b2_); } } \
-    }
-
-    const bool topf = !PERNODE && !RAGGED && (U.flags & HQ_BK_TOPFACE) != 0, botf = !PERNODE && !RAGGED && (U.flags & HQ_BK_BOTFACE) != 0;
-    const double rho = hq_uniform((U.c1 - U.c2) / (U.c1 + U.c2));
-
-    HQ_BK_LOAD((int64_t)id_lo)
-    rid = utab[nr + rofs];
-    if (topf) HQ_BK_PUT(0, fB, U.ft[1 + d], U.ft[4 + d])
-    else { double dummy[3] = { 0.0, 0.0, 0.0 }; HQ_BK_PUT(0, dummy, mn[1], mn[2]) }
-    for (int k = 0; k <= np + 1; k++) {
-        if (k <= np) {
-            if (RAGGED) {
-                HQ_BK_LOAD((int64_t)(vCur >= 0 ? vCur : -vCur - 2))
-                if (k < np) vNext = cap[(k + 2) * nxy + sidx];
-            } else HQ_BK_LOAD(k == np ? (int64_t)cap[nxy + sidx] : U.base + (int64_t)k * nxy + sidx)
-            if (k < np) rid = utab[(k + 2) * nr + rofs];
-        }
-        __syncthreads();
-        const hq_lds_double* __restrict__ q = (const hq_lds_double*)s_w + 3 * (HQ_BK_PLANE * (k & 1) + myrow);
-        double m[3], g[3], Uo[3];
-        if (BYCOMP) {
-            double A_x, A_y;
-            {
-                const double C = q[2], XM = q[2 - 3], XP = q[2 + 3], YM = q[2 - 3 * HQ_BK_PY], YP = q[2 + 3 * HQ_BK_PY];
-                const double MM = q[2 - 3 * HQ_BK_PY - 3], PM = q[2 - 3 * HQ_BK_PY + 3], MP = q[2 + 3 * HQ_BK_PY - 3], PP = q[2 + 3 * HQ_BK_PY + 3];
-                const double sxy = (XM + XP) + (YM + YP), dg = (MM + PP) + (PM + MP);
-                m[2] = fma(P[0], C, fma(P[2], sxy, P[4] * dg));
-                g[2] = fma(P[1], C, fma(P[3], sxy, P[5] * dg));
-                Uo[0] = fma(Q[0], XP - XM, Q[1] * ((PP - MP) + (PM - MM)));
-                Uo[1] = fma(Q[0], YP - YM, Q[1] * ((PP - PM) + (MP - MM)));
-            }
-            __builtin_amdgcn_sched_barrier(0);
-            {
-                const double C = q[0], XM = q[0 - 3], XP = q[0 + 3], YM = q[0 - 3 * HQ_BK_PY], YP = q[0 + 3 * HQ_BK_PY];
-                const double MM = q[0 - 3 * HQ_BK_PY - 3], PM = q[0 - 3 * HQ_BK_PY + 3], MP = q[0 + 3 * HQ_BK_PY - 3], PP = q[0 + 3 * HQ_BK_PY + 3];
-                const double sx = XM + XP, sy = YM + YP, dg = (MM + PP) + (PM + MP);
-                A_x = (PP + MM) - (PM + MP);
-                m[0] = fma(P[0], C, fma(P[1], sx, fma(P[2], sy, P[3] * dg)));
-                g[0] = fma(P[2], C, fma(P[3], sx, fma(P[4], sy, P[5] * dg)));
-                Uo[2] = fma(Q[0], XP - XM, Q[1] * ((PP - MP) + (PM - MM)));
-            }
-            __builtin_amdgcn_sched_barrier(0);
-            {
-                const double C = q[1], XM = q[1 - 3], XP = q[1 + 3], YM = q[1 - 3 * HQ_BK_PY], YP = q[1 + 3 * HQ_BK_PY];
-                const double MM = q[1 - 3 * HQ_BK_PY - 3], PM = q[1 - 3 * HQ_BK_PY + 3], MP = q[1 + 3 * HQ_BK_PY - 3], PP = q[1 + 3 * HQ_BK_PY + 3];
-                const double sx = XM + XP, sy = YM + YP, dg = (MM + PP) + (PM + MP);
-                A_y = (PP + MM) - (PM + MP);
-                m[1] = fma(P[0], C, fma(P[1], sy, fma(P[2], sx, fma(P[3], dg, Q[0] * A_x))));
-                g[1] = fma(P[2], C, fma(P[3], sy, fma(P[4], sx, fma(P[5], dg, Q[1] * A_x))));
-                Uo[2] += fma(Q[0], YP - YM, Q[1] * ((PP - PM) + (MP - MM)));
-            }
-            m[0] = fma(Q[0], A_y, m[0]);
-            g[0] = fma(Q[1], A_y, g[0]);
-        } else {
-            double C[3], XM[3], XP[3], YM[3], YP[3], MM[3], PM[3], MP[3], PP[3];
-#pragma unroll
-            for (int d = 0; d < 3; d++) {
-                C[d] = q[d]; XM[d] = q[d - 3]; XP[d] = q[d + 3]; YM[d] = q[d - 3 * HQ_BK_PY]; YP[d] = q[d + 3 * HQ_BK_PY];
-                MM[d] = q[d - 3 * HQ_BK_PY - 3]; PM[d] = q[d - 3 * HQ_BK_PY + 3];
-                MP[d] = q[d + 3 * HQ_BK_PY - 3]; PP[d] = q[d + 3 * HQ_BK_PY + 3];
-            }
-            double sx[3], sy[3], dg[3];
-#pragma unroll
-            for (int d = 0; d < 3; d++) { sx[d] = XM[d] + XP[d]; sy[d] = YM[d] + YP[d]; dg[d] = (MM[d] + PP[d]) + (PM[d] + MP[d]); }
-            const double A_x = (PP[0] + MM[0]) - (PM[0] + MP[0]), A_y = (PP[1] + MM[1]) - (PM[1] + MP[1]);
-            const double Bx0_z = XP[2] - XM[2], Bx0_x = XP[0] - XM[0], By0_z = YP[2] - YM[2], By0_y = YP[1] - YM[1];
-            const double Bx1_z = (PP[2] - MP[2]) + (PM[2] - MM[2]), Bx1_x = (PP[0] - MP[0]) + (PM[0] - MM[0]);
-            const double By1_z = (PP[2] - PM[2]) + (MP[2] - MM[2]), By1_y = (PP[1] - PM[1]) + (MP[1] - MM[1]);
-            const double sxy_z = sx[2] + sy[2];
-            m[0] = fma(P[0], C[0], fma(P[1], sx[0], fma(P[2], sy[0], fma(P[3], dg[0], Q[0] * A_y))));
-            m[1] = fma(P[0], C[1], fma(P[1], sy[1], fma(P[2], sx[1], fma(P[3], dg[1], Q[0] * A_x))));
-            m[2] = fma(P[0], C[2], fma(P[2], sxy_z, P[4] * dg[2]));
-            g[0] = fma(P[2], C[0], fma(P[3], sx[0], fma(P[4], sy[0], fma(P[5], dg[0], Q[1] * A_y))));
-            g[1] = fma(P[2], C[1], fma(P[3], sy[1], fma(P[4], sx[1], fma(P[5], dg[1], Q[1] * A_x))));
-            g[2] = fma(P[1], C[2], fma(P[3], sxy_z, P[5] * dg[2]));
-            Uo[0] = fma(Q[0], Bx0_z, Q[1] * Bx1_z);
-            Uo[1] = fma(Q[0], By0_z, Q[1] * By1_z);
-            Uo[2] = fma(Q[0], Bx0_x, fma(Q[1], Bx1_x, fma(Q[0], By0_y, Q[1] * By1_y)));
-        }
-        if (k == 0 && topf) {
-            m[0] = fma(rho, Uo[0], 0.5 * m[0]); m[1] = fma(rho, Uo[1], 0.5 * m[1]); m[2] = fma(-rho, Uo[2], 0.5 * m[2]);
-        }
-        if (k == np + 1 && botf && active) {
-            double f[3];
-            f[0] = fB[0] + fma(-rho, Uo[0], 0.5 * m[0]); f[1] = fB[1] + fma(-rho, Uo[1], 0.5 * m[1]); f[2] = fB[2] + fma(rho, Uo[2], 0.5 * m[2]);
-            const int local = np * nxy + sidx;
-            if (has_src) {
-                for (int i = src_ptr[slot]; i < src_ptr[slot + 1]; i++)
-                    if (src_ent[2 * i] == local) {
-                        const int li = src_ent[2 * i + 1];
-                        for (int d = 0; d < 3; d++) f[d] += F[3 * li + d] * dt2;
-                    }
-            }
-            hq_real* out = ung + 3 * (int64_t)cap[nxy + sidx];
-            const double rm = 1.0 / U.fb[0];
-#pragma unroll
-            for (int d = 0; d < 3; d++) out[d] = f[d] * rm;
-        }
-        const bool outface = k == 1 && topf;
-        if ((k >= 2 || outface) && active && (!RAGGED || vOut >= 0)) {
-            double f[3];
-#pragma unroll
-            for (int d = 0; d < 3; d++) f[d] = fA[d] + (g[d] + Uo[d]);
-            const int local = RAGGED ? (int)(vOut - U.base) : (k - 2) * nxy + sidx;
-            if (has_src) {
-                for (int i = src_ptr[slot]; i < src_ptr[slot + 1]; i++)
-                    if (src_ent[2 * i] == local) {
-                        const int li = src_ent[2 * i + 1];
-                        for (int d = 0; d < 3; d++) f[d] += F[3 * li + d] * dt2;
-                    }
-            }
-            hq_real* out = ung + 3 * (RAGGED ? (int64_t)vOut : (outface ? (int64_t)cap[sidx] : U.base + (int64_t)local));
-            const double rm = outface ? 1.0 / U.ft[0] : m0A;
-#pragma unroll
-            for (int d = 0; d < 3; d++) out[d] = f[d] * rm;
-        }
-#pragma unroll
-        for (int d = 0; d < 3; d++) { fA[d] = fB[d] + m[d]; fB[d] = g[d] - Uo[d]; }
-        if (RAGGED) { vOut = vMid; vMid = vCur; vCur = vNext; }
-        if (PERNODE) { m0A = m0B; m0B = 1.0 / mn[0]; }
-        if (k < np || (k == np && !botf)) HQ_BK_PUT((k + 1) & 1, fB, mn[1], mn[2])
-        else if (k == np) HQ_BK_PUT((k + 1) & 1, fB, U.fb[1 + d], U.fb[4 + d])
-    }
-#undef HQ_BK_LOAD
-#undef HQ_BK_PUT
+#include "hq_brick_march.inc"
+}
+
+enum { HQ_FUSE_FIRST = 0, HQ_FUSE_SPREAD = 1, HQ_FUSE_LAST = 2 };
+#define HQ_FUSE_LDS_MAX (80 * 1024)
+#define HQ_BK_LDS_BYTES (2 * 3 * HQ_BK_PLANE * 8)
+
+struct hq_shell_args {
+    int32_t npatches, per_xcd, nlmax, hstride;
+    const int32_t* order;
+    const hq_patch_desc* desc;
+    const uint4* pidx;
+    const double *pc1, *pc2, *pbeta;
+    const int32_t* halo;
+    const double* nt;
+    const int32_t *src_ptr, *src_ent;
+    const double* F;
+    const int32_t *ds_ptr, *ds_ent;
+};
+
+__global__ void __launch_bounds__(HQ_BK_THREADS, 4)
+hq_k_brick_shell(int32_t count, int32_t per_xcd, const hq_brick_unit* __restrict__ units, const int32_t* __restrict__ tab,
+                 const hq_real* __restrict__ u1g, const hq_real* __restrict__ u2g, hq_real* __restrict__ ung,
+                 const double* __restrict__ nt3, const int32_t* __restrict__ src_ptr, const int32_t* __restrict__ src_ent,
+                 const double* __restrict__ F, double dt2, hq_stencil_coef sc, int32_t place, hq_shell_args S)
+{
+    extern __shared__ __align__(16) double s_dyn[];
+    const uint32_t grp = blockIdx.x >> 3, xcd = blockIdx.x & 7, nbg = (uint32_t)per_xcd, npg = (uint32_t)S.per_xcd;
+    uint32_t before, upto;
+    if (place == HQ_FUSE_FIRST) { before = min(grp, npg); upto = min(grp + 1, npg); }
+    else if (place == HQ_FUSE_LAST) { before = grp > nbg ? grp - nbg : 0u; upto = grp + 1 > nbg ? grp + 1 - nbg : 0u; }
+    else { before = grp * npg / (nbg + npg); upto = (grp + 1) * npg / (nbg + npg); }
+    if (upto == before) {
+        const int slot = (int)(xcd * nbg + (grp - before));
+        if (slot >= count) return;
+        constexpr bool PERNODE = false, BYCOMP = false, RAGGED = false;
+        double* const s_w = s_dyn;
+#include "hq_brick_march.inc"
+    } else {
+        const int slot = (int)(xcd * npg + before);
+        if (slot >= S.npatches) return;
+        constexpr int DIAG = 0;
+        const int32_t nlmax = S.nlmax, hstride = S.hstride;
+        double* __restrict__ s_u1 = s_dyn;
+        double* __restrict__ s_u2 = s_dyn + 3 * nlmax;
+        double* __restrict__ s_f = s_dyn + 6 * nlmax;
+        const int32_t* __restrict__ order = S.order;
+        const hq_patch_desc* __restrict__ desc = S.desc;
+        const uint4* __restrict__ pidx = S.pidx;
+        const double* __restrict__ pc1 = S.pc1;
+        const double* __restrict__ pc2 = S.pc2;
+        const double* __restrict__ pbeta = S.pbeta;
+        const int32_t* __restrict__ halo = S.halo;
+        const double* __restrict__ nt = S.nt;
+        const int32_t* __restrict__ src_ptr = S.src_ptr;
+        const int32_t* __restrict__ src_ent = S.src_ent;
+        const double* __restrict__ F = S.F;
+        const int32_t* __restrict__ ds_ptr = S.ds_ptr;
+        const int32_t* __restrict__ ds_ent = S.ds_ent;
+        const int32_t* const if_ptr = nullptr;
+        const int32_t* const if_ent = nullptr;
+        double* const iforce = nullptr;
+#include "hq_patch_step.inc"
+    }
 }
 
 
@@ -1224,7 +1105,7 @@
 }
 
 static void hq_brick_launch(const hq_brick_plan* P, const hq_real* u1, const hq_real* u2, hq_real* un, const double* nt3,
-                            const double* F, double dt2, hipStream_t stream, bool light = false)
+                            const double* F, double dt2, hipStream_t stream, bool light = false, bool skip_first = false)
 {
     const int32_t cnt[7] = { P->nsame - P->nrag, P->nunits - P->nsame - P->nhet - P->nrhet, P->nhet - P->npacked, P->npacked, P->nrag,
                              P->nrhet - P->nrpacked, P->nrpacked };
@@ -1233,6 +1114,7 @@
         const int k = k4 == 0 ? 0 : (k4 == 1 ? 4 : (k4 < 5 ? k4 - 1 : k4));
         const int32_t count = cnt[k];
         if (count <= 0) continue;
+        if (k == 0 && skip_first) { first += count; continue; }
         const int per_xcd = (count + 7) / 8;
         const int32_t* sp = P->d_src_ptr ? P->d_src_ptr + first : nullptr;
 #define HQ_BK_ARGS count, per_xcd, P->d_units + first, P->d_tab, u1, u2, un, nt3, sp, P->d_src_ent, (sp ? F : nullptr), dt2, hq_stencil().c
@@ -1268,4 +1150,44 @@
     }
 }
 
+static bool hq_brick_shell_fits(const hq_brick_plan* P, const hq_patch_plan* S, int32_t npatch)
+{
+    const int32_t count = P->nsame - P->nrag;
+    if (count <= 0 || npatch <= 0 || npatch > S->npatches) return false;
+    if (S->cfg.threads != HQ_BK_THREADS || hq_patch_uses_pers(S) || S->d_if_ptr) return false;
+    int32_t rows = 0;
+    if (std::max(hq_patch_step_lds(S, &rows), (size_t)HQ_BK_LDS_BYTES) > (size_t)HQ_FUSE_LDS_MAX) return false;
+    const int64_t nbg = (count + 7) / 8, npg = (npatch + 7) / 8;
+    return (nbg + npg) * npg < 0x7fffffffLL && (nbg + npg) * 8 < 0x7fffffffLL;
+}
+
+static int hq_brick_shell_launch(const hq_brick_plan* P, const hq_patch_plan* S, int32_t npatch, int place, const hq_real* u1,
+                                 const hq_real* u2, hq_real* un, const double* nt, const double* F, double dt2, hipStream_t stream)
+{
+    const int32_t count = P->nsame - P->nrag;
+    const int per_xcd = (count + 7) / 8;
+    hq_shell_args A;
+    A.npatches = npatch;
+    A.per_xcd = (npatch + 7) / 8;
+    const size_t lds = std::max(hq_patch_step_lds(S, &A.nlmax), (size_t)HQ_BK_LDS_BYTES);
+    A.hstride = S->hstride;
+    A.order = S->d_order;
+    A.desc = S->d_desc; A.pidx = S->d_pidx; A.pc1 = S->d_pc1; A.pc2 = S->d_pc2; A.pbeta = S->d_pbeta; A.halo = S->d_halo;
+    A.nt = nt;
+    A.src_ptr = S->d_src_ptr; A.src_ent = S->d_src_ent;
+    A.F = S->d_src_ptr ? F : nullptr;
+    A.ds_ptr = S->d_ds_ptr; A.ds_ent = S->d_ds_ent;
+    static bool attr_set = false;
+    if (!attr_set) {
+        if (hipFuncSetAttribute((const void*)hq_k_brick_shell, hipFuncAttributeMaxDynamicSharedMemorySize, HQ_FUSE_LDS_MAX) != hipSuccess)
+            return hq_fail(HQ_ERR_DEVICE, "hq_k_brick_shell: LDS attribute%s", "");
+        attr_set = true;
+    }
+    const int32_t* sp = P->d_src_ptr ? (const int32_t*)P->d_src_ptr : nullptr;
+    hq_k_brick_shell<<<(per_xcd + A.per_xcd) * 8, HQ_BK_THREADS, lds, stream>>>(
+        count, per_xcd, P->d_units, P->d_tab, u1, u2, un, S->d_nt3, sp, P->d_src_ent, (sp ? F : nullptr), dt2, hq_stencil().c,
+        place, A);
+    return HQ_OK;
+}
+
 #endif
diff --git a/hercules_amd/csrc/hq_brick_march.inc b/hercules_amd/csrc/hq_brick_march.inc
--- /dev/null
+++ b/hercules_amd/csrc/hq_brick_march.inc
@@ -0,0 +1,183 @@
+    const hq_brick_unit U = units[slot];
+    const int nx = U.nx, ny = U.ny, np = U.np, nxy = nx * ny, nr = 2 * (nx + 2) + 2 * ny;
+    const int t = threadIdx.x, lx = t & (HQ_BK_TX - 1), ly = t >> 6;
+    const bool active = lx < nx && ly < ny;
+    const int sidx = active ? ly * nx + lx : 0;
+    const int myrow = (ly + 1) * HQ_BK_PY + lx + 1;
+    const bool ring = t < nr;
+    int rrow;
+    {
+        int rx, ry;
+        if (t < nx + 2) { rx = t - 1; ry = -1; }
+        else if (t < 2 * (nx + 2)) { rx = t - (nx + 2) - 1; ry = ny; }
+        else if (t < 2 * (nx + 2) + ny) { rx = -1; ry = t - 2 * (nx + 2); }
+        else { rx = nx; ry = t - 2 * (nx + 2) - ny; }
+        rrow = (ry + 1) * HQ_BK_PY + rx + 1;
+    }
+    const int32_t* __restrict__ utab = tab + U.tab;
+    const int rofs = ring ? t : 0;
+    const int32_t* __restrict__ cap = utab + (int64_t)(np + 2) * nr;
+    int32_t vOut = -1, vMid = RAGGED ? cap[sidx] : 0, vCur = RAGGED ? cap[nxy + sidx] : 0, vNext = 0;
+    const int32_t id_lo = RAGGED ? (vMid >= 0 ? vMid : -vMid - 2) : cap[sidx];
+    const double beta = U.beta;
+    double P[6], Q[2];
+#pragma unroll
+    for (int i = 0; i < 6; i++) P[i] = hq_uniform(U.c1 * sc.p1[i] + U.c2 * sc.p2[i]);
+#pragma unroll
+    for (int i = 0; i < 2; i++) Q[i] = hq_uniform(U.c1 * sc.q1[i] + U.c2 * sc.q2[i]);
+    const bool has_src = F && src_ptr[slot + 1] > src_ptr[slot];
+
+    hq_real x1[3] = { 0, 0, 0 }, x2[3] = { 0, 0, 0 }, y1[3] = { 0, 0, 0 }, y2[3] = { 0, 0, 0 };
+    double mn[3] = { U.m0, U.m2, U.m1 };
+    double m0A = hq_uniform(1.0 / U.m0), m0B = m0A;
+    double fA[3] = { 0.0, 0.0, 0.0 }, fB[3] = { 0.0, 0.0, 0.0 };
+    int32_t rid = utab[rofs];
+
+#define HQ_BK_LOAD(node_)                                                                             \
+    {                                                                                                 \
+        const int64_t a_ = (node_);                                                                   \
+        if (active && (!RAGGED || a_ >= 0)) {                                                         \
+            _Pragma("unroll") for (int d = 0; d < 3; d++) { x1[d] = u1g[3 * a_ + d]; x2[d] = u2g[3 * a_ + d]; } \
+            if (PERNODE) { _Pragma("unroll") for (int d = 0; d < 3; d++) mn[d] = nt3[3 * a_ + d]; }    \
+        }                                                                                             \
+        if (ring && (!RAGGED || rid >= 0)) {                                                          \
+            const int64_t b_ = (int64_t)rid;                                                          \
+            _Pragma("unroll") for (int d = 0; d < 3; d++) { y1[d] = u1g[3 * b_ + d]; y2[d] = u2g[3 * b_ + d]; } \
+        }                                                                                             \
+    }
+#define HQ_BK_PUT(s_, acc_, M2_, M1_)                                                                 \
+    {                                                                                                 \
+        hq_lds_double* img_ = (hq_lds_double*)s_w + 3 * HQ_BK_PLANE * (s_);                            \
+        if (active) {                                                                                 \
+            _Pragma("unroll") for (int d = 0; d < 3; d++) {                                           \
+                const double a1_ = x1[d], a2_ = x2[d];                                                \
+                img_[3 * myrow + d] = a1_ + beta * (a1_ - a2_);                                       \
+                acc_[d] += (M2_) * a1_ - (M1_) * a2_;                                                 \
+            }                                                                                         \
+        }                                                                                             \
+        if (ring) { _Pragma("unroll") for (int d = 0; d < 3; d++) { const double b1_ = y1[d], b2_ = y2[d]; img_[3 * rrow + d] = b1_ + beta * (b1_ - b2_); } } \
+    }
+
+    const bool topf = !PERNODE && !RAGGED && (U.flags & HQ_BK_TOPFACE) != 0, botf = !PERNODE && !RAGGED && (U.flags & HQ_BK_BOTFACE) != 0;
+    const double rho = hq_uniform((U.c1 - U.c2) / (U.c1 + U.c2));
+
+    HQ_BK_LOAD((int64_t)id_lo)
+    rid = utab[nr + rofs];
+    if (topf) HQ_BK_PUT(0, fB, U.ft[1 + d], U.ft[4 + d])
+    else { double dummy[3] = { 0.0, 0.0, 0.0 }; HQ_BK_PUT(0, dummy, mn[1], mn[2]) }
+    for (int k = 0; k <= np + 1; k++) {
+        if (k <= np) {
+            if (RAGGED) {
+                HQ_BK_LOAD((int64_t)(vCur >= 0 ? vCur : -vCur - 2))
+                if (k < np) vNext = cap[(k + 2) * nxy + sidx];
+            } else HQ_BK_LOAD(k == np ? (int64_t)cap[nxy + sidx] : U.base + (int64_t)k * nxy + sidx)
+            if (k < np) rid = utab[(k + 2) * nr + rofs];
+        }
+        __syncthreads();
+        const hq_lds_double* __restrict__ q = (const hq_lds_double*)s_w + 3 * (HQ_BK_PLANE * (k & 1) + myrow);
+        double m[3], g[3], Uo[3];
+        if (BYCOMP) {
+            double A_x, A_y;
+            {
+                const double C = q[2], XM = q[2 - 3], XP = q[2 + 3], YM = q[2 - 3 * HQ_BK_PY], YP = q[2 + 3 * HQ_BK_PY];
+                const double MM = q[2 - 3 * HQ_BK_PY - 3], PM = q[2 - 3 * HQ_BK_PY + 3], MP = q[2 + 3 * HQ_BK_PY - 3], PP = q[2 + 3 * HQ_BK_PY + 3];
+                const double sxy = (XM + XP) + (YM + YP), dg = (MM + PP) + (PM + MP);
+                m[2] = fma(P[0], C, fma(P[2], sxy, P[4] * dg));
+                g[2] = fma(P[1], C, fma(P[3], sxy, P[5] * dg));
+                Uo[0] = fma(Q[0], XP - XM, Q[1] * ((PP - MP) + (PM - MM)));
+                Uo[1] = fma(Q[0], YP - YM, Q[1] * ((PP - PM) + (MP - MM)));
+            }
+            __builtin_amdgcn_sched_barrier(0);
+            {
+                const double C = q[0], XM = q[0 - 3], XP = q[0 + 3], YM = q[0 - 3 * HQ_BK_PY], YP = q[0 + 3 * HQ_BK_PY];
+                const double MM = q[0 - 3 * HQ_BK_PY - 3], PM = q[0 - 3 * HQ_BK_PY + 3], MP = q[0 + 3 * HQ_BK_PY - 3], PP = q[0 + 3 * HQ_BK_PY + 3];
+                const double sx = XM + XP, sy = YM + YP, dg = (MM + PP) + (PM + MP);
+                A_x = (PP + MM) - (PM + MP);
+                m[0] = fma(P[0], C, fma(P[1], sx, fma(P[2], sy, P[3] * dg)));
+                g[0] = fma(P[2], C, fma(P[3], sx, fma(P[4], sy, P[5] * dg)));
+                Uo[2] = fma(Q[0], XP - XM, Q[1] * ((PP - MP) + (PM - MM)));
+            }
+            __builtin_amdgcn_sched_barrier(0);
+            {
+                const double C = q[1], XM = q[1 - 3], XP = q[1 + 3], YM = q[1 - 3 * HQ_BK_PY], YP = q[1 + 3 * HQ_BK_PY];
+                const double MM = q[1 - 3 * HQ_BK_PY - 3], PM = q[1 - 3 * HQ_BK_PY + 3], MP = q[1 + 3 * HQ_BK_PY - 3], PP = q[1 + 3 * HQ_BK_PY + 3];
+                const double sx = XM + XP, sy = YM + YP, dg = (MM + PP) + (PM + MP);
+                A_y = (PP + MM) - (PM + MP);
+                m[1] = fma(P[0], C, fma(P[1], sy, fma(P[2], sx, fma(P[3], dg, Q[0] * A_x))));
+                g[1] = fma(P[2], C, fma(P[3], sy, fma(P[4], sx, fma(P[5], dg, Q[1] * A_x))));
+                Uo[2] += fma(Q[0], YP - YM, Q[1] * ((PP - PM) + (MP - MM)));
+            }
+            m[0] = fma(Q[0], A_y, m[0]);
+            g[0] = fma(Q[1], A_y, g[0]);
+        } else {
+            double C[3], XM[3], XP[3], YM[3], YP[3], MM[3], PM[3], MP[3], PP[3];
+#pragma unroll
+            for (int d = 0; d < 3; d++) {
+                C[d] = q[d]; XM[d] = q[d - 3]; XP[d] = q[d + 3]; YM[d] = q[d - 3 * HQ_BK_PY]; YP[d] = q[d + 3 * HQ_BK_PY];
+                MM[d] = q[d - 3 * HQ_BK_PY - 3]; PM[d] = q[d - 3 * HQ_BK_PY + 3];
+                MP[d] = q[d + 3 * HQ_BK_PY - 3]; PP[d] = q[d + 3 * HQ_BK_PY + 3];
+            }
+            double sx[3], sy[3], dg[3];
+#pragma unroll
+            for (int d = 0; d < 3; d++) { sx[d] = XM[d] + XP[d]; sy[d] = YM[d] + YP[d]; dg[d] = (MM[d] + PP[d]) + (PM[d] + MP[d]); }
+            const double A_x = (PP[0] + MM[0]) - (PM[0] + MP[0]), A_y = (PP[1] + MM[1]) - (PM[1] + MP[1]);
+            const double Bx0_z = XP[2] - XM[2], Bx0_x = XP[0] - XM[0], By0_z = YP[2] - YM[2], By0_y = YP[1] - YM[1];
+            const double Bx1_z = (PP[2] - MP[2]) + (PM[2] - MM[2]), Bx1_x = (PP[0] - MP[0]) + (PM[0] - MM[0]);
+            const double By1_z = (PP[2] - PM[2]) + (MP[2] - MM[2]), By1_y = (PP[1] - PM[1]) + (MP[1] - MM[1]);
+            const double sxy_z = sx[2] + sy[2];
+            m[0] = fma(P[0], C[0], fma(P[1], sx[0], fma(P[2], sy[0], fma(P[3], dg[0], Q[0] * A_y))));
+            m[1] = fma(P[0], C[1], fma(P[1], sy[1], fma(P[2], sx[1], fma(P[3], dg[1], Q[0] * A_x))));
+            m[2] = fma(P[0], C[2], fma(P[2], sxy_z, P[4] * dg[2]));
+            g[0] = fma(P[2], C[0], fma(P[3], sx[0], fma(P[4], sy[0], fma(P[5], dg[0], Q[1] * A_y))));
+            g[1] = fma(P[2], C[1], fma(P[3], sy[1], fma(P[4], sx[1], fma(P[5], dg[1], Q[1] * A_x))));
+            g[2] = fma(P[1], C[2], fma(P[3], sxy_z, P[5] * dg[2]));
+            Uo[0] = fma(Q[0], Bx0_z, Q[1] * Bx1_z);
+            Uo[1] = fma(Q[0], By0_z, Q[1] * By1_z);
+            Uo[2] = fma(Q[0], Bx0_x, fma(Q[1], Bx1_x, fma(Q[0], By0_y, Q[1] * By1_y)));
+        }
+        if (k == 0 && topf) {
+            m[0] = fma(rho, Uo[0], 0.5 * m[0]); m[1] = fma(rho, Uo[1], 0.5 * m[1]); m[2] = fma(-rho, Uo[2], 0.5 * m[2]);
+        }
+        if (k == np + 1 && botf && active) {
+            double f[3];
+            f[0] = fB[0] + fma(-rho, Uo[0], 0.5 * m[0]); f[1] = fB[1] + fma(-rho, Uo[1], 0.5 * m[1]); f[2] = fB[2] + fma(rho, Uo[2], 0.5 * m[2]);
+            const int local = np * nxy + sidx;
+            if (has_src) {
+                for (int i = src_ptr[slot]; i < src_ptr[slot + 1]; i++)
+                    if (src_ent[2 * i] == local) {
+                        const int li = src_ent[2 * i + 1];
+                        for (int d = 0; d < 3; d++) f[d] += F[3 * li + d] * dt2;
+                    }
+            }
+            hq_real* out = ung + 3 * (int64_t)cap[nxy + sidx];
+            const double rm = 1.0 / U.fb[0];
+#pragma unroll
+            for (int d = 0; d < 3; d++) out[d] = f[d] * rm;
+        }
+        const bool outface = k == 1 && topf;
+        if ((k >= 2 || outface) && active && (!RAGGED || vOut >= 0)) {
+            double f[3];
+#pragma unroll
+            for (int d = 0; d < 3; d++) f[d] = fA[d] + (g[d] + Uo[d]);
+            const int local = RAGGED ? (int)(vOut - U.base) : (k - 2) * nxy + sidx;
+            if (has_src) {
+                for (int i = src_ptr[slot]; i < src_ptr[slot + 1]; i++)
+                    if (src_ent[2 * i] == local) {
+                        const int li = src_ent[2 * i + 1];
+                        for (int d = 0; d < 3; d++) f[d] += F[3 * li + d] * dt2;
+                    }
+            }
+            hq_real* out = ung + 3 * (RAGGED ? (int64_t)vOut : (outface ? (int64_t)cap[sidx] : U.base + (int64_t)local));
+            const double rm = outface ? 1.0 / U.ft[0] : m0A;
+#pragma unroll
+            for (int d = 0; d < 3; d++) out[d] = f[d] * rm;
+        }
+#pragma unroll
+        for (int d = 0; d < 3; d++) { fA[d] = fB[d] + m[d]; fB[d] = g[d] - Uo[d]; }
+        if (RAGGED) { vOut = vMid; vMid = vCur; vCur = vNext; }
+        if (PERNODE) { m0A = m0B; m0B = 1.0 / mn[0]; }
+        if (k < np || (k == np && !botf)) HQ_BK_PUT((k + 1) & 1, fB, mn[1], mn[2])
+        else if (k == np) HQ_BK_PUT((k + 1) & 1, fB, U.fb[1 + d], U.fb[4 + d])
+    }
+#undef HQ_BK_LOAD
+#undef HQ_BK_PUT
diff --git a/hercules_amd/csrc/hq_engine.hip b/hercules_amd/csrc/hq_engine.hip
--- a/hercules_amd/csrc/hq_engine.hip
+++ b/hercules_amd/csrc/hq_engine.hip
@@ -150,6 +150,7 @@
     bool overlap = false;
     bool stream_masked = false;
     bool can_overlap = false;
+    int fused_place = 2;
     int reserve_cus = 8;
     int32_t nI = 0, nOI = 0;
     hq_dbuf<double> d_iforce;
@@ -914,11 +915,11 @@
 
 enum { HQ_NPHASE = 9 };
 
+static bool hq_want_brick_stream(const hq_ctx* c);
+
 static bool hq_use_brick_stream(hq_ctx* c)
 {
-    const bool solo = !hq_has_transport(c) && c->nranks == 1 && c->plan.npatches > 16 * c->plan.grid_cus;
-    const bool want = hq_given(c->opts.brick_stream) ? c->opts.brick_stream != 0 : solo;
-    if (!want || !(c->overlap || (!hq_has_transport(c) && c->nranks == 1)) || c->stream_masked || c->bricks.nunits <= 0 || c->plan.npatches <= 0) return false;
+    if (!hq_want_brick_stream(c)) return false;
     if (!c->bstream) {
         int prio_lo = 0, prio_hi = 0;
         if (hipDeviceGetStreamPriorityRange(&prio_lo, &prio_hi) != hipSuccess) return false;
@@ -935,6 +936,22 @@
     return true;
 }
 
+static bool hq_want_brick_stream(const hq_ctx* c)
+{
+    const bool solo = !hq_has_transport(c) && c->nranks == 1 && c->plan.npatches > 16 * c->plan.grid_cus;
+    const bool want = hq_given(c->opts.brick_stream) ? c->opts.brick_stream != 0 : solo;
+    return want && (c->overlap || (!hq_has_transport(c) && c->nranks == 1)) && !c->stream_masked && c->bricks.nunits > 0 && c->plan.npatches > 0;
+}
+
+static bool hq_use_fused_step(const hq_ctx* c)
+{
+    if (c->variant != HQ_VARIANT_PATCH || !hq_value_or(c->opts.fused_step, 0)) return false;
+    if (hq_has_transport(c) || c->nranks != 1 || c->group || c->overlap || hq_want_brick_stream(c)) return false;
+    if (hq_given(c->opts.brick_by_component) && c->opts.brick_by_component != 0) return false;
+    if (c->plan.ns > 0 || c->plan.nr > 0 || c->plan.nstencil > 0 || c->plan.nlattice > 0) return false;
+    return hq_brick_shell_fits(&c->bricks, &c->plan, c->plan.nb + c->plan.ne);
+}
+
 #include "hq_outputs.h"
 
 static int hq_phase(hq_ctx* c, int ph)
@@ -951,6 +968,7 @@
             int32_t nb = c->plan.nb, ne = c->plan.ne;
             if (c->overlap && !hq_patch_uses_pers(&c->plan) && nb > 0 && nb + ne <= 2 * hq_value_or(c->opts.patch_merge_rounds, 2) * c->plan.grid_cus) { nb += ne; ne = 0; }
             const bool bs = hq_use_brick_stream(c);
+            const bool fused = !bs && hq_use_fused_step(c);
             if (c->overlap) HQ_HIP(hipStreamWaitEvent(c->stream, c->ev_shared, 0));
             if (bs) {
                 HQ_HIP(hipStreamWaitEvent(c->stream, c->ev_bricks, 0));
@@ -961,13 +979,14 @@
             auto launch_bricks = [&]() {
                 if (c->bricks.nunits > 0)
                     hq_brick_launch(&c->bricks, c->d_u[c->now], c->d_u[c->prev], c->d_u[c->spare], c->plan.d_nt3, F, c->dt2,
-                                    bs ? c->bstream : c->stream, hq_given(c->opts.brick_by_component) ? c->opts.brick_by_component != 0 : c->overlap);
+                                    bs ? c->bstream : c->stream, hq_given(c->opts.brick_by_component) ? c->opts.brick_by_component != 0 : c->overlap, fused);
                 if (bs) hipEventRecord(c->ev_bricks, c->bstream);
             };
             hq_mark(c);
             hq_clock_begin(c);
             hq_clock(c, hq_ctx::HQ_CLK_STEP0, c->stream);
             if (bs) hq_clock(c, hq_ctx::HQ_CLK_INT0, c->bstream);
+            if (fused) hq_clock(c, hq_ctx::HQ_CLK_INT0, c->stream);
             bool chain_marked = false;
             auto chain_released = [&]() {
                 if (!chain_marked && c->overlap) hq_clock(c, hq_ctx::HQ_CLK_CHAIN0, c->cstream);
@@ -997,14 +1016,17 @@
                     chain_released();
                     hq_patch_launch(&c->plan, nb, ne, c->d_u[c->now], c->d_u[c->prev], c->d_u[c->spare], c->d_nt, F,
                                     c->dt2, c->d_iforce, c->stream, c->reserve_cus);
+                } else if (fused) {
+                    HQ_TRY(hq_brick_shell_launch(&c->bricks, &c->plan, nb + ne, c->fused_place, c->d_u[c->now], c->d_u[c->prev],
+                                                 c->d_u[c->spare], c->d_nt, F, c->dt2, c->stream));
                 } else {
                     hq_patch_launch(&c->plan, 0, nb + ne, c->d_u[c->now], c->d_u[c->prev], c->d_u[c->spare], c->d_nt, F,
                                     c->dt2, c->d_iforce, c->stream);
                 }
             }
             if (bs) HQ_HIP(hipEventRecord(c->ev_patches, c->stream));
-            hq_clock(c, hq_ctx::HQ_CLK_SHELL1, c->stream);
-            if (!bs) hq_clock(c, hq_ctx::HQ_CLK_INT0, c->stream);
+            if (!fused) hq_clock(c, hq_ctx::HQ_CLK_SHELL1, c->stream);
+            if (!bs && !fused) hq_clock(c, hq_ctx::HQ_CLK_INT0, c->stream);
             launch_bricks();
             hq_clock(c, hq_ctx::HQ_CLK_INT1, bs ? c->bstream : c->stream);
             if (!c->overlap && hq_has_transport(c)) hq_clock(c, hq_ctx::HQ_CLK_CHAIN0, c->stream);
@@ -1311,6 +1333,14 @@
     return HQ_OK;
 }
 
+static int hq_fused_place_of(const hq_options& o)
+{
+    const char* w = hq_opt_env_only(o, "HQ_FUSED_PLACE");
+    if (w && !strcmp(w, "first")) return HQ_FUSE_FIRST;
+    if (w && !strcmp(w, "spread")) return HQ_FUSE_SPREAD;
+    return HQ_FUSE_LAST;
+}
+
 static int hq_create_impl(const hq_desc* d, int device, const hq_options& opts, hq_ctx** out)
 {
     if (!d || !out) return hq_fail(HQ_ERR_ARG, "null argument%s", "");
@@ -1347,6 +1377,7 @@
     if (!c) return hq_fail(HQ_ERR_NOMEM, "out of host memory%s", "");
     c->device = device;
     c->opts = opts;
+    c->fused_place = hq_fused_place_of(opts);
     c->E = d->lenum; c->N = d->nharbored; c->ldnnum = d->ldnnum;
     c->dt = d->deltaT; c->dt2 = d->deltaT * d->deltaT;
     c->rank = d->rank; c->nranks = d->nranks > 0 ? d->nranks : 1;
@@ -2104,6 +2135,8 @@
     return HQ_OK;
 }
 
+extern "C" int hq_fused_step(hq_ctx* c) { return c && hq_use_fused_step(c) ? 1 : 0; }
+
 extern "C" const char* hq_dominant_kernel(hq_ctx* c)
 {
     if (!c || c->variant != HQ_VARIANT_PATCH) return "hq_k_element_scatter";
diff --git a/hercules_amd/csrc/hq_opts.h b/hercules_amd/csrc/hq_opts.h
--- a/hercules_amd/csrc/hq_opts.h
+++ b/hercules_amd/csrc/hq_opts.h
@@ -26,6 +26,7 @@
     HQ_OPT_D("HQ_LOOPBACK_DELAY_US", loopback_delay_us), HQ_OPT_I("HQ_PATCH_VERBOSE", verbose), HQ_OPT_I("HQ_QUIET", quiet),
     HQ_OPT_I("HQ_BRICK_RAGGED", brick_ragged), HQ_OPT_I("HQ_BRICK_RAGGED_MINFILL", brick_ragged_minfill),
     HQ_OPT_I("HQ_PHASE_TIMING", phase_timing), HQ_OPT_I("HQ_BRICK_RAGGED_HET", brick_ragged_het),
+    HQ_OPT_I("HQ_FUSED_STEP", fused_step),
 };
 #undef HQ_OPT_I
 #undef HQ_OPT_D
@@ -38,7 +39,6 @@
         else *(double*)((char*)o + e.off) = -1.0;
     }
     o->allow_env = -1;
-    o->reserved0 = -1;
 }
 
 static void hq_options_adopt(hq_options* dst, const hq_options* src)
diff --git a/hercules_amd/csrc/hq_patch.h b/hercules_amd/csrc/hq_patch.h
--- a/hercules_amd/csrc/hq_patch.h
+++ b/hercules_amd/csrc/hq_patch.h
@@ -845,159 +845,7 @@
 
     const int slot = (int)(blockIdx.x & 7) * per_xcd + (int)(blockIdx.x >> 3);
     if (slot >= npatches) return;
-    const int p = order ? order[slot] : slot;
-    const int tid = threadIdx.x, T = blockDim.x;
-    HQ_STAMP(0);
-    const int32_t* __restrict__ hl = halo + (int64_t)p * hstride;
-    int32_t hid[4];
-#pragma unroll
-    for (int k = 0; k < 4; k++) hid[k] = hl[(k * T + tid) / 3];
-    const hq_patch_desc D = desc[p];
-    const int own3 = D.nown * 3, halo3 = D.nhalo * 3;
-    for (int i = own3 + tid; i < 3 * D.nacc; i += T) s_f[i] = 0.0;
-    if (DIAG == 6 && D.nown > 0) HQ_STAMP(1);
-
-    const bool wf = (D.flags & HQ_PATCH_WFORM) != 0;
-    const double wbeta = wf ? pbeta[D.pair_off] : 0.0;
-    const int o2off = 3 * (nlmax / 2);
-    hq_pair_data cur;
-    const int cstep = (D.flags & HQ_PATCH_UNIFORM) ? 0 : 1;
-    if (tid < D.npairs) cur = hq_pair_load(pidx, pc1, pc2, pbeta, D.pidx_off + tid, D.pair_off + cstep * tid);
-
-    {
-        const hq_real* g1 = u1g + 3 * (int64_t)D.base;
-        const hq_real* g2 = u2g + 3 * (int64_t)D.base;
-        for (int i0 = 0; i0 < own3 || i0 < halo3; i0 += 4 * T) {
-            double a1[4], a2[4], b1[4], b2[4];
-#pragma unroll
-            for (int k = 0; k < 4; k++) {
-                int i = i0 + k * T + tid;
-                if (DIAG == 2) { a1[k] = a2[k] = b1[k] = b2[k] = 1e-3 * i; continue; }
-                if (i < own3) { a1[k] = g1[i]; a2[k] = g2[i]; }
-                if (i < halo3) {
-                    int h = i / 3, d = i - 3 * h;
-                    int32_t id = hid[k];
-                    if (i0 > 0) id = hl[h];
-                    int64_t g = 3 * (int64_t)id + d;
-                    b1[k] = u1g[g]; b2[k] = u2g[g];
-                }
-            }
-#pragma unroll
-            for (int k = 0; k < 4; k++) {
-                int i = i0 + k * T + tid;
-                if (wf) {
-                    if (i < own3) { s_u1[i] = a1[k] + wbeta * (a1[k] - a2[k]); s_u2[i] = a1[k]; s_u2[o2off + i] = a2[k]; s_f[i] = 0.0; }
-                    if (i < halo3) s_u1[own3 + i] = b1[k] + wbeta * (b1[k] - b2[k]);
-                } else {
-                    if (i < own3) { s_u1[i] = a1[k]; s_u2[i] = a2[k]; s_f[i] = 0.0; }
-                    if (i < halo3) { s_u1[own3 + i] = b1[k]; s_u2[own3 + i] = b2[k]; }
-                }
-            }
-        }
-    }
-    HQ_STAMP(2);
-    __syncthreads();
-    HQ_STAMP(3);
-
-    const bool iso = (D.flags & HQ_PATCH_ISO) != 0;
-    double np[7];
-    if (tid < D.nown) {
-        if (iso) {
-            const double* q = nt3 + 3 * ((int64_t)D.base + ((D.flags & HQ_PATCH_NTSAME) ? 0 : tid));
-            np[0] = q[0];
-            np[1] = q[1];
-            np[4] = q[2];
-        } else {
-            const double* q = nt + 7 * ((int64_t)D.base + tid);
-#pragma unroll
-            for (int k = 0; k < 7; k++) np[k] = q[k];
-        }
-    }
-
-    for (int q = tid; q < (DIAG == 1 ? 0 : D.npairs); q += T) {
-        hq_pair_data nxt;
-        if (q + T < D.npairs)
-            nxt = hq_pair_load(pidx, pc1, pc2, pbeta, D.pidx_off + q + T, D.pair_off + cstep * (q + T));
-        const uint4 raw = cur.raw;
-        const double beta = cur.beta;
-        int l[8];
-        HQ_PIDX_UNPACK(l, raw)
-        double X[8], Y[8], Z[8];
-        if (wf) {
-#pragma unroll
-            for (int n = 0; n < 8; n++) {
-                const double* a = &s_u1[3 * (DIAG == 5 ? (tid & 7) : l[n])];
-                X[n] = a[0]; Y[n] = a[1]; Z[n] = a[2];
-            }
-        } else {
-#pragma unroll
-            for (int n = 0; n < 8; n++) {
-                const double* a = &s_u1[3 * (DIAG == 5 ? (tid & 7) : l[n])];
-                const double* b = &s_u2[3 * (DIAG == 5 ? (tid & 7) : l[n])];
-                double a0 = a[0], a1 = a[1], a2 = a[2];
-                X[n] = a0 + beta * (a0 - b[0]);
-                Y[n] = a1 + beta * (a1 - b[1]);
-                Z[n] = a2 + beta * (a2 - b[2]);
-            }
-        }
-        hq_element_force(X, Y, Z, cur.c1, cur.c2);
-#pragma unroll
-        for (int n = 0; n < 8; n++) {
-            if (DIAG == 4) { if (X[n] + Y[n] + Z[n] == 1.2345e-300) s_f[n] = 1.0; continue; }
-            if (HQ_PIDX_HAS_ACC(raw, n)) {
-                atomicAdd(&s_f[3 * l[n] + 0], X[n]);
-                atomicAdd(&s_f[3 * l[n] + 1], Y[n]);
-                atomicAdd(&s_f[3 * l[n] + 2], Z[n]);
-            }
-        }
-        cur = nxt;
-    }
-    HQ_STAMP(4);
-    if (F) {
-        for (int k = src_ptr[p] + tid; k < src_ptr[p + 1]; k += T) {
-            int ln = src_ent[2 * k], li = src_ent[2 * k + 1];
-            for (int d = 0; d < 3; d++) atomicAdd(&s_f[3 * ln + d], F[3 * li + d] * dt2);
-        }
-    }
-    if (ds_ptr && ds_ptr[p + 1] > ds_ptr[p]) {
-        __syncthreads();
-        for (int k = ds_ptr[p] + tid; k < ds_ptr[p + 1]; k += T) {
-            const int src = ds_ent[3 * k], dst = ds_ent[3 * k + 1];
-            const double deps = (double)(unsigned)ds_ent[3 * k + 2];
-            for (int d = 0; d < 3; d++) atomicAdd(&s_f[3 * dst + d], s_f[3 * src + d] / deps);
-        }
-    }
-    __syncthreads();
-    HQ_STAMP(5);
-
-    for (int n = tid; n < (DIAG == 3 ? (tid == 0 ? 1 : 0) : D.nown); n += T) {
-        if (n != tid) {
-            if (iso) {
-                const double* q = nt3 + 3 * ((int64_t)D.base + ((D.flags & HQ_PATCH_NTSAME) ? 0 : n));
-                np[0] = q[0]; np[1] = q[1]; np[4] = q[2];
-            } else {
-                const double* q = nt + 7 * ((int64_t)D.base + n);
-#pragma unroll
-                for (int k = 0; k < 7; k++) np[k] = q[k];
-            }
-        }
-        hq_real* out = ung + 3 * ((int64_t)D.base + n);
-#pragma unroll
-        for (int d = 0; d < 3; d++) {
-            const double m2 = iso ? np[1] : np[1 + d], m1 = iso ? np[4] : np[4 + d];
-            const double x1 = wf ? s_u2[3 * n + d] : s_u1[3 * n + d], x2 = wf ? s_u2[o2off + 3 * n + d] : s_u2[3 * n + d];
-            double f = s_f[3 * n + d] + (m2 * x1 - m1 * x2);
-            out[d] = f / np[0];
-        }
-    }
-    if (if_ptr) {
-        for (int k = if_ptr[p] + tid; k < if_ptr[p + 1]; k += T) {
-            int ln = if_ent[2 * k];
-            double* o = iforce + 3 * (int64_t)if_ent[2 * k + 1];
-            o[0] = s_f[3 * ln]; o[1] = s_f[3 * ln + 1]; o[2] = s_f[3 * ln + 2];
-        }
-    }
-    HQ_STAMP(6);
+#include "hq_patch_step.inc"
 }
 
 __device__ __forceinline__ hq_patch_desc hq_patch_desc_or_empty(const hq_patch_desc* __restrict__ desc, int p)
@@ -2137,6 +1985,14 @@
     return (12 * (size_t)P->nrows + 3 * (size_t)(P->cfg.pmax + P->cfg.vmax) + 36) * sizeof(double) <= 160 * 1024;
 }
 
+static size_t hq_patch_step_lds(const hq_patch_plan* P, int32_t* rows)
+{
+    const int32_t step_nl = P->step_nl > 0 ? P->step_nl : P->cfg.nlmax;
+    const int32_t step_na = P->step_nl > 0 && P->max_nacc > 0 ? P->max_nacc : P->cfg.pmax + P->cfg.vmax;
+    *rows = step_nl;
+    return (6 * (size_t)step_nl + 3 * (size_t)step_na) * sizeof(double);
+}
+
 static void hq_patch_launch(const hq_patch_plan* P, int32_t first, int32_t count, const hq_real* u1,
                             const hq_real* u2, hq_real* un, const double* nt, const double* F, double dt2,
                             double* iforce, hipStream_t stream, int reserve_cus = 0)
@@ -2146,9 +2002,8 @@
     if (getenv("HQ_X_NO_SHELL")) return;
 #endif
     int per_xcd = (count + 7) / 8;
-    const int32_t step_nl = P->step_nl > 0 ? P->step_nl : P->cfg.nlmax;
-    const int32_t step_na = P->step_nl > 0 && P->max_nacc > 0 ? P->max_nacc : P->cfg.pmax + P->cfg.vmax;
-    size_t lds = (6 * (size_t)step_nl + 3 * (size_t)step_na) * sizeof(double);
+    int32_t step_nl = 0;
+    const size_t lds = hq_patch_step_lds(P, &step_nl);
 #ifdef HQ_PATCH_PROFILING
     const int diag = getenv("HQ_PATCH_DIAG") ? atoi(getenv("HQ_PATCH_DIAG")) : 0;
     if (diag == 6) {
diff --git a/hercules_amd/csrc/hq_patch_step.inc b/hercules_amd/csrc/hq_patch_step.inc
--- /dev/null
+++ b/hercules_amd/csrc/hq_patch_step.inc
@@ -0,0 +1,153 @@
+    const int p = order ? order[slot] : slot;
+    const int tid = threadIdx.x, T = blockDim.x;
+    HQ_STAMP(0);
+    const int32_t* __restrict__ hl = halo + (int64_t)p * hstride;
+    int32_t hid[4];
+#pragma unroll
+    for (int k = 0; k < 4; k++) hid[k] = hl[(k * T + tid) / 3];
+    const hq_patch_desc D = desc[p];
+    const int own3 = D.nown * 3, halo3 = D.nhalo * 3;
+    for (int i = own3 + tid; i < 3 * D.nacc; i += T) s_f[i] = 0.0;
+    if (DIAG == 6 && D.nown > 0) HQ_STAMP(1);
+
+    const bool wf = (D.flags & HQ_PATCH_WFORM) != 0;
+    const double wbeta = wf ? pbeta[D.pair_off] : 0.0;
+    const int o2off = 3 * (nlmax / 2);
+    hq_pair_data cur;
+    const int cstep = (D.flags & HQ_PATCH_UNIFORM) ? 0 : 1;
+    if (tid < D.npairs) cur = hq_pair_load(pidx, pc1, pc2, pbeta, D.pidx_off + tid, D.pair_off + cstep * tid);
+
+    {
+        const hq_real* g1 = u1g + 3 * (int64_t)D.base;
+        const hq_real* g2 = u2g + 3 * (int64_t)D.base;
+        for (int i0 = 0; i0 < own3 || i0 < halo3; i0 += 4 * T) {
+            double a1[4], a2[4], b1[4], b2[4];
+#pragma unroll
+            for (int k = 0; k < 4; k++) {
+                int i = i0 + k * T + tid;
+                if (DIAG == 2) { a1[k] = a2[k] = b1[k] = b2[k] = 1e-3 * i; continue; }
+                if (i < own3) { a1[k] = g1[i]; a2[k] = g2[i]; }
+                if (i < halo3) {
+                    int h = i / 3, d = i - 3 * h;
+                    int32_t id = hid[k];
+                    if (i0 > 0) id = hl[h];
+                    int64_t g = 3 * (int64_t)id + d;
+                    b1[k] = u1g[g]; b2[k] = u2g[g];
+                }
+            }
+#pragma unroll
+            for (int k = 0; k < 4; k++) {
+                int i = i0 + k * T + tid;
+                if (wf) {
+                    if (i < own3) { s_u1[i] = a1[k] + wbeta * (a1[k] - a2[k]); s_u2[i] = a1[k]; s_u2[o2off + i] = a2[k]; s_f[i] = 0.0; }
+                    if (i < halo3) s_u1[own3 + i] = b1[k] + wbeta * (b1[k] - b2[k]);
+                } else {
+                    if (i < own3) { s_u1[i] = a1[k]; s_u2[i] = a2[k]; s_f[i] = 0.0; }
+                    if (i < halo3) { s_u1[own3 + i] = b1[k]; s_u2[own3 + i] = b2[k]; }
+                }
+            }
+        }
+    }
+    HQ_STAMP(2);
+    __syncthreads();
+    HQ_STAMP(3);
+
+    const bool iso = (D.flags & HQ_PATCH_ISO) != 0;
+    double np[7];
+    if (tid < D.nown) {
+        if (iso) {
+            const double* q = nt3 + 3 * ((int64_t)D.base + ((D.flags & HQ_PATCH_NTSAME) ? 0 : tid));
+            np[0] = q[0];
+            np[1] = q[1];
+            np[4] = q[2];
+        } else {
+            const double* q = nt + 7 * ((int64_t)D.base + tid);
+#pragma unroll
+            for (int k = 0; k < 7; k++) np[k] = q[k];
+        }
+    }
+
+    for (int q = tid; q < (DIAG == 1 ? 0 : D.npairs); q += T) {
+        hq_pair_data nxt;
+        if (q + T < D.npairs)
+            nxt = hq_pair_load(pidx, pc1, pc2, pbeta, D.pidx_off + q + T, D.pair_off + cstep * (q + T));
+        const uint4 raw = cur.raw;
+        const double beta = cur.beta;
+        int l[8];
+        HQ_PIDX_UNPACK(l, raw)
+        double X[8], Y[8], Z[8];
+        if (wf) {
+#pragma unroll
+            for (int n = 0; n < 8; n++) {
+                const double* a = &s_u1[3 * (DIAG == 5 ? (tid & 7) : l[n])];
+                X[n] = a[0]; Y[n] = a[1]; Z[n] = a[2];
+            }
+        } else {
+#pragma unroll
+            for (int n = 0; n < 8; n++) {
+                const double* a = &s_u1[3 * (DIAG == 5 ? (tid & 7) : l[n])];
+                const double* b = &s_u2[3 * (DIAG == 5 ? (tid & 7) : l[n])];
+                double a0 = a[0], a1 = a[1], a2 = a[2];
+                X[n] = a0 + beta * (a0 - b[0]);
+                Y[n] = a1 + beta * (a1 - b[1]);
+                Z[n] = a2 + beta * (a2 - b[2]);
+            }
+        }
+        hq_element_force(X, Y, Z, cur.c1, cur.c2);
+#pragma unroll
+        for (int n = 0; n < 8; n++) {
+            if (DIAG == 4) { if (X[n] + Y[n] + Z[n] == 1.2345e-300) s_f[n] = 1.0; continue; }
+            if (HQ_PIDX_HAS_ACC(raw, n)) {
+                atomicAdd(&s_f[3 * l[n] + 0], X[n]);
+                atomicAdd(&s_f[3 * l[n] + 1], Y[n]);
+                atomicAdd(&s_f[3 * l[n] + 2], Z[n]);
+            }
+        }
+        cur = nxt;
+    }
+    HQ_STAMP(4);
+    if (F) {
+        for (int k = src_ptr[p] + tid; k < src_ptr[p + 1]; k += T) {
+            int ln = src_ent[2 * k], li = src_ent[2 * k + 1];
+            for (int d = 0; d < 3; d++) atomicAdd(&s_f[3 * ln + d], F[3 * li + d] * dt2);
+        }
+    }
+    if (ds_ptr && ds_ptr[p + 1] > ds_ptr[p]) {
+        __syncthreads();
+        for (int k = ds_ptr[p] + tid; k < ds_ptr[p + 1]; k += T) {
+            const int src = ds_ent[3 * k], dst = ds_ent[3 * k + 1];
+            const double deps = (double)(unsigned)ds_ent[3 * k + 2];
+            for (int d = 0; d < 3; d++) atomicAdd(&s_f[3 * dst + d], s_f[3 * src + d] / deps);
+        }
+    }
+    __syncthreads();
+    HQ_STAMP(5);
+
+    for (int n = tid; n < (DIAG == 3 ? (tid == 0 ? 1 : 0) : D.nown); n += T) {
+        if (n != tid) {
+            if (iso) {
+                const double* q = nt3 + 3 * ((int64_t)D.base + ((D.flags & HQ_PATCH_NTSAME) ? 0 : n));
+                np[0] = q[0]; np[1] = q[1]; np[4] = q[2];
+            } else {
+                const double* q = nt + 7 * ((int64_t)D.base + n);
+#pragma unroll
+                for (int k = 0; k < 7; k++) np[k] = q[k];
+            }
+        }
+        hq_real* out = ung + 3 * ((int64_t)D.base + n);
+#pragma unroll
+        for (int d = 0; d < 3; d++) {
+            const double m2 = iso ? np[1] : np[1 + d], m1 = iso ? np[4] : np[4 + d];
+            const double x1 = wf ? s_u2[3 * n + d] : s_u1[3 * n + d], x2 = wf ? s_u2[o2off + 3 * n + d] : s_u2[3 * n + d];
+            double f = s_f[3 * n + d] + (m2 * x1 - m1 * x2);
+            out[d] = f / np[0];
+        }
+    }
+    if (if_ptr) {
+        for (int k = if_ptr[p] + tid; k < if_ptr[p + 1]; k += T) {
+            int ln = if_ent[2 * k];
+            double* o = iforce + 3 * (int64_t)if_ent[2 * k + 1];
+            o[0] = s_f[3 * ln]; o[1] = s_f[3 * ln + 1]; o[2] = s_f[3 * ln + 2];
+        }
+    }
+    HQ_STAMP(6);
diff --git a/include/hq_solver.h b/include/hq_solver.h
--- a/include/hq_solver.h
+++ b/include/hq_solver.h
@@ -155,7 +155,7 @@
     int32_t brick_ragged_minfill;
     int32_t allow_env;
     int32_t brick_ragged_het;
-    int32_t reserved0;
+    int32_t fused_step;
     int32_t phase_timing;
 } hq_options;
 
@@ -305,6 +305,8 @@
 
 HQ_API const char* hq_dominant_kernel(hq_ctx* ctx);
 
+HQ_API int hq_fused_step(hq_ctx* ctx);
+
 #ifdef __cplusplus
 }
 #endif
```
